# SitaoLuan/ACM-GNN

Measured on AMD Instinct MI355X. Metric: edges/sec ACM-GCN fwd+bwd on twitch-gamer, higher is better.
Workload: dtype f32; 1 GPU; twitch-gamer-shaped Chung-Lu graph: 168114 nodes, 6797557 undirected edges, nnz(A_low)=13763228, F_in=7, hidden=64, classes=2; 2-layer acmgcnp (variant=0, structure_info=0, attention LayerNorm on), dropout 0.1 (counter-based, masks regenerated in the kernels), AdamW (fused); step = fwd + NLL loss + bwd + optimizer update; parallelism=single-gpu, node_order=degree, launch=hipGraph replay of the captured step (1 consecutive steps per graph), operator_form=pattern-only P + row scale (shared by A_low and A_low^T), full=False, input_pipeline=True, checked=False

## Files before the change

acm_gnn_amd/_lib.py:

```python
import ctypes as C
import os
import threading

from . import build as _build

c_f32p = C.POINTER(C.c_float)
c_i32p = C.POINTER(C.c_int32)

ACM_OK = 0
STATUS_NAMES = {1: "ACM_EINVAL", 2: "ACM_ESHAPE", 3: "ACM_EHIP", 4: "ACM_EUNSUPPORTED", 5: "ACM_ENOMEM"}
ABI_VERSION = 28

EXPORTED_SYMBOLS = (
    "acm_version", "acm_last_error", "acm_tuning_get", "acm_tuning_set", "acm_csr_create", "acm_csr_transpose", "acm_csr_slice_rows",
    "acm_csr_destroy", "acm_csr_info", "acm_csr_build_streams", "acm_csr_build_item_streams", "acm_spmm_workspace_bytes", "acm_gemm_workspace_bytes",
    "acm_gemm", "acm_gemm_blocks", "acm_gemm_drop", "acm_proj3", "acm_gemm_split", "acm_proj_fwd", "acm_proj_fwd_at", "acm_proj_bwd_workspace_bytes", "acm_proj_bwd", "acm_spmm", "acm_spmm_v", "acm_spmm_ex", "acm_cast_bf16", "acm_conv_fwd", "acm_conv_bwd_local_workspace_bytes",
    "acm_conv_bwd_local", "acm_conv_bwd_spmm", "acm_conv_agg_fwd", "acm_conv_agg_bwd_workspace_bytes",
    "acm_conv_agg_bwd", "acm_nll_loss_workspace_bytes", "acm_nll_loss", "acm_adam_step", "acm_dropout",
    "acm_reduce_flush", "acm_conv_fwd_tail_workspace_bytes", "acm_conv_fwd_tail", "acm_shard_plan",
    "acm_conv_acmii_fwd_workspace_bytes", "acm_conv_acmii_fwd", "acm_linear_fwd", "acm_bias_act", "acm_bias_act_bwd_workspace_bytes", "acm_bias_act_bwd",
    "acm_acmii_table_bytes", "acm_acmii_table", "acm_conv_acmii_v_fwd", "acm_conv_acmii_v_bwd_workspace_bytes", "acm_conv_acmii_v_bwd",
    "acm_linear_bwd_workspace_bytes", "acm_linear_bwd", "acm_linear_fwd_add", "acm_linear_bwd_recompute",
    "acm_small_step_workspace_bytes", "acm_small_step", "acm_conv_head_fwd", "acm_conv_aggw_fwd", "acm_conv_aggw_bwd_workspace_bytes", "acm_conv_aggw_bwd",
    "acm_eval_metrics_workspace_bytes", "acm_eval_metrics",
)


class Dropout(C.Structure):
    _fields_ = [("p", C.c_float), ("tag", C.c_int32), ("seed", C.c_uint64), ("step", C.c_void_p),
                ("row_offset", C.c_int64), ("step_offset", C.c_int64)]


class CsrInfo(C.Structure):
    _fields_ = [("n_rows", C.c_int64), ("n_cols", C.c_int64), ("nnz", C.c_int64),
                ("n_items", C.c_int64), ("n_long_rows", C.c_int64), ("n_partial_slots", C.c_int64),
                ("chunk", C.c_int32), ("max_degree", C.c_int32),
                ("indptr", C.c_void_p), ("indices", C.c_void_p), ("vals", C.c_void_p),
                ("src_pos", C.c_void_p),
                ("stream_steps", C.c_int64), ("stream_slices", C.c_int64),
                ("stream_waves", C.c_int32), ("stream_long_rows", C.c_int32),
                ("item_stream_waves", C.c_int32), ("reserved", C.c_int32), ("item_stream_batches", C.c_int64)]


class ConvFwd(C.Structure):
    _fields_ = [("f_out", C.c_int32), ("n_channels", C.c_int32), ("relu_after", C.c_int32),
                ("relu_mlp", C.c_int32), ("layernorm", C.c_int32), ("scale", C.c_float),
                ("row_offset", C.c_int64),
                ("g_low", C.c_void_p), ("ld_g_low", C.c_int64),
                ("g_high", C.c_void_p), ("ld_g_high", C.c_int64),
                ("g_struc", C.c_void_p), ("ld_g_struc", C.c_int64),
                ("s_high", C.c_void_p), ("ld_s_high", C.c_int64),
                ("s_mlp", C.c_void_p), ("ld_s_mlp", C.c_int64),
                ("s_struc", C.c_void_p), ("ld_s_struc", C.c_int64),
                ("deg", C.c_void_p),
                ("att_vec", C.c_void_p * 4), ("ln_weight", C.c_void_p * 4), ("ln_bias", C.c_void_p * 4),
                ("att_mix", C.c_void_p),
                ("out", C.c_void_p), ("ld_out", C.c_int64),
                ("pre", C.c_void_p), ("ld_pre", C.c_int64),
                ("att", C.c_void_p), ("post_scale", C.c_void_p), ("ld_post_scale", C.c_int64), ("post_relu", C.c_int32),
                ("gather_bf16", C.c_int32), ("row_scale", C.c_void_p), ("post_drop", Dropout)]


class ConvBwdLocal(C.Structure):
    _fields_ = [("f_out", C.c_int32), ("n_channels", C.c_int32), ("relu_after", C.c_int32),
                ("relu_mlp", C.c_int32), ("layernorm", C.c_int32), ("scale", C.c_float),
                ("grad_out", C.c_void_p), ("ld_grad_out", C.c_int64),
                ("pre", C.c_void_p), ("ld_pre", C.c_int64),
                ("s_mlp", C.c_void_p), ("ld_s_mlp", C.c_int64),
                ("deg", C.c_void_p),
                ("att_vec", C.c_void_p * 4), ("ln_weight", C.c_void_p * 4), ("ln_bias", C.c_void_p * 4),
                ("att_mix", C.c_void_p),
                ("g_low", C.c_void_p), ("ld_g_low", C.c_int64),
                ("g_high", C.c_void_p), ("ld_g_high", C.c_int64),
                ("g_mlp", C.c_void_p), ("ld_g_mlp", C.c_int64),
                ("g_struc", C.c_void_p), ("ld_g_struc", C.c_int64),
                ("d_att_vec", C.c_void_p * 4), ("d_ln_weight", C.c_void_p * 4),
                ("d_ln_bias", C.c_void_p * 4), ("d_att_mix", C.c_void_p),
                ("post_scale", C.c_void_p), ("ld_post_scale", C.c_int64), ("post_relu", C.c_int32),
                ("g_scale", C.c_void_p), ("post_drop", Dropout), ("defer", C.c_void_p)]


class ConvBwdSpmm(C.Structure):
    _fields_ = [("f_out", C.c_int32), ("row_offset", C.c_int64),
                ("g_low", C.c_void_p), ("ld_g_low", C.c_int64),
                ("g_high", C.c_void_p), ("ld_g_high", C.c_int64),
                ("g_struc", C.c_void_p), ("ld_g_struc", C.c_int64),
                ("s_high", C.c_void_p), ("ld_s_high", C.c_int64),
                ("s_struc", C.c_void_p), ("ld_s_struc", C.c_int64),
                ("inv_deg", C.c_void_p),
                ("mask_low", C.c_void_p), ("ld_mask_low", C.c_int64),
                ("mask_high", C.c_void_p), ("ld_mask_high", C.c_int64),
                ("dz_low", C.c_void_p), ("ld_dz_low", C.c_int64),
                ("dz_high", C.c_void_p), ("ld_dz_high", C.c_int64),
                ("d_struc", C.c_void_p), ("ld_d_struc", C.c_int64), ("self_scale", C.c_void_p),
                ("gather_bf16", C.c_int32)]


class ConvAggFwd(C.Structure):
    _fields_ = [("f_in", C.c_int32), ("f_pad", C.c_int32), ("f_out", C.c_int32), ("relu_after", C.c_int32),
                ("relu_mlp", C.c_int32), ("layernorm", C.c_int32), ("scale", C.c_float),
                ("xg", C.c_void_p), ("ld_xg", C.c_int64),
                ("xs", C.c_void_p), ("ld_xs", C.c_int64),
                ("w_low", C.c_void_p), ("w_high", C.c_void_p), ("w_mlp", C.c_void_p), ("ld_w", C.c_int64),
                ("att_vec", C.c_void_p * 4), ("ln_weight", C.c_void_p * 4), ("ln_bias", C.c_void_p * 4),
                ("att_mix", C.c_void_p),
                ("out", C.c_void_p), ("ld_out", C.c_int64),
                ("agg", C.c_void_p), ("ld_agg", C.c_int64),
                ("att", C.c_void_p), ("post_scale", C.c_void_p), ("ld_post_scale", C.c_int64), ("post_relu", C.c_int32),
                ("n_channels", C.c_int32), ("sg", C.c_void_p), ("ld_sg", C.c_int64), ("sg_bf16", C.c_int32),
                ("ss", C.c_void_p), ("ld_ss", C.c_int64), ("deg", C.c_void_p),
                ("ps", C.c_void_p), ("ld_ps", C.c_int64), ("row_scale", C.c_void_p), ("post_drop", Dropout),
                ("head_stats", C.c_void_p), ("ld_head_stats", C.c_int64),
                ("next_w_low", C.c_void_p), ("next_w_high", C.c_void_p), ("next_w_mlp", C.c_void_p), ("next_ld_w", C.c_int64),
                ("next_f", C.c_int32), ("next_relu", C.c_int32),
                ("next_zlh", C.c_void_p), ("ld_next_zlh", C.c_int64), ("next_zi", C.c_void_p), ("ld_next_zi", C.c_int64),
                ("agg_given", C.c_int32), ("reserved0", C.c_int32),
                ("agg_copy", C.c_void_p), ("ld_agg_copy", C.c_int64), ("xs_copy", C.c_void_p), ("ld_xs_copy", C.c_int64),
                ("next_x", C.c_void_p), ("ld_next_x", C.c_int64), ("next_drop", Dropout)]


class ConvAggBwd(C.Structure):
    _fields_ = [("f_in", C.c_int32), ("f_pad", C.c_int32), ("f_out", C.c_int32), ("relu_after", C.c_int32),
                ("relu_mlp", C.c_int32), ("layernorm", C.c_int32), ("scale", C.c_float),
                ("grad_out", C.c_void_p), ("ld_grad_out", C.c_int64),
                ("agg", C.c_void_p), ("ld_agg", C.c_int64),
                ("xs", C.c_void_p), ("ld_xs", C.c_int64),
                ("w_low", C.c_void_p), ("w_high", C.c_void_p), ("w_mlp", C.c_void_p), ("ld_w", C.c_int64),
                ("att_vec", C.c_void_p * 4), ("ln_weight", C.c_void_p * 4), ("ln_bias", C.c_void_p * 4),
                ("att_mix", C.c_void_p),
                ("d_params", C.c_void_p), ("post_scale", C.c_void_p), ("ld_post_scale", C.c_int64), ("post_relu", C.c_int32),
                ("n_channels", C.c_int32), ("ps", C.c_void_p), ("ld_ps", C.c_int64),
                ("ss", C.c_void_p), ("ld_ss", C.c_int64), ("deg", C.c_void_p),
                ("g_struc", C.c_void_p), ("ld_g_struc", C.c_int64), ("g_struc_scale", C.c_void_p),
                ("post_drop", Dropout), ("defer", C.c_void_p),
                ("head_stats", C.c_void_p), ("ld_head_stats", C.c_int64),
                ("out", C.c_void_p), ("ld_out", C.c_int64),
                ("next_a", C.c_void_p), ("next_xg", C.c_void_p), ("ld_next_xg", C.c_int64),
                ("next_row_scale", C.c_void_p), ("next_agg", C.c_void_p), ("ld_next_agg", C.c_int64),
                ("proj_dz", C.c_void_p), ("ld_proj_dz", C.c_int64),
                ("proj_w_low", C.c_void_p), ("proj_w_high", C.c_void_p), ("proj_w_mlp", C.c_void_p), ("proj_ld_w", C.c_int64),
                ("proj_f", C.c_int32), ("proj_d_w", C.c_void_p)]


class ConvAcmiiFwd(C.Structure):
    _fields_ = [("f_in", C.c_int32), ("f_pad", C.c_int32), ("f_out", C.c_int32), ("layernorm", C.c_int32),
                ("scale", C.c_float),
                ("xg", C.c_void_p), ("ld_xg", C.c_int64), ("xs", C.c_void_p), ("ld_xs", C.c_int64),
                ("w_low", C.c_void_p), ("w_high", C.c_void_p), ("w_mlp", C.c_void_p), ("ld_w", C.c_int64),
                ("att_vec", C.c_void_p * 4), ("ln_weight", C.c_void_p * 4), ("ln_bias", C.c_void_p * 4),
                ("att_mix", C.c_void_p),
                ("out", C.c_void_p), ("ld_out", C.c_int64), ("pre", C.c_void_p), ("ld_pre", C.c_int64),
                ("att", C.c_void_p), ("zlh", C.c_void_p), ("ld_zlh", C.c_int64), ("zi", C.c_void_p), ("ld_zi", C.c_int64),
                ("post_scale", C.c_void_p), ("ld_post_scale", C.c_int64), ("post_relu", C.c_int32),
                ("row_scale", C.c_void_p), ("post_drop", Dropout),
                ("n_channels", C.c_int32), ("ps", C.c_void_p), ("ld_ps", C.c_int64), ("ss", C.c_void_p), ("ld_ss", C.c_int64),
                ("deg", C.c_void_p)]


class ConvAcmiiBwd(C.Structure):
    _fields_ = [("f_in", C.c_int32), ("table", C.c_void_p),
                ("g_low", C.c_void_p), ("ld_g_low", C.c_int64), ("g_high", C.c_void_p), ("ld_g_high", C.c_int64),
                ("g_mlp", C.c_void_p), ("ld_g_mlp", C.c_int64), ("x", C.c_void_p), ("ld_x", C.c_int64),
                ("self_offset", C.c_int64), ("row_scale", C.c_void_p),
                ("d_w_low", C.c_void_p), ("d_w_high", C.c_void_p), ("d_w_mlp", C.c_void_p), ("ld_dw", C.c_int64),
                ("defer", C.c_void_p)]


class Loss(C.Structure):
    _fields_ = [("n_classes", C.c_int32), ("labels", C.c_void_p), ("row_weight", C.c_void_p),
                ("loss", C.c_void_p), ("dlogits", C.c_void_p), ("ld_dlogits", C.c_int64)]


class ReduceSeg(C.Structure):
    _fields_ = [("partial", C.c_void_p), ("nblk", C.c_int32), ("row_stride", C.c_int32),
                ("q0", C.c_int32), ("len", C.c_int32), ("dst", C.c_void_p),
                ("inner", C.c_int32), ("col_block", C.c_int32),
                ("outer_stride", C.c_int64), ("block_stride", C.c_int64),
                ("elem_stride", C.c_int32), ("reserved", C.c_int32)]


class ReduceList(C.Structure):
    _fields_ = [("n", C.c_int32), ("cap", C.c_int32), ("segs", C.POINTER(ReduceSeg))]


class SpmmOpts(C.Structure):
    _fields_ = [("vals", C.c_void_p), ("row_scale", C.c_void_p), ("sub", C.c_void_p), ("ld_sub", C.c_int64),
                ("sub_scale", C.c_void_p), ("relu", C.c_int32), ("g_bf16", C.c_int32)]


class AdamTensor(C.Structure):
    _fields_ = [("param", C.c_void_p), ("grad", C.c_void_p), ("exp_avg", C.c_void_p), ("exp_avg_sq", C.c_void_p),
                ("step", C.c_void_p), ("numel", C.c_int64)]


class AdamConfig(C.Structure):
    _fields_ = [("lr", C.c_double), ("beta1", C.c_double), ("beta2", C.c_double), ("eps", C.c_double),
                ("weight_decay", C.c_double), ("decoupled", C.c_int32), ("also_advance", C.c_void_p),
                ("arrive", C.c_void_p), ("pending", C.c_void_p)]


SMALL_ROLES = 17
SR_W_LOW, SR_W_HIGH, SR_W_MLP, SR_V_LOW, SR_V_HIGH, SR_V_MLP, SR_V_STRUC = range(7)
SR_LNW_LOW, SR_LNW_HIGH, SR_LNW_MLP, SR_LNW_STRUC, SR_LNB_LOW, SR_LNB_HIGH, SR_LNB_MLP, SR_LNB_STRUC, SR_MIX, SR_STRUC = range(7, 17)


class SmallStep(C.Structure):
    _fields_ = [("n_classes", C.c_int32), ("n_channels", C.c_int32), ("relu_before", C.c_int32), ("layernorm", C.c_int32),
                ("scale", C.c_float), ("train", C.c_int32), ("update", C.c_int32), ("reserved0", C.c_int32),
                ("t", (AdamTensor * SMALL_ROLES) * 2),
                ("x_vals", C.c_void_p), ("xt_src_pos", C.c_void_p), ("xt_vals", C.c_void_p), ("f_in", C.c_int32), ("reserved1", C.c_int32), ("drop_in", Dropout), ("drop_hidden", Dropout),
                ("row_scale", C.c_void_p), ("labels", C.c_void_p), ("row_weight", C.c_void_p), ("loss", C.c_void_p),
                ("logits", C.c_void_p), ("att1", C.c_void_p), ("att2", C.c_void_p),
                ("lr", C.c_double), ("beta1", C.c_double), ("beta2", C.c_double), ("eps", C.c_double),
                ("weight_decay", C.c_double), ("decoupled", C.c_int32), ("also_advance", C.c_void_p), ("arrive", C.c_void_p),
                ("workspace", C.c_void_p), ("workspace_bytes", C.c_size_t)]


_lib = None
_lock = threading.Lock()


def _declare(lib):
    vp, i64, i32, sz = C.c_void_p, C.c_int64, C.c_int, C.c_size_t
    lib.acm_version.restype = C.c_int
    lib.acm_version.argtypes = []
    lib.acm_last_error.restype = C.c_char_p
    lib.acm_last_error.argtypes = []
    lib.acm_csr_create.argtypes = [i64, i64, i64, vp, vp, vp, i32, C.POINTER(vp)]
    lib.acm_csr_transpose.argtypes = [vp, i32, C.POINTER(vp)]
    lib.acm_csr_slice_rows.argtypes = [vp, i64, i64, i32, C.POINTER(vp)]
    lib.acm_csr_destroy.argtypes = [vp]
    lib.acm_csr_destroy.restype = None
    lib.acm_csr_info.argtypes = [vp, C.POINTER(CsrInfo)]
    lib.acm_csr_build_streams.argtypes = [vp, i32, i32]
    lib.acm_csr_build_item_streams.argtypes = [vp, i32]
    lib.acm_shard_plan.argtypes = [i64, vp, i32, i64, vp]
    lib.acm_conv_acmii_fwd_workspace_bytes.argtypes = [vp, C.POINTER(sz)]
    lib.acm_conv_acmii_fwd.argtypes = [vp, C.POINTER(ConvAcmiiFwd), vp, sz, vp]
    lib.acm_acmii_table_bytes.argtypes = [i64, C.POINTER(sz)]
    lib.acm_acmii_table.argtypes = [i64, i32, vp, i64, vp, vp, i64, vp, sz, vp]
    lib.acm_conv_acmii_v_fwd.argtypes = [vp, C.POINTER(ConvAcmiiFwd), vp, vp, sz, vp]
    lib.acm_conv_acmii_v_bwd_workspace_bytes.argtypes = [vp, C.POINTER(sz)]
    lib.acm_conv_acmii_v_bwd.argtypes = [vp, C.POINTER(ConvAcmiiBwd), vp, sz, vp]
    lib.acm_linear_fwd.argtypes = [i64, i64, i64, vp, i64, vp, i64, vp, i32, vp, vp, i64, vp, sz, vp]
    lib.acm_bias_act.argtypes = [i64, i32, vp, i64, vp, i32, vp, vp]
    lib.acm_linear_bwd_workspace_bytes.argtypes = [i64, i32, i32, C.POINTER(sz)]
    lib.acm_linear_bwd.argtypes = [i64, i32, i32, vp, i64, vp, i64, vp, i64, C.c_float, i32, vp, i64, vp, vp, sz, vp, vp]
    lib.acm_linear_fwd_add.argtypes = [i64, i32, i32, vp, i64, vp, i64, vp, i32, vp, vp, i64, vp, i64, vp]
    lib.acm_linear_bwd_recompute.argtypes = [i64, i32, i32, vp, i64, vp, i64, vp, i32, vp, vp, i64, vp, i64, vp, vp, sz, vp, vp]
    lib.acm_bias_act_bwd_workspace_bytes.argtypes = [i64, i32, C.POINTER(sz)]
    lib.acm_bias_act_bwd.argtypes = [i64, i32, vp, i64, vp, i64, C.c_float, i32, vp, i64, vp, vp, sz, vp, vp]
    lib.acm_spmm_workspace_bytes.argtypes = [vp, i32, C.POINTER(sz)]
    lib.acm_gemm_workspace_bytes.argtypes = [i32, i32, i64, i64, i64, C.POINTER(sz)]
    lib.acm_gemm.argtypes = [i32, i32, i64, i64, i64, vp, i64, vp, i64, vp, i64, i32, vp, sz, vp]
    lib.acm_proj_bwd_workspace_bytes.argtypes = [i64, i64, i32, C.POINTER(sz)]
    lib.acm_proj_fwd.argtypes = [i64, i64, i32, vp, i64, vp, vp, vp, i64, i32, vp, i64, vp, i64, vp]
    lib.acm_proj_fwd_at.argtypes = [i64, i64, i32, vp, i64, vp, vp, vp, i64, i32, vp, i64, i64, vp, i64, vp]
    lib.acm_proj_bwd.argtypes = [i64, i64, i32, vp, i64, vp, i64, vp, vp, vp, i64, vp, i64, vp, i64, i64, i64, vp, sz, vp, vp]
    lib.acm_gemm_split.argtypes = [i32, i32, i64, i64, i64, vp, i64, vp, i64, vp, i64, i64, vp, i64, i32, vp, sz, vp]
    lib.acm_gemm_blocks.argtypes = [i32, i32, i64, i64, i64, vp, i64, vp, i64, vp, i64, i64, i64, i32, vp, sz, vp]
    lib.acm_gemm_drop.argtypes = [i32, i32, i64, i64, i64, vp, i64, vp, i64, vp, i64, i64, i64, i32, C.POINTER(Dropout), vp, sz, vp]
    lib.acm_proj3.argtypes = [i64, i64, vp, i64, vp, vp, vp, i64, i64, i64, vp, i64, i64, vp, i64, i32, C.POINTER(Dropout), vp]
    lib.acm_spmm.argtypes = [vp, vp, i64, i32, vp, i64, vp, sz, vp]
    lib.acm_spmm_v.argtypes = [vp, vp, vp, i64, i32, vp, i64, i32, vp, sz, vp]
    lib.acm_adam_step.argtypes = [i32, vp, vp, vp]
    lib.acm_dropout.argtypes = [i64, i64, vp, i64, vp, i64, i64, vp, vp]
    lib.acm_spmm_ex.argtypes = [vp, vp, i64, i32, vp, i64, vp, vp, sz, vp]
    lib.acm_cast_bf16.argtypes = [i64, i64, vp, i64, vp, i64, vp]
    lib.acm_conv_fwd.argtypes = [vp, C.POINTER(ConvFwd), vp, sz, vp]
    lib.acm_conv_head_fwd.argtypes = [i64, C.POINTER(ConvFwd), vp]
    lib.acm_conv_aggw_bwd_workspace_bytes.argtypes = [i64, i64, C.POINTER(C.c_size_t)]
    lib.acm_conv_aggw_bwd.argtypes = [i64, i64, i64, vp, i64, vp, i64, C.POINTER(ConvBwdLocal), vp, vp, vp, i64, vp, C.c_size_t, vp]
    lib.acm_conv_aggw_fwd.argtypes = [i64, i64, i64, vp, i64, vp, i64, vp, vp, vp, i64, vp, i64, C.POINTER(ConvFwd), vp]
    lib.acm_conv_bwd_local_workspace_bytes.argtypes = [i64, i32, i32, C.POINTER(sz)]
    lib.acm_conv_bwd_local.argtypes = [i64, C.POINTER(ConvBwdLocal), vp, sz, vp]
    lib.acm_conv_bwd_spmm.argtypes = [vp, C.POINTER(ConvBwdSpmm), vp, sz, vp]
    lib.acm_conv_agg_fwd.argtypes = [vp, C.POINTER(ConvAggFwd), vp, sz, vp]
    lib.acm_conv_agg_bwd_workspace_bytes.argtypes = [i64, i32, i32, C.POINTER(sz)]
    lib.acm_conv_agg_bwd.argtypes = [i64, C.POINTER(ConvAggBwd), vp, sz, vp]
    lib.acm_nll_loss_workspace_bytes.argtypes = [i64, C.POINTER(sz)]
    lib.acm_nll_loss.argtypes = [i64, i32, vp, i64, vp, vp, vp, vp, i64, vp, sz, vp, vp]
    lib.acm_eval_metrics_workspace_bytes.argtypes = [i64, i32, C.POINTER(sz)]
    lib.acm_eval_metrics.argtypes = [i64, i32, vp, i64, vp, vp, i64, i32, i32, vp, vp, sz, vp]
    lib.acm_reduce_flush.argtypes = [vp, vp]
    lib.acm_conv_fwd_tail_workspace_bytes.argtypes = [i64, i32, i32, C.POINTER(sz)]
    lib.acm_conv_fwd_tail.argtypes = [vp, C.POINTER(ConvFwd), C.POINTER(Loss), C.POINTER(ConvBwdLocal), vp, sz, vp, sz, vp]
    lib.acm_small_step_workspace_bytes.argtypes = [vp, vp, vp, C.POINTER(sz)]
    lib.acm_small_step.argtypes = [vp, vp, vp, C.POINTER(SmallStep), vp]
    for name in EXPORTED_SYMBOLS:
        fn = getattr(lib, name)
        if name not in ("acm_version", "acm_last_error", "acm_csr_destroy"):
            fn.restype = C.c_int


def library_path():
    return os.environ.get("ACM_HIP_LIBRARY", _build.LIB_PATH)


def load(build_if_missing=True):
    global _lib
    with _lock:
        if _lib is not None:
            return _lib
        path = library_path()
        if "ACM_HIP_LIBRARY" not in os.environ and build_if_missing:
            try:
                if _build.is_stale():
                    _build.build_library()
            except Exception as exc:
                if not os.path.exists(path):
                    raise RuntimeError(f"libacm_hip.so is not built and cannot be built here: {exc}")
        if not os.path.exists(path):
            raise RuntimeError(f"libacm_hip.so not found at {path}; run `python -m acm_gnn_amd.build`")
        lib = C.CDLL(path)
        _declare(lib)
        ver = lib.acm_version()
        if ver != ABI_VERSION:
            raise RuntimeError(f"libacm_hip.so ABI version {ver} != expected {ABI_VERSION}")
        _lib = lib
        return _lib


def check(status, what=""):
    if status != ACM_OK:
        msg = load().acm_last_error().decode(errors="replace")
        raise RuntimeError(f"{what or 'libacm_hip'} failed with {STATUS_NAMES.get(status, status)}: {msg}")
```

acm_gnn_amd/csrc/acm_common.h:

```cpp
#pragma once

#include <hip/hip_runtime.h>
#include <math.h>
#include <stdint.h>

#include "acm_hip.h"

#define ACM_WAVE 64
#define ACM_NXCD 8
#define ACM_WINDOW 16
#define ACM_MIN_CHUNK 128
#define ACM_MAX_CHUNK 1024
#define ACM_GROUPS_IN_FLIGHT 8192
#define ACM_LN_EPS 1e-5f

void acm_set_error(const char* fmt, ...);
const acm_tuning_t& acm_tuning();
#define ACM_ROWS16_EPI 1
#define ACM_ROWS16_BWD 2
#define ACM_ROWS16_LOCAL 4
#define ACM_GEMM_ROWS 1
#define ACM_GEMM_BX3 2
#define ACM_GEMM_BX3_WIDE 4
#define ACM_GEMM_ROWS_ALWAYS 8

#define ACM_CHECK_HIP(expr)                                                            \
    do {                                                                               \
        hipError_t e__ = (expr);                                                       \
        if (e__ != hipSuccess) {                                                       \
            acm_set_error("%s -> %s (%s:%d)", #expr, hipGetErrorString(e__), __FILE__, \
                          __LINE__);                                                   \
            return ACM_EHIP;                                                           \
        }                                                                              \
    } while (0)

#define ACM_REQUIRE(cond, code, ...)    \
    do {                                \
        if (!(cond)) {                  \
            acm_set_error(__VA_ARGS__); \
            return (code);              \
        }                               \
    } while (0)

struct AcmItem {
    int32_t row, begin, end, slot;
};
struct AcmLongRow {
    int32_t row, slot_begin, slot_end, windows;
};

#define ACM_STREAM_SENTINEL 0x07FFFFFF
#define ACM_STREAM_PAD_STEPS 8
struct AcmStreams {
    int32_t* ids;
    int32_t* waves;
    int32_t* items;
    AcmLongRow* long_rows;
    int32_t* long_index;
    int32_t* counters;
    float* slots;
    int64_t total_steps, n_slices, n_long, n_slots;
    int32_t n_waves, lmax;
};

#define ACM_ITEM_STREAM_PAD 8
struct AcmItemStreams {
    int32_t* ids;
    int32_t* quads;
    int32_t* waves;
    int64_t total_batches, n_quads;
    int32_t n_waves;
};

struct acm_csr {
    int64_t n_rows, n_cols, nnz;
    int32_t chunk, max_degree;
    int32_t* indptr;
    int32_t* indices;
    float* vals;
    int32_t* src_pos;
    AcmItem* items;
    int64_t n_items;
    AcmLongRow* long_rows;
    int32_t* long_index;
    int64_t n_long;
    int64_t n_slots;
    int64_t n_windows;
    int64_t n_multi;
    AcmStreams* streams;
    AcmItemStreams* item_streams;
    int device;
};

struct StreamView {
    const int32_t* ids;
    const int32_t* waves;
    const int32_t* items;
    const AcmLongRow* long_rows;
    const int32_t* long_index;
    int32_t* counters;
    float* slots;
    unsigned ids_bytes, slots_bytes;
    int n_waves;
};

struct CsrView {
    const AcmItem* items;
    int n_items;
    const AcmLongRow* long_rows;
    const int32_t* long_index;
    int n_long;
    int n_windows;
    int n_multi;
    const int32_t* indices;
    const float* vals;
};

int acm_reduce_emit(acm_reduce_list_t* defer, const acm_reduce_seg_t* segs, int n, hipStream_t st);
int acm_reduce_check_segment(const acm_reduce_seg_t& sg, int index);

int acm_spmm_internal(const acm_csr* a, const void* G, int64_t ldg, int width, float* Y, int64_t ldy,
                      const acm_spmm_opts_t* o, void* workspace, size_t workspace_bytes, acm_stream_t stream,
                      bool* defer_fixup);
int acm_bwd_local_reduce(const acm_conv_bwd_local_t* p, const float* partial, int nblk, hipStream_t st);
int acm_bwd_local16(const acm_conv_bwd_local_t* p, int64_t n_rows, float* partial, int max_blocks, hipStream_t s);
int acm_agg_epi16(const acm_conv_agg_fwd_t* p, int64_t n_rows, bool* next_done, hipStream_t s);
struct GatherRole;
int acm_agg_bwd16(const acm_conv_agg_bwd_t* p, int64_t n_rows, float* partial, int max_blocks, hipStream_t s, const GatherRole* gr,
                  int gather_blocks);
int acm_acmii_fixup_launch(const acm_csr_t* a, const acm_conv_acmii_fwd_t* p, const float* partial, hipStream_t s);
bool acm_gemm_rows_nn_ok(int64_t M, int64_t N, int64_t K, const float* B, int64_t ldb);
int acm_gemm_rows_nn(int64_t M, int64_t N, int64_t K, const float* A, int64_t lda, const float* B, int64_t ldb, float* C,
                     int64_t ldc, int relu, const acm_dropout_t* drop, hipStream_t st);
bool acm_gemm_rows_tn_ok(int64_t n_rows, int64_t K, int64_t N);
int acm_gemm_rows_tn_blocks(int64_t n_rows);
int acm_gemm_rows_tn(int64_t n_rows, int64_t K, int64_t N, const float* X, int64_t ldx, const float* Dz, int64_t lddz,
                     float* slabs, int blocks, const acm_dropout_t* drop, hipStream_t st);
bool acm_gemm_bx3_nn_ok(int64_t M, int64_t N, int64_t K, const float* A, int64_t lda);
int acm_gemm_bx3_nn(int64_t M, int64_t N, int64_t K, const float* A, int64_t lda, const float* B, int64_t ldb, float* C,
                    int64_t ldc, int relu, const acm_dropout_t* drop, hipStream_t st);
bool acm_gemm_bx3_tn_ok(int64_t n_rows, int64_t K, int64_t N);
int acm_gemm_bx3_tn_blocks(int64_t n_rows, int64_t K);
int acm_gemm_bx3_tn(int64_t n_rows, int64_t K, int64_t N, const float* X, int64_t ldx, const float* Dz, int64_t lddz,
                    float* slabs, int blocks, const acm_dropout_t* drop, hipStream_t st);
int acm_linear_fwd_narrow(int64_t n_rows, int64_t f_in, int64_t f_out, const float* X, int64_t ldx, const float* W, int64_t ldw,
                          const float* bias, int relu, const acm_dropout_t* drop, float* Y, int64_t ldy, hipStream_t s,
                          const float* add, int64_t ld_add);

static inline CsrView acm_view(const acm_csr* a) {
    CsrView v;
    v.items = a->items;
    v.n_items = (int)a->n_items;
    v.long_rows = a->long_rows;
    v.long_index = a->long_index;
    v.n_long = (int)a->n_long;
    v.n_windows = (int)a->n_windows;
    v.n_multi = (int)a->n_multi;
    v.indices = a->indices;
    v.vals = a->vals;
    return v;
}

#ifdef __HIPCC__
template <int CTRL>
__device__ __forceinline__ float acm_dpp(float v) {
    return __int_as_float(__builtin_amdgcn_update_dpp(0, __float_as_int(v), CTRL, 0xf, 0xf, false));
}
typedef unsigned acm_u32x2 __attribute__((ext_vector_type(2)));
template <int W>
__device__ __forceinline__ float acm_group_sum(float v) {
    static_assert(W == 1 || W == 2 || W == 4 || W == 8 || W == 16 || W == 32 || W == 64, "group width");
    if (W >= 2) v += acm_dpp<0xB1>(v);
    if (W >= 4) v += acm_dpp<0x4E>(v);
    if (W >= 8) v += acm_dpp<0x141>(v);
    if (W >= 16) v += acm_dpp<0x140>(v);
    if (W >= 32) {
        const acm_u32x2 r = __builtin_amdgcn_permlane16_swap(__float_as_uint(v), __float_as_uint(v), false, false);
        v = __uint_as_float(r[0]) + __uint_as_float(r[1]);
    }
    if (W >= 64) {
        const acm_u32x2 r = __builtin_amdgcn_permlane32_swap(__float_as_uint(v), __float_as_uint(v), false, false);
        v = __uint_as_float(r[0]) + __uint_as_float(r[1]);
    }
    return v;
}

__device__ __forceinline__ float acm_cross_row_sum(float v) {
    acm_u32x2 r = __builtin_amdgcn_permlane16_swap(__float_as_uint(v), __float_as_uint(v), false, false);
    v = __uint_as_float(r[0]) + __uint_as_float(r[1]);
    r = __builtin_amdgcn_permlane32_swap(__float_as_uint(v), __float_as_uint(v), false, false);
    return __uint_as_float(r[0]) + __uint_as_float(r[1]);
}

__device__ __forceinline__ int acm_row_bcast(int v, int u) {
#define ACM_BC(U) case U: return __builtin_amdgcn_update_dpp(0, v, 0x150 + U, 0xf, 0xf, false)
    switch (u & 15) {
        ACM_BC(0); ACM_BC(1); ACM_BC(2); ACM_BC(3); ACM_BC(4); ACM_BC(5); ACM_BC(6); ACM_BC(7);
        ACM_BC(8); ACM_BC(9); ACM_BC(10); ACM_BC(11); ACM_BC(12); ACM_BC(13); ACM_BC(14);
        default: return __builtin_amdgcn_update_dpp(0, v, 0x15F, 0xf, 0xf, false);
    }
#undef ACM_BC
}

__device__ __forceinline__ int acm_uniform(int v) { return __builtin_amdgcn_readfirstlane(v); }
__device__ __forceinline__ float acm_lane_f(float v, int lane) {
    return __int_as_float(__builtin_amdgcn_readlane(__float_as_int(v), lane));
}

__device__ __forceinline__ float acm_nll_row(int C, const float* zi, int yi, float wi, float* di) {
    if (wi == 0.f) {
        for (int c = 0; c < C; ++c) di[c] = 0.f;
        return 0.f;
    }
    float m = -INFINITY;
    for (int c = 0; c < C; ++c) m = fmaxf(m, zi[c]);
    float s = 0.f;
    for (int c = 0; c < C; ++c) s += expf(zi[c] - m);
    const float lse = m + logf(s);
    const float inv = 1.0f / s;
    const float zy = zi[yi];
    for (int c = 0; c < C; ++c) di[c] = wi * (expf(zi[c] - m) * inv - (c == yi ? 1.f : 0.f));
    return wi * (lse - zy);
}

struct AcmDropCtx {
    unsigned k0, k1, c2, c3, thresh, tag16;
    float inv_keep;
    long row_offset;
    bool on;
};

__device__ __forceinline__ AcmDropCtx acm_drop_ctx(const acm_dropout_t& d) {
    AcmDropCtx c;
    c.on = d.p > 0.f;
    const unsigned long long step = c.on ? (unsigned long long)(d.step[0] + d.step_offset) : 0ull;
    c.k0 = (unsigned)d.seed;
    c.k1 = (unsigned)(d.seed >> 32);
    c.c2 = (unsigned)step;
    c.c3 = (unsigned)(step >> 32);
    const double t = (double)d.p * 4294967296.0;
    c.thresh = t >= 4294967295.0 ? 0xFFFFFFFFu : (unsigned)t;
    c.tag16 = ((unsigned)d.tag) << 16;
    c.inv_keep = 1.0f / (1.0f - d.p);
    c.row_offset = (long)d.row_offset;
    return c;
// ... 42 lines not shown
```

acm_gnn_amd/csrc/acm_conv.hip:

```cpp
#include "acm_gather_device.h"

struct EpiFwd {
    static constexpr bool kFusedHead = true;
    using Args = acm_conv_fwd_t;
    template <class L, int NG>
    static __device__ __forceinline__ void apply(const Args& p, int row, const L& lay, int F,
                                                 const float (&acc)[NG][L::NV]) {
        constexpr int NV = L::NV;
        float H[4][NV], hn[4][NV], xhat[4][NV], pre[3][NV];
        const float dg = (NG == 3) ? p.deg[row] : 0.f;
        const float rs = p.row_scale ? p.row_scale[row] : 1.f;
#pragma unroll
        for (int i = 0; i < NV; ++i) {
            const int col = lay.col(i);
            const bool ok = col < F;
            const float zh = ok ? p.s_high[(long)row * p.ld_s_high + col] : 0.f;
            const float zi = ok ? p.s_mlp[(long)row * p.ld_s_mlp + col] : 0.f;
            const float p0 = rs * acc[0][i];
            const float p1 = zh - rs * acc[1][i];
            pre[0][i] = p0;
            pre[1][i] = p1;
            H[0][i] = p.relu_after ? fmaxf(p0, 0.f) : p0;
            H[1][i] = p.relu_after ? fmaxf(p1, 0.f) : p1;
            H[2][i] = p.relu_mlp ? fmaxf(zi, 0.f) : zi;
// ... 62 lines not shown
                                                            const float* __restrict__ partial, int row_blocks) {
    const int F = p.f_out;
    float acc[NG][FP];
    if ((int)blockIdx.x >= row_blocks) {
        const int m = threadIdx.x & 15;
        const int w = ((int)blockIdx.x - row_blocks) * 16 + (threadIdx.x >> 4);
        if (w >= csr.n_long) return;
        const AcmLongRow lr = csr.long_rows[w];
#pragma unroll
        for (int c = 0; c < NG; ++c)
#pragma unroll
            for (int f = 0; f < FP; ++f) acc[c][f] = 0.f;
        for (int s = lr.slot_begin + m; s < lr.slot_end; s += 16) {
            const float* ps = partial + (long)s * (NG * F);
#pragma unroll
            for (int c = 0; c < NG; ++c)
#pragma unroll
                for (int f = 0; f < FP; ++f)
                    if (f < F) acc[c][f] += ps[c * F + f];
        }
#pragma unroll
        for (int c = 0; c < NG; ++c)
#pragma unroll
            for (int f = 0; f < FP; ++f) acc[c][f] = acm_group_sum<16>(acc[c][f]);
        const LaySerial<FP> lay{m == 0};
        EpiFwd::apply<LaySerial<FP>, NG>(p, lr.row, lay, F, acc);
        return;
    }
    const int row = blockIdx.x * 256 + threadIdx.x;
    if (row >= n_rows) return;
    if (csr.long_index && csr.long_index[row] >= 0) return;
    const float* pr = p.pre + (long)row * p.ld_pre;
#pragma unroll
    for (int c = 0; c < NG; ++c)
#pragma unroll
        for (int f = 0; f < FP; ++f) acc[c][f] = (f < F) ? pr[c * F + f] : 0.f;
    const LaySerial<FP> lay{true};
    EpiFwd::apply<LaySerial<FP>, NG>(p, row, lay, F, acc);
}

__global__ __launch_bounds__(256) void conv_head_rows_kernel(acm_conv_fwd_t p, int n_rows) {
    const int lane = threadIdx.x & 63, m = lane & 15;
    const int row = ((int)blockIdx.x * 4 + (threadIdx.x >> 6)) * 4 + (lane >> 4);
    if (row >= n_rows) return;
    constexpr int F = 64;
    const float4 a = *reinterpret_cast<const float4*>(p.g_low + (long)row * p.ld_g_low + 4 * m);
    const float4 b = *reinterpret_cast<const float4*>(p.g_high + (long)row * p.ld_g_high + 4 * m);
    const float4 zh4 = *reinterpret_cast<const float4*>(p.s_high + (long)row * p.ld_s_high + 4 * m);
    const float4 zi4 = *reinterpret_cast<const float4*>(p.s_mlp + (long)row * p.ld_s_mlp + 4 * m);
    const float aa[4] = {a.x, a.y, a.z, a.w}, bb[4] = {b.x, b.y, b.z, b.w};
    const float zh[4] = {zh4.x, zh4.y, zh4.z, zh4.w}, zi[4] = {zi4.x, zi4.y, zi4.z, zi4.w};
    float H[4][4], hn[4][4], xhat[4][4], pre[2][4];
#pragma unroll
    for (int i = 0; i < 4; ++i) {
        const float p0 = 1.f * aa[i];
        const float p1 = zh[i] - 1.f * bb[i];
        pre[0][i] = p0, pre[1][i] = p1;
        H[0][i] = p.relu_after ? fmaxf(p0, 0.f) : p0;
        H[1][i] = p.relu_after ? fmaxf(p1, 0.f) : p1;
        H[2][i] = p.relu_mlp ? fmaxf(zi[i], 0.f) : zi[i];
        H[3][i] = 0.f;
    }
    const LayRow16 lay{lane};
    HeadOut ho;
    const HeadParams hp = acm_head_params(p);
    acm_head<LayRow16, 3>(lay, F, p.layernorm, hp, H, hn, xhat, ho);
    float o[4];
    const AcmDropCtx dc = acm_drop_ctx(p.post_drop);
#pragma unroll
    for (int i = 0; i < 4; ++i) {
        const int col = 4 * m + i;
        float v = ho.alpha[0] * H[0][i] + ho.alpha[1] * H[1][i] + ho.alpha[2] * H[2][i];
        v *= p.scale;
        if (p.post_relu) v = fmaxf(v, 0.f);
        if (p.post_scale) v *= p.post_scale[(long)row * p.ld_post_scale + col];
        if (p.post_drop.p > 0.f) v *= acm_drop1(dc, row, col);
        o[i] = v;
    }
    *reinterpret_cast<float4*>(p.out + (long)row * p.ld_out + 4 * m) = make_float4(o[0], o[1], o[2], o[3]);
    float* pr = p.pre + (long)row * p.ld_pre + 4 * m;
    *reinterpret_cast<float4*>(pr) = make_float4(pre[0][0], pre[0][1], pre[0][2], pre[0][3]);
    *reinterpret_cast<float4*>(pr + F) = make_float4(pre[1][0], pre[1][1], pre[1][2], pre[1][3]);
    if (m == 0) *reinterpret_cast<float4*>(p.att + (long)row * 4) = make_float4(ho.alpha[0], ho.alpha[1], ho.alpha[2], ho.alpha[3]);
}

extern "C" int acm_conv_head_fwd(int64_t n_rows, const acm_conv_fwd_t* p, acm_stream_t stream) {
    ACM_REQUIRE(p, ACM_EINVAL, "acm_conv_head_fwd: NULL argument");
    ACM_REQUIRE(n_rows >= 0 && n_rows < INT32_MAX, ACM_ESHAPE, "acm_conv_head_fwd: bad row count");
    ACM_REQUIRE(p->f_out == 64 && p->n_channels == 3 && !p->gather_bf16 && !p->row_scale && !p->deg, ACM_EUNSUPPORTED,
                "acm_conv_head_fwd: three fp32 channels of 64 columns, no row scale (got F %d, k %d)", p->f_out, p->n_channels);
    ACM_REQUIRE(p->g_low && p->g_high && p->s_high && p->s_mlp && p->out && p->pre && p->att && p->att_mix, ACM_EINVAL,
                "acm_conv_head_fwd: NULL pointer in the parameter block");
    const uintptr_t bits = (uintptr_t)p->g_low | (uintptr_t)p->g_high | (uintptr_t)p->s_high | (uintptr_t)p->s_mlp | (uintptr_t)p->out |
                           (uintptr_t)p->pre | (uintptr_t)p->att;
    ACM_REQUIRE((p->ld_g_low | p->ld_g_high | p->ld_s_high | p->ld_s_mlp | p->ld_out | p->ld_pre) % 4 == 0 && (bits & 15) == 0,
                ACM_EUNSUPPORTED, "acm_conv_head_fwd: every row (inputs, out, pre, att) must be 16-byte aligned");
    if (n_rows == 0) return ACM_OK;
    hipLaunchKernelGGL(conv_head_rows_kernel, dim3((unsigned)((n_rows + 15) / 16)), dim3(256), 0, (hipStream_t)stream, *p, (int)n_rows);
    ACM_CHECK_HIP(hipGetLastError());
    return ACM_OK;
}

extern "C" int acm_conv_fwd(const acm_csr_t* a, const acm_conv_fwd_t* p, void* workspace,
                            size_t workspace_bytes, acm_stream_t stream) {
    ACM_REQUIRE(a && p, ACM_EINVAL, "acm_conv_fwd: NULL argument");
    const int F = p->f_out, k = p->n_channels;
    ACM_REQUIRE(F > 0 && (k == 3 || k == 4), ACM_ESHAPE, "acm_conv_fwd: f_out %d n_channels %d", F, k);
    ACM_REQUIRE(p->g_low && p->g_high && p->s_high && p->s_mlp && p->out && p->pre && p->att &&
                    p->att_mix, ACM_EINVAL, "acm_conv_fwd: NULL tensor pointer");
    for (int c = 0; c < k; ++c) {
        ACM_REQUIRE(p->att_vec[c], ACM_EINVAL, "acm_conv_fwd: att_vec[%d] is NULL", c);
        ACM_REQUIRE(!p->layernorm || (p->ln_weight[c] && p->ln_bias[c]), ACM_EINVAL,
                    "acm_conv_fwd: layernorm parameters of channel %d are NULL", c);
    }
    ACM_REQUIRE(p->ld_out >= F && p->ld_pre >= (k - 1) * F, ACM_ESHAPE,
                "acm_conv_fwd: ld_out %lld / ld_pre %lld too small", (long long)p->ld_out,
                (long long)p->ld_pre);
    ACM_REQUIRE(((uintptr_t)p->att) % 16 == 0, ACM_EINVAL, "acm_conv_fwd: att must be 16-byte aligned");
    ACM_REQUIRE(k == 3 || (p->g_struc && p->s_struc && p->deg), ACM_EINVAL,
                "acm_conv_fwd: structure channel pointers are NULL");
    const GatherSrc g = {{p->g_low, p->g_high, k == 4 ? p->g_struc : nullptr}, {p->ld_g_low, p->ld_g_high, k == 4 ? p->ld_g_struc : 0}};
    hipStream_t s = (hipStream_t)stream;
    int st = ACM_OK;
    if (F > 8) {
        acm_with_k(k, [&](auto kc) {
            st = launch_gather<decltype(kc)::value - 1, EpiFwd>(a, g, F, *p, workspace, workspace_bytes, s, "acm_conv_fwd", nullptr, p->gather_bf16 != 0);
        });
        return st;
    }
    ACM_REQUIRE(!p->gather_bf16, ACM_EUNSUPPORTED, "acm_conv_fwd: bf16 operands need F > 8");
    acm_with_k(k, [&](auto kc) {
        st = launch_gather<decltype(kc)::value - 1, EpiRaw>(a, g, F, *p, workspace, workspace_bytes, s, "acm_conv_fwd", nullptr, false, true);
    });
    if (st != ACM_OK || a->n_rows == 0) return st;
    const int grid = (int)((a->n_rows + 255) / 256), n = (int)a->n_rows;
    CsrView cv = acm_view(a);
    const float* part = (const float*)workspace;
    const bool done = narrow_finishes_long_rows(a);
    if (done) cv.long_index = nullptr;
    const int tail = done ? 0 : (int)((a->n_long + 15) / 16);
    acm_with_fp(F, [&](auto fp) {
        acm_with_k(k, [&](auto kc) {
            hipLaunchKernelGGL((conv_fwd_rows_kernel<decltype(fp)::value, decltype(kc)::value - 1>), dim3(grid + tail), dim3(256), 0, s, *p, n,
                               cv, part, grid);
        });
    });
    ACM_CHECK_HIP(hipGetLastError());
    return ACM_OK;
}

template <int FP, int NG>
__global__ __launch_bounds__(256) void conv_tail_rows_kernel(acm_conv_fwd_t pf, acm_loss_t pl, acm_conv_bwd_local_t pb,
                                                             int n_rows, float* __restrict__ loss_partial,
                                                             float* __restrict__ k3_partial) {
    extern __shared__ float lds[];
    __shared__ float red[256];
    constexpr int K = NG + 1;
    const int F = pf.f_out;
    const int npg = 3 * K * F + K * K;
    const int row = blockIdx.x * 256 + threadIdx.x;
    const bool active = row < n_rows;
    const LaySerial<FP> lay{true};
    ParamAcc<LaySerial<FP>> pa;
    pa.zero();
    float term = 0.f;
    if (active) {
        float acc[NG][FP];
        const float* pr = pf.pre + (long)row * pf.ld_pre;
#pragma unroll
        for (int c = 0; c < NG; ++c)
#pragma unroll
            for (int f = 0; f < FP; ++f) acc[c][f] = (f < F) ? pr[c * F + f] : 0.f;
        EpiFwd::apply<LaySerial<FP>, NG>(pf, row, lay, F, acc);
        term = acm_nll_row(F, pf.out + (long)row * pf.ld_out, (int)pl.labels[row], pl.row_weight[row],
                           pl.dlogits + (long)row * pl.ld_dlogits);
        conv_bwd_row<LaySerial<FP>, K>(pb, row, true, lay, pa);
    }
    red[threadIdx.x] = term;
    __syncthreads();
    for (int m = 128; m >= 1; m >>= 1) {
        if ((int)threadIdx.x < m) red[threadIdx.x] += red[threadIdx.x + m];
        __syncthreads();
    }
    if (threadIdx.x == 0) loss_partial[blockIdx.x] = red[0];
    bwd_local_block_reduce<LaySerial<FP>, 64, K>(pa, lay, F, lds, k3_partial + (long)blockIdx.x * npg);
}

__device__ __forceinline__ float acm_group8_max(float v) {
    v = fmaxf(v, acm_dpp<0xB1>(v));
    v = fmaxf(v, acm_dpp<0x4E>(v));
    return fmaxf(v, acm_dpp<0x141>(v));
}

template <int NG>
__global__ __launch_bounds__(256) void conv_tail_packed8_kernel(acm_conv_fwd_t pf, acm_loss_t pl, acm_conv_bwd_local_t pb,
                                                                int n_rows, float* __restrict__ loss_partial,
                                                                float* __restrict__ k3_partial) {
    extern __shared__ float lds[];
    __shared__ float red[256];
    constexpr int K = NG + 1;
    using L = LayPacked<8>;
    const int F = pf.f_out;
    const int npg = 3 * K * F + K * K;
    const int lane = threadIdx.x & 63, col = lane & 7;
    const int row = blockIdx.x * 32 + (threadIdx.x >> 3);
    const bool active = row < n_rows;
    const int rr = active ? row : 0;
    const L lay{lane};
    ParamAcc<L> pa;
    pa.zero();
    float term = 0.f;
    {
        float acc[NG][1];
        const float* pr = pf.pre + (long)rr * pf.ld_pre;
#pragma unroll
        for (int c = 0; c < NG; ++c) acc[c][0] = (col < F) ? pr[c * F + col] : 0.f;
        if (active) EpiFwd::apply<L, NG>(pf, rr, lay, F, acc);
        const bool mine = active && col < F;
        const float z = mine ? pf.out[(long)rr * pf.ld_out + col] : -INFINITY;
        const float wi = active ? pl.row_weight[rr] : 0.f;
        const int yi = active ? (int)pl.labels[rr] : 0;
        const float m = acm_group8_max(z);
        const float e = mine ? expf(z - m) : 0.f;
        const float ssum = acm_group_sum<8>(e);
        const float zy = acm_group_sum<8>((mine && col == yi) ? z : 0.f);
        if (mine) pl.dlogits[(long)rr * pl.ld_dlogits + col] = (wi == 0.f) ? 0.f : wi * (e / ssum - (col == yi ? 1.f : 0.f));
        if (active && col == 0 && wi != 0.f) term = wi * (m + logf(ssum) - zy);
        conv_bwd_row<L, K>(pb, rr, active, lay, pa);
    }
    red[threadIdx.x] = term;
    __syncthreads();
    for (int m = 128; m >= 1; m >>= 1) {
        if ((int)threadIdx.x < m) red[threadIdx.x] += red[threadIdx.x + m];
        __syncthreads();
    }
    if (threadIdx.x == 0) loss_partial[blockIdx.x] = red[0];
    bwd_local_block_reduce<L, 8, K>(pa, lay, F, lds, k3_partial + (long)blockIdx.x * npg);
}

extern "C" int acm_conv_fwd_tail_workspace_bytes(int64_t n_rows, int f_out, int n_channels, size_t* bytes) {
    ACM_REQUIRE(bytes, ACM_EINVAL, "acm_conv_fwd_tail_workspace_bytes: NULL argument");
    ACM_REQUIRE(n_rows >= 0 && f_out > 0 && f_out <= 8 && n_channels == 3, ACM_EUNSUPPORTED,
                "acm_conv_fwd_tail: f_out %d n_channels %d (needs f_out <= 8, three channels)", f_out, n_channels);
    const int64_t rows_per_block = f_out > 4 ? 32 : 256;
    const int64_t nblk = (n_rows + rows_per_block - 1) / rows_per_block > 0 ? (n_rows + rows_per_block - 1) / rows_per_block : 1;
    *bytes = (size_t)nblk * (size_t)(1 + 3 * n_channels * f_out + n_channels * n_channels) * sizeof(float);
    return ACM_OK;
}

extern "C" int acm_conv_fwd_tail(const acm_csr_t* a, const acm_conv_fwd_t* p, const acm_loss_t* l,
                                 const acm_conv_bwd_local_t* b, void* workspace, size_t workspace_bytes,
                                 void* tail_workspace, size_t tail_workspace_bytes, acm_stream_t stream) {
    ACM_REQUIRE(a && p && l && b, ACM_EINVAL, "acm_conv_fwd_tail: NULL argument");
    const int F = p->f_out, k = p->n_channels;
    size_t need = 0;
    int st = acm_conv_fwd_tail_workspace_bytes(a->n_rows, F, k, &need);
    if (st != ACM_OK) return st;
    ACM_REQUIRE(l->n_classes == F && b->f_out == F && b->n_channels == k, ACM_EUNSUPPORTED,
                "acm_conv_fwd_tail: the layer's f_out must be the number of classes");
    ACM_REQUIRE(!p->post_relu && !p->post_scale && p->post_drop.p == 0.f && !b->post_relu && !b->post_scale &&
                    b->post_drop.p == 0.f && !p->gather_bf16, ACM_EUNSUPPORTED,
                "acm_conv_fwd_tail: post-ops / bf16 operands are not part of the fused tail");
    ACM_REQUIRE(a->n_long == 0 || narrow_finishes_long_rows(a), ACM_EUNSUPPORTED,
                "acm_conv_fwd_tail: this graph's narrow gather leaves partial sums of long rows");
    ACM_REQUIRE(p->g_low && p->g_high && p->s_high && p->s_mlp && p->out && p->pre && p->att && p->att_mix &&
                    l->labels && l->row_weight && l->loss && l->dlogits && b->att_mix && b->g_low && b->g_high &&
                    b->g_mlp && b->d_att_mix, ACM_EINVAL, "acm_conv_fwd_tail: NULL tensor pointer");
    ACM_REQUIRE(b->grad_out == l->dlogits && b->ld_grad_out == l->ld_dlogits && b->pre == p->pre &&
                    b->ld_pre == p->ld_pre && b->s_mlp == p->s_mlp && b->ld_s_mlp == p->ld_s_mlp, ACM_EINVAL,
                "acm_conv_fwd_tail: bwd must read what fwd / loss write (grad_out = dlogits, pre, s_mlp)");
    ACM_REQUIRE(p->ld_out >= F && p->ld_pre >= (k - 1) * F && l->ld_dlogits >= F && ((uintptr_t)p->att) % 16 == 0,
                ACM_ESHAPE, "acm_conv_fwd_tail: leading dimensions / alignment");
    for (int c = 0; c < k; ++c) {
        ACM_REQUIRE(p->att_vec[c] && b->att_vec[c], ACM_EINVAL, "acm_conv_fwd_tail: att_vec[%d] is NULL", c);
        ACM_REQUIRE(!p->layernorm || (p->ln_weight[c] && p->ln_bias[c] && b->ln_weight[c] && b->ln_bias[c]), ACM_EINVAL,
                    "acm_conv_fwd_tail: layernorm parameters of channel %d are NULL", c);
    }
    ACM_REQUIRE(tail_workspace && tail_workspace_bytes >= need, ACM_ENOMEM,
                "acm_conv_fwd_tail: tail workspace %zu B < required %zu B", tail_workspace_bytes, need);
    if (a->n_rows == 0) return ACM_OK;
    hipStream_t s = (hipStream_t)stream;
    GatherSrc g = {{p->g_low, p->g_high, nullptr}, {p->ld_g_low, p->ld_g_high, 0}};
    st = launch_gather<2, EpiRaw>(a, g, F, *p, workspace, workspace_bytes, s, "acm_conv_fwd_tail", nullptr, false, true);
    if (st != ACM_OK) return st;
    const bool packed = F > 4;
    const int n = (int)a->n_rows, nblk = packed ? (n + 31) / 32 : (n + 255) / 256;
    const int npg = 3 * k * F + k * k;
    float* loss_partial = (float*)tail_workspace;
    float* k3_partial = loss_partial + nblk;
    const size_t lds = (size_t)4 * npg * sizeof(float);
    acm_with_fp(F, [&](auto fp) {
        if constexpr (decltype(fp)::value == 8)
            hipLaunchKernelGGL((conv_tail_packed8_kernel<2>), dim3(nblk), dim3(256), lds, s, *p, *l, *b, n, loss_partial, k3_partial);
        else
            hipLaunchKernelGGL((conv_tail_rows_kernel<decltype(fp)::value, 2>), dim3(nblk), dim3(256), lds, s, *p, *l, *b, n, loss_partial,
                               k3_partial);
    });
    ACM_CHECK_HIP(hipGetLastError());
    const acm_reduce_seg_t seg = {loss_partial, nblk, 1, 0, 1, l->loss, 1, 0, 0, 0};
    st = acm_reduce_emit(b->defer, &seg, 1, s);
    if (st != ACM_OK) return st;
    return acm_bwd_local_reduce(b, k3_partial, nblk, s);
}
```

acm_gnn_amd/csrc/acm_csr.cpp:

```cpp
#include <stdarg.h>
#include <stdio.h>
#include <string.h>

#include <stdlib.h>

#include <algorithm>
#include <functional>
#include <new>
#include <queue>
#include <string>
#include <utility>
#include <vector>

#include "acm_common.h"

static thread_local char g_err[512] = "";

void acm_set_error(const char* fmt, ...) {
    va_list ap;
    va_start(ap, fmt);
    vsnprintf(g_err, sizeof(g_err), fmt, ap);
    va_end(ap);
}

extern "C" int acm_version(void) { return ACM_ABI_VERSION; }
extern "C" const char* acm_last_error(void) { return g_err; }

namespace {
const acm_tuning_t kTuningDefaults = {0, 0, -1, 7, 1, 7, {0}};
struct TuningField { const char* name; int32_t acm_tuning_t::*field; };
const TuningField kTuningFields[] = {{"chunk", &acm_tuning_t::chunk},           {"wide_form", &acm_tuning_t::wide_form},
                                     {"bwd_split", &acm_tuning_t::bwd_split},   {"rows16", &acm_tuning_t::rows16},
                                     {"agg_fused", &acm_tuning_t::agg_fused},   {"gemm_forms", &acm_tuning_t::gemm_forms}};
const char* const kHostKeys[] = {"rewrites", "implicit", "relabel", "pipeline", "csr_features", "small_step"};

const char* tuning_invalid(const acm_tuning_t& t) {
    if (t.chunk != 0 && (t.chunk < 8 || t.chunk > 4096 || (t.chunk & (t.chunk - 1)))) return "chunk";
    if (t.wide_form < 0 || t.wide_form > 3) return "wide_form";
    if (t.bwd_split < -1 || t.bwd_split > 1) return "bwd_split";
    if (t.rows16 < 0 || t.rows16 > 7) return "rows16";
    if (t.agg_fused < 0 || t.agg_fused > 1) return "agg_fused";
    if (t.gemm_forms < 0 || t.gemm_forms > 15) return "gemm_forms";
    return nullptr;
}

acm_tuning_t tuning_from_environment() {
    acm_tuning_t t = kTuningDefaults;
    const char* env = getenv("ACM_TUNING");
    if (!env) return t;
    std::string text(env);
    size_t pos = 0;
    while (pos < text.size()) {
        size_t end = text.find(',', pos);
        if (end == std::string::npos) end = text.size();
        const std::string item = text.substr(pos, end - pos);
        pos = end + 1;
        if (item.empty()) continue;
        const size_t eq = item.find('=');
        const std::string key = item.substr(0, eq), val = eq == std::string::npos ? "" : item.substr(eq + 1);
        bool known = false;
        for (const char* h : kHostKeys) known = known || key == h;
        for (const TuningField& f : kTuningFields) {
            if (key != f.name) continue;
            known = true;
            char* stop = nullptr;
            const long v = strtol(val.c_str(), &stop, 0);
            acm_tuning_t probe = t;
            probe.*(f.field) = (int32_t)v;
            if (val.empty() || *stop || tuning_invalid(probe)) fprintf(stderr, "libacm_hip: ACM_TUNING: bad value '%s' ignored\n", item.c_str());
            else t = probe;
        }
        if (!known) fprintf(stderr, "libacm_hip: ACM_TUNING: unknown key '%s' ignored\n", key.c_str());
    }
    return t;
}
const acm_tuning_t g_tuning_loaded = tuning_from_environment();
acm_tuning_t g_tuning = g_tuning_loaded;
}

const acm_tuning_t& acm_tuning() { return g_tuning; }

extern "C" int acm_tuning_get(acm_tuning_t* out) {
    ACM_REQUIRE(out, ACM_EINVAL, "acm_tuning_get: NULL argument");
    *out = g_tuning;
    return ACM_OK;
}

extern "C" int acm_tuning_set(const acm_tuning_t* in) {
    if (!in) {
        g_tuning = g_tuning_loaded;
        return ACM_OK;
    }
    const char* bad = tuning_invalid(*in);
    ACM_REQUIRE(!bad, ACM_EINVAL, "acm_tuning_set: field '%s' out of range", bad);
    g_tuning = *in;
    for (int32_t& r : g_tuning.reserved) r = 0;
    return ACM_OK;
}

namespace {

void free_streams(AcmStreams* t) {
    if (!t) return;
    for (void* q : {(void*)t->ids, (void*)t->waves, (void*)t->items, (void*)t->long_rows,
                    (void*)t->long_index, (void*)t->counters, (void*)t->slots})
        if (q) (void)hipFree(q);
    delete t;
}

void free_item_streams(AcmItemStreams* t) {
    if (!t) return;
    for (void* q : {(void*)t->ids, (void*)t->quads, (void*)t->waves})
        if (q) (void)hipFree(q);
    delete t;
}

void free_handle(acm_csr* a) {
    if (!a) return;
    if (a->indptr) (void)hipFree(a->indptr);
    if (a->indices) (void)hipFree(a->indices);
    if (a->vals) (void)hipFree(a->vals);
    if (a->long_index) (void)hipFree(a->long_index);
    if (a->src_pos) (void)hipFree(a->src_pos);
    if (a->items) (void)hipFree(a->items);
    if (a->long_rows) (void)hipFree(a->long_rows);
    free_streams(a->streams);
    free_item_streams(a->item_streams);
    delete a;
}

void build_items(const std::vector<int32_t>& indptr, int chunk, std::vector<AcmItem>& items,
                 std::vector<AcmLongRow>& longs, int64_t& n_slots, int32_t& max_deg, int64_t& n_windows, int64_t& n_multi) {
    const int64_t n = (int64_t)indptr.size() - 1;
    items.clear();
    longs.clear();
    items.reserve(n + n / 8);
    n_slots = 0;
    max_deg = 0;
    n_multi = 0;
    for (int64_t r = 0; r < n; ++r) {
        const int32_t b = indptr[r], e = indptr[r + 1];
        const int32_t deg = e - b;
        max_deg = std::max(max_deg, deg);
        if (deg <= chunk) continue;
        int32_t pieces = (deg + chunk - 1) / chunk;
        int32_t windows = 0;
        if (pieces > ACM_WINDOW && (deg + ACM_WINDOW - 1) / ACM_WINDOW > 4 * chunk) {
            windows = (deg + 2 * ACM_WINDOW * chunk - 1) / (2 * ACM_WINDOW * chunk);
            if (windows > ACM_WINDOW) windows = ACM_WINDOW;
            pieces = windows * ACM_WINDOW;
        } else if (pieces > ACM_WINDOW) {
            pieces = ACM_WINDOW;
        }
        const int32_t room = ACM_WINDOW - (int32_t)(items.size() % ACM_WINDOW);
        if ((room < pieces || windows) && room < ACM_WINDOW) {
            AcmLongRow& prev = longs.back();
            for (int32_t q = 0; q < room; ++q) items.push_back({prev.row, indptr[prev.row + 1], indptr[prev.row + 1], (int32_t)n_slots++});
            prev.slot_end = (int32_t)n_slots;
        }
        const int32_t per = (deg + pieces - 1) / pieces;
        AcmLongRow lr = {(int32_t)r, (int32_t)n_slots, 0, windows};
        for (int32_t q = 0; q < pieces; ++q) {
            const int32_t s = std::min(e, b + q * per);
            items.push_back({(int32_t)r, s, std::min(e, s + per), (int32_t)n_slots++});
        }
        lr.slot_end = (int32_t)n_slots;
        n_multi += windows > 1;
        longs.push_back(lr);
    }
    if (!longs.empty() && items.size() % ACM_WINDOW) {
        AcmLongRow& prev = longs.back();
        while (items.size() % ACM_WINDOW) items.push_back({prev.row, indptr[prev.row + 1], indptr[prev.row + 1], (int32_t)n_slots++});
        prev.slot_end = (int32_t)n_slots;
    }
    n_windows = (int64_t)items.size() / ACM_WINDOW;
    for (int64_t r = 0; r < n; ++r)
        if (indptr[r + 1] - indptr[r] <= chunk) items.push_back({(int32_t)r, indptr[r], indptr[r + 1], -1});
}

int finish_handle(acm_csr* a, const std::vector<int32_t>& h_indptr, int chunk) {
    const int env_chunk = acm_tuning().chunk;
    int auto_chunk = ACM_MIN_CHUNK;
    while (auto_chunk < ACM_MAX_CHUNK && 2 * (int64_t)auto_chunk <= a->nnz / ACM_GROUPS_IN_FLIGHT) auto_chunk *= 2;
    a->chunk = chunk > 0 ? chunk : (env_chunk > 0 ? env_chunk : auto_chunk);
    std::vector<AcmItem> items;
    std::vector<AcmLongRow> longs;
    build_items(h_indptr, a->chunk, items, longs, a->n_slots, a->max_degree, a->n_windows, a->n_multi);
    a->n_items = (int64_t)items.size();
    a->n_long = (int64_t)longs.size();
    if (a->n_items) {
        ACM_CHECK_HIP(hipMalloc((void**)&a->items, items.size() * sizeof(AcmItem)));
        ACM_CHECK_HIP(hipMemcpy(a->items, items.data(), items.size() * sizeof(AcmItem),
                                hipMemcpyHostToDevice));
    }
    if (a->n_long) {
        ACM_CHECK_HIP(hipMalloc((void**)&a->long_rows, longs.size() * sizeof(AcmLongRow)));
        ACM_CHECK_HIP(hipMemcpy(a->long_rows, longs.data(), longs.size() * sizeof(AcmLongRow),
                                hipMemcpyHostToDevice));
        std::vector<int32_t> index((size_t)a->n_rows, -1);
        for (size_t i = 0; i < longs.size(); ++i) index[(size_t)longs[i].row] = (int32_t)i;
        ACM_CHECK_HIP(hipMalloc((void**)&a->long_index, index.size() * sizeof(int32_t)));
        ACM_CHECK_HIP(hipMemcpy(a->long_index, index.data(), index.size() * sizeof(int32_t), hipMemcpyHostToDevice));
    }
    return ACM_OK;
}

acm_csr* new_handle(int64_t n_rows, int64_t n_cols, int64_t nnz) {
    acm_csr* a = new (std::nothrow) acm_csr();
    if (!a) return nullptr;
    memset(a, 0, sizeof(*a));
    a->n_rows = n_rows;
    a->n_cols = n_cols;
    a->nnz = nnz;
    (void)hipGetDevice(&a->device);
    return a;
}

int alloc_arrays(acm_csr* a, bool with_vals = true) {
    ACM_CHECK_HIP(hipMalloc((void**)&a->indptr, (size_t)(a->n_rows + 1) * sizeof(int32_t)));
    const size_t m = (size_t)std::max<int64_t>(a->nnz, 1);
    ACM_CHECK_HIP(hipMalloc((void**)&a->indices, m * sizeof(int32_t)));
    if (with_vals) ACM_CHECK_HIP(hipMalloc((void**)&a->vals, m * sizeof(float)));
    return ACM_OK;
}

}

extern "C" int acm_csr_create(int64_t n_rows, int64_t n_cols, int64_t nnz,
                              const int32_t* indptr_dev, const int32_t* indices_dev,
                              const float* vals_dev, int chunk, acm_csr_t** out) {
    ACM_REQUIRE(out, ACM_EINVAL, "acm_csr_create: out is NULL");
    *out = nullptr;
    ACM_REQUIRE(indptr_dev, ACM_EINVAL, "acm_csr_create: indptr is NULL");
    ACM_REQUIRE(nnz == 0 || indices_dev, ACM_EINVAL, "acm_csr_create: indices NULL with nnz > 0");
    ACM_REQUIRE(n_rows >= 0 && n_cols >= 0 && nnz >= 0, ACM_ESHAPE, "acm_csr_create: negative size");
    ACM_REQUIRE(n_rows < INT32_MAX && n_cols < INT32_MAX && nnz < INT32_MAX, ACM_EUNSUPPORTED,
                "acm_csr_create: sizes must fit int32 (rows %lld cols %lld nnz %lld)",
                (long long)n_rows, (long long)n_cols, (long long)nnz);
    ACM_CHECK_HIP(hipDeviceSynchronize());
    std::vector<int32_t> h_indptr((size_t)n_rows + 1);
    ACM_CHECK_HIP(hipMemcpy(h_indptr.data(), indptr_dev, h_indptr.size() * sizeof(int32_t),
                            hipMemcpyDeviceToHost));
    ACM_REQUIRE(h_indptr[0] == 0 && h_indptr[n_rows] == nnz, ACM_ESHAPE,
                "acm_csr_create: indptr[0]=%d indptr[n]=%d but nnz=%lld", h_indptr[0],
                h_indptr[n_rows], (long long)nnz);
    for (int64_t r = 0; r < n_rows; ++r)
        ACM_REQUIRE(h_indptr[r] <= h_indptr[r + 1], ACM_ESHAPE,
                    "acm_csr_create: indptr not monotone at row %lld", (long long)r);
    if (nnz) {
        std::vector<int32_t> h_idx((size_t)nnz);
        ACM_CHECK_HIP(hipMemcpy(h_idx.data(), indices_dev, (size_t)nnz * sizeof(int32_t),
                                hipMemcpyDeviceToHost));
        for (int64_t k = 0; k < nnz; ++k)
            ACM_REQUIRE(h_idx[k] >= 0 && h_idx[k] < n_cols, ACM_ESHAPE,
                        "acm_csr_create: column id %d out of range at position %lld", h_idx[k],
                        (long long)k);
    }
    acm_csr* a = new_handle(n_rows, n_cols, nnz);
    ACM_REQUIRE(a, ACM_ENOMEM, "acm_csr_create: host allocation failed");
    int st = alloc_arrays(a, vals_dev != nullptr);
    if (st == ACM_OK) {
        hipError_t e = hipMemcpy(a->indptr, indptr_dev, (size_t)(n_rows + 1) * sizeof(int32_t),
                                 hipMemcpyDeviceToDevice);
        if (e == hipSuccess && nnz)
            e = hipMemcpy(a->indices, indices_dev, (size_t)nnz * sizeof(int32_t),
                          hipMemcpyDeviceToDevice);
        if (e == hipSuccess && nnz && vals_dev)
            e = hipMemcpy(a->vals, vals_dev, (size_t)nnz * sizeof(float), hipMemcpyDeviceToDevice);
        if (e != hipSuccess) {
            acm_set_error("acm_csr_create: device copy failed: %s", hipGetErrorString(e));
            st = ACM_EHIP;
        }
    }
    if (st == ACM_OK) st = finish_handle(a, h_indptr, chunk);
    if (st != ACM_OK) {
        free_handle(a);
        return st;
    }
    *out = a;
    return ACM_OK;
}

extern "C" int acm_csr_transpose(const acm_csr_t* a, int chunk, acm_csr_t** out) {
    ACM_REQUIRE(a && out, ACM_EINVAL, "acm_csr_transpose: NULL argument");
    *out = nullptr;
    ACM_CHECK_HIP(hipDeviceSynchronize());
    const int64_t n = a->n_rows, m = a->n_cols, nnz = a->nnz;
    std::vector<int32_t> ip((size_t)n + 1), ix((size_t)nnz);
    std::vector<float> v((size_t)nnz);
    ACM_CHECK_HIP(hipMemcpy(ip.data(), a->indptr, ip.size() * sizeof(int32_t), hipMemcpyDeviceToHost));
    if (nnz) {
        ACM_CHECK_HIP(hipMemcpy(ix.data(), a->indices, (size_t)nnz * sizeof(int32_t), hipMemcpyDeviceToHost));
        if (a->vals) ACM_CHECK_HIP(hipMemcpy(v.data(), a->vals, (size_t)nnz * sizeof(float), hipMemcpyDeviceToHost));
    }
    std::vector<int32_t> tp((size_t)m + 1, 0), tx((size_t)nnz), tpos((size_t)nnz);
    std::vector<float> tv((size_t)nnz);
    for (int64_t k = 0; k < nnz; ++k) ++tp[(size_t)ix[k] + 1];
    for (int64_t c = 0; c < m; ++c) tp[c + 1] += tp[c];
    std::vector<int32_t> cur(tp.begin(), tp.end() - 1);
    for (int64_t r = 0; r < n; ++r)
        for (int32_t k = ip[r]; k < ip[r + 1]; ++k) {
            const int32_t pos = cur[ix[k]]++;
            tx[pos] = (int32_t)r;
            tv[pos] = v[k];
            tpos[pos] = k;
        }
    acm_csr* t = new_handle(m, n, nnz);
    ACM_REQUIRE(t, ACM_ENOMEM, "acm_csr_transpose: host allocation failed");
    int st = alloc_arrays(t, a->vals != nullptr);
    if (st == ACM_OK) {
        hipError_t e = hipMemcpy(t->indptr, tp.data(), tp.size() * sizeof(int32_t), hipMemcpyHostToDevice);
        if (e == hipSuccess && nnz)
            e = hipMemcpy(t->indices, tx.data(), (size_t)nnz * sizeof(int32_t), hipMemcpyHostToDevice);
        if (e == hipSuccess && nnz && t->vals)
            e = hipMemcpy(t->vals, tv.data(), (size_t)nnz * sizeof(float), hipMemcpyHostToDevice);
        if (e == hipSuccess) e = hipMalloc((void**)&t->src_pos, (size_t)(nnz > 0 ? nnz : 1) * sizeof(int32_t));
        if (e == hipSuccess && nnz)
            e = hipMemcpy(t->src_pos, tpos.data(), (size_t)nnz * sizeof(int32_t), hipMemcpyHostToDevice);
        if (e != hipSuccess) {
            acm_set_error("acm_csr_transpose: upload failed: %s", hipGetErrorString(e));
            st = ACM_EHIP;
        }
    }
    if (st == ACM_OK) st = finish_handle(t, tp, chunk);
    if (st != ACM_OK) {
        free_handle(t);
        return st;
    }
    *out = t;
    return ACM_OK;
}

extern "C" int acm_csr_slice_rows(const acm_csr_t* a, int64_t row_begin, int64_t row_end, int chunk,
                                  acm_csr_t** out) {
    ACM_REQUIRE(a && out, ACM_EINVAL, "acm_csr_slice_rows: NULL argument");
    *out = nullptr;
    ACM_REQUIRE(0 <= row_begin && row_begin <= row_end && row_end <= a->n_rows, ACM_ESHAPE,
                "acm_csr_slice_rows: bad range [%lld,%lld) of %lld rows", (long long)row_begin,
                (long long)row_end, (long long)a->n_rows);
    ACM_CHECK_HIP(hipDeviceSynchronize());
    const int64_t n = row_end - row_begin;
    std::vector<int32_t> ip((size_t)n + 1);
    ACM_CHECK_HIP(hipMemcpy(ip.data(), a->indptr + row_begin, ip.size() * sizeof(int32_t),
                            hipMemcpyDeviceToHost));
    const int32_t base = ip[0];
    for (auto& x : ip) x -= base;
    const int64_t nnz = ip[n];
    acm_csr* s = new_handle(n, a->n_cols, nnz);
    ACM_REQUIRE(s, ACM_ENOMEM, "acm_csr_slice_rows: host allocation failed");
    int st = alloc_arrays(s, a->vals != nullptr);
    if (st == ACM_OK) {
        hipError_t e = hipMemcpy(s->indptr, ip.data(), ip.size() * sizeof(int32_t), hipMemcpyHostToDevice);
        if (e == hipSuccess && nnz)
            e = hipMemcpy(s->indices, a->indices + base, (size_t)nnz * sizeof(int32_t), hipMemcpyDeviceToDevice);
        if (e == hipSuccess && nnz && a->vals)
            e = hipMemcpy(s->vals, a->vals + base, (size_t)nnz * sizeof(float), hipMemcpyDeviceToDevice);
        if (e != hipSuccess) {
            acm_set_error("acm_csr_slice_rows: copy failed: %s", hipGetErrorString(e));
            st = ACM_EHIP;
        }
    }
    if (st == ACM_OK) st = finish_handle(s, ip, chunk);
    if (st != ACM_OK) {
        free_handle(s);
        return st;
    }
    *out = s;
    return ACM_OK;
}

extern "C" void acm_csr_destroy(acm_csr_t* a) { free_handle(a); }

extern "C" int acm_shard_plan(int64_t n_rows, const int64_t* indptr, int world, int64_t row_cost, int64_t* bounds) {
    ACM_REQUIRE(indptr && bounds, ACM_EINVAL, "acm_shard_plan: NULL argument");
    ACM_REQUIRE(n_rows >= 0 && world >= 1 && row_cost >= 0, ACM_ESHAPE, "acm_shard_plan: n_rows %lld world %d row_cost %lld",
                (long long)n_rows, world, (long long)row_cost);
    ACM_REQUIRE(indptr[0] == 0, ACM_EINVAL, "acm_shard_plan: indptr[0] must be 0");
    auto cost = [&](int64_t r) { return (__int128)indptr[r] + (__int128)row_cost * r; };
    const __int128 total = cost(n_rows);
    bounds[0] = 0;
    for (int p = 1; p < world; ++p) {
        const __int128 target = total * p / world;
        int64_t lo = bounds[p - 1], hi = n_rows;
        while (lo < hi) {
            const int64_t mid = lo + (hi - lo) / 2;
            if (cost(mid) >= target) hi = mid; else lo = mid + 1;
        }
        int64_t r = lo;
        if (r > bounds[p - 1] && target - cost(r - 1) < cost(r) - target) --r;
        bounds[p] = r;
    }
    bounds[world] = n_rows;
    return ACM_OK;
}


namespace {

template <class T>
int upload(T** dev, const std::vector<T>& host, size_t min_elems = 1) {
    const size_t n = std::max(host.size(), min_elems);
    ACM_CHECK_HIP(hipMalloc((void**)dev, n * sizeof(T)));
    if (!host.empty()) ACM_CHECK_HIP(hipMemcpy(*dev, host.data(), host.size() * sizeof(T), hipMemcpyHostToDevice));
    return ACM_OK;
}

}

extern "C" int acm_csr_build_streams(acm_csr_t* a, int n_waves, int lmax) {
    ACM_REQUIRE(a, ACM_EINVAL, "acm_csr_build_streams: NULL handle");
    if (a->streams) return ACM_OK;
    ACM_REQUIRE(a->vals == nullptr, ACM_EUNSUPPORTED, "acm_csr_build_streams: pattern-only operators only");
    ACM_REQUIRE(a->n_cols < ACM_STREAM_SENTINEL, ACM_EUNSUPPORTED, "acm_csr_build_streams: %lld columns", (long long)a->n_cols);
    if (lmax <= 0) lmax = 512;
    ACM_REQUIRE(lmax % 32 == 0 && lmax <= 4096, ACM_EINVAL, "acm_csr_build_streams: lmax %d must be a multiple of 32, at most 4096", lmax);
    ACM_CHECK_HIP(hipDeviceSynchronize());
    const int64_t n = a->n_rows, nnz = a->nnz;
    std::vector<int32_t> ip((size_t)n + 1), ix((size_t)nnz);
    ACM_CHECK_HIP(hipMemcpy(ip.data(), a->indptr, ip.size() * sizeof(int32_t), hipMemcpyDeviceToHost));
    if (nnz) ACM_CHECK_HIP(hipMemcpy(ix.data(), a->indices, (size_t)nnz * sizeof(int32_t), hipMemcpyDeviceToHost));
    struct Item { int32_t row, begin, len, slot; };
    std::vector<Item> items;
    items.reserve((size_t)n + (size_t)(nnz / lmax) + 16);
    std::vector<AcmLongRow> longs;
    int64_t n_slots = 0;
    for (int64_t r = 0; r < n; ++r) {
        const int32_t b = ip[r], deg = ip[r + 1] - ip[r];
        if (deg <= lmax) {
            items.push_back({(int32_t)r, b, deg, -1});
            continue;
        }
        const int32_t pieces = (deg + lmax - 1) / lmax;
        const int32_t per = (((deg + pieces - 1) / pieces) + 31) / 32 * 32;
        AcmLongRow lr = {(int32_t)r, (int32_t)n_slots, 0, 0};
        for (int32_t q = 0; q * per < deg; ++q) items.push_back({(int32_t)r, b + q * per, std::min(per, deg - q * per), (int32_t)n_slots++});
        lr.slot_end = (int32_t)n_slots;
        longs.push_back(lr);
    }
    std::stable_sort(items.begin(), items.end(), [](const Item& x, const Item& y) { return x.len > y.len; });
    const int64_t n_items = (int64_t)items.size(), n_slices = (n_items + 3) / 4;
    std::vector<int32_t> sl_steps((size_t)n_slices);
    int64_t total_steps = 0;
    for (int64_t s = 0; s < n_slices; ++s) {
        int32_t longest = 0;
        for (int64_t i = s * 4; i < std::min(n_items, s * 4 + 4); ++i) longest = std::max(longest, items[(size_t)i].len);
        sl_steps[(size_t)s] = std::max(1, (longest + 31) / 32);
        total_steps += sl_steps[(size_t)s];
    }
    ACM_REQUIRE((total_steps + ACM_STREAM_PAD_STEPS) * 512 < (int64_t)0xFFFFFFF0u, ACM_EUNSUPPORTED,
                "acm_csr_build_streams: %lld steps exceed 32-bit stream offsets", (long long)total_steps);
    if (n_waves <= 0) {
        int cus = 256;
        (void)hipDeviceGetAttribute(&cus, hipDeviceAttributeMultiprocessorCount, a->device);
        n_waves = cus * 4 * 5;
    }
    if ((int64_t)n_waves > n_slices) n_waves = (int)std::max<int64_t>(n_slices, 1);
    n_waves = (n_waves + 3) / 4 * 4;
    const int64_t epi_cost = 1;
    std::vector<int32_t> wave_of((size_t)n_slices);
    {
        typedef std::pair<int64_t, int32_t> Load;
        std::priority_queue<Load, std::vector<Load>, std::greater<Load>> heap;
        for (int32_t w = 0; w < n_waves; ++w) heap.push({0, w});
        for (int64_t s = 0; s < n_slices; ++s) {
            Load l = heap.top();
            heap.pop();
            wave_of[(size_t)s] = l.second;
            l.first += 4 * (int64_t)sl_steps[(size_t)s] + epi_cost;
            heap.push(l);
        }
    }
    std::vector<int32_t> count((size_t)n_waves + 1, 0);
    for (int64_t s = 0; s < n_slices; ++s) ++count[(size_t)wave_of[(size_t)s] + 1];
    for (int32_t w = 0; w < n_waves; ++w) count[(size_t)w + 1] += count[(size_t)w];
    std::vector<int32_t> pos_of((size_t)n_slices), cur(count.begin(), count.end() - 1);
    for (int64_t s = 0; s < n_slices; ++s) pos_of[(size_t)s] = cur[(size_t)wave_of[(size_t)s]]++;
    {
        {
            std::vector<int32_t> slice_at((size_t)n_slices);
            for (int64_t s = 0; s < n_slices; ++s) slice_at[(size_t)pos_of[(size_t)s]] = (int32_t)s;
            for (int32_t w = 0; w < n_waves; ++w) {
                const int32_t b = count[(size_t)w], m = count[(size_t)w + 1] - b;
                uint64_t state = 0x9E3779B97F4A7C15ull * (uint64_t)(w + 1);
                for (int32_t i = m - 1; i > 0; --i) {
                    state = state * 6364136223846793005ull + 1442695040888963407ull;
                    const int32_t j = (int32_t)((state >> 33) % (uint64_t)(i + 1));
                    std::swap(slice_at[(size_t)(b + i)], slice_at[(size_t)(b + j)]);
                }
            }
            for (int64_t q = 0; q < n_slices; ++q) pos_of[(size_t)slice_at[(size_t)q]] = (int32_t)q;
        }
    }
    std::vector<int32_t> h_steps((size_t)n_slices + 2, 1), h_items(((size_t)n_slices + 2) * 16, -1), step_base((size_t)n_slices + 1, 0);
    for (int64_t s = 0; s < n_slices; ++s) h_steps[(size_t)pos_of[(size_t)s]] = sl_steps[(size_t)s];
    for (int64_t q = 0; q < n_slices; ++q) step_base[(size_t)q + 1] = step_base[(size_t)q] + h_steps[(size_t)q];
    std::vector<int32_t> h_waves((size_t)n_waves * 4);
    for (int32_t w = 0; w < n_waves; ++w) {
        const int32_t b = count[(size_t)w], e = count[(size_t)w + 1];
        h_waves[(size_t)w * 4 + 0] = b;
        h_waves[(size_t)w * 4 + 1] = e;
        h_waves[(size_t)w * 4 + 2] = step_base[(size_t)b];
        h_waves[(size_t)w * 4 + 3] = step_base[(size_t)e] - step_base[(size_t)b];
    }
    std::vector<int32_t> h_ids(((size_t)total_steps + ACM_STREAM_PAD_STEPS) * 128, ACM_STREAM_SENTINEL);
    for (int64_t s = 0; s < n_slices; ++s) {
        const size_t q = (size_t)pos_of[(size_t)s];
        for (int g = 0; g < 4; ++g) {
            const int64_t i = s * 4 + g;
            if (i >= n_items) break;
            const Item& it = items[(size_t)i];
            h_items[q * 16 + 4 * g + 0] = it.row;
            h_items[q * 16 + 4 * g + 1] = it.slot;
            int32_t* dst = h_ids.data() + (size_t)step_base[q] * 128 + (size_t)g * 32;
            for (int32_t k = 0; k < it.len; ++k) dst[(size_t)(k >> 5) * 128 + (k & 31)] = ix[(size_t)it.begin + k];
        }
    }
    for (size_t q = 0; q < (size_t)n_slices + 2; ++q)
        for (int g = 0; g < 4; ++g) h_items[q * 16 + 4 * g + 2] = h_steps[q], h_items[q * 16 + 4 * g + 3] = 0;
    AcmStreams* t = new (std::nothrow) AcmStreams();
    ACM_REQUIRE(t, ACM_ENOMEM, "acm_csr_build_streams: host allocation failed");
    memset(t, 0, sizeof(*t));
    t->total_steps = total_steps;
    t->n_slices = n_slices;
    t->n_long = (int64_t)longs.size();
    t->n_slots = n_slots;
    t->n_waves = n_waves;
    t->lmax = lmax;
    int st = upload(&t->ids, h_ids);
    if (st == ACM_OK) st = upload(&t->waves, h_waves);
    if (st == ACM_OK) st = upload(&t->items, h_items);
    if (st == ACM_OK && !longs.empty()) {
        st = upload(&t->long_rows, longs);
        std::vector<int32_t> index((size_t)n, -1);
        for (size_t i = 0; i < longs.size(); ++i) index[(size_t)longs[i].row] = (int32_t)i;
        if (st == ACM_OK) st = upload(&t->long_index, index);
        if (st == ACM_OK && hipMalloc((void**)&t->counters, longs.size() * sizeof(int32_t)) != hipSuccess) st = ACM_EHIP;
        if (st == ACM_OK && hipMemset(t->counters, 0, longs.size() * sizeof(int32_t)) != hipSuccess) st = ACM_EHIP;
        if (st == ACM_OK && hipMalloc((void**)&t->slots, (size_t)n_slots * 8 * sizeof(float)) != hipSuccess) st = ACM_EHIP;
        if (st == ACM_EHIP) acm_set_error("acm_csr_build_streams: device allocation failed");
    }
    if (st != ACM_OK) {
        free_streams(t);
        return st;
    }
    a->streams = t;
    return ACM_OK;
}

extern "C" int acm_csr_build_item_streams(acm_csr_t* a, int n_waves) {
    ACM_REQUIRE(a, ACM_EINVAL, "acm_csr_build_item_streams: NULL handle");
    if (a->item_streams) return ACM_OK;
    ACM_REQUIRE(a->vals == nullptr, ACM_EUNSUPPORTED, "acm_csr_build_item_streams: pattern-only operators only");
    ACM_REQUIRE(a->n_items > 0 && a->nnz > 0, ACM_EUNSUPPORTED, "acm_csr_build_item_streams: empty operator");
    ACM_REQUIRE(a->n_cols < ((int64_t)1 << 31) - 1, ACM_EUNSUPPORTED, "acm_csr_build_item_streams: %lld columns", (long long)a->n_cols);
    ACM_CHECK_HIP(hipDeviceSynchronize());
    const int64_t n_items = a->n_items, nnz = a->nnz;
    std::vector<AcmItem> items((size_t)n_items);
    std::vector<AcmLongRow> longs((size_t)a->n_long);
    std::vector<int32_t> ix((size_t)nnz), lidx;
    ACM_CHECK_HIP(hipMemcpy(items.data(), a->items, items.size() * sizeof(AcmItem), hipMemcpyDeviceToHost));
    ACM_CHECK_HIP(hipMemcpy(ix.data(), a->indices, ix.size() * sizeof(int32_t), hipMemcpyDeviceToHost));
    if (a->n_long) {
        ACM_REQUIRE(a->long_index, ACM_EUNSUPPORTED, "acm_csr_build_item_streams: handle without a long-row index");
        lidx.resize((size_t)a->n_rows);
        ACM_CHECK_HIP(hipMemcpy(longs.data(), a->long_rows, longs.size() * sizeof(AcmLongRow), hipMemcpyDeviceToHost));
        ACM_CHECK_HIP(hipMemcpy(lidx.data(), a->long_index, lidx.size() * sizeof(int32_t), hipMemcpyDeviceToHost));
    }
    const int64_t n_quads = (n_items + 3) / 4;
    std::vector<int32_t> qb((size_t)n_quads, 0);
    int64_t total = 0;
    for (int64_t i = 0; i < n_items; ++i) {
        const int32_t nb = (items[(size_t)i].end - items[(size_t)i].begin + 31) / 32;
        qb[(size_t)(i / 4)] += nb;
        total += nb;
    }
    ACM_REQUIRE((total + ACM_ITEM_STREAM_PAD) * 128 < ((int64_t)1 << 32), ACM_EUNSUPPORTED,
                "acm_csr_build_item_streams: %lld batches exceed 32-bit stream offsets", (long long)total);
    if (n_waves <= 0) {
        int cus = 256;
        (void)hipDeviceGetAttribute(&cus, hipDeviceAttributeMultiprocessorCount, a->device);
        n_waves = cus * 8;
    }
    if ((int64_t)n_waves > n_quads) n_waves = (int)n_quads;
    n_waves = (n_waves + 3) / 4 * 4;
    const int64_t quad_cost = 10;
    std::vector<int32_t> order((size_t)n_quads), wave_of((size_t)n_quads);
    for (int64_t q = 0; q < n_quads; ++q) order[(size_t)q] = (int32_t)q;
    std::stable_sort(order.begin(), order.end(), [&](int32_t x, int32_t y) { return qb[(size_t)x] > qb[(size_t)y]; });
    {
        typedef std::pair<int64_t, int32_t> Load;
        std::priority_queue<Load, std::vector<Load>, std::greater<Load>> heap;
        for (int32_t w = 0; w < n_waves; ++w) heap.push({0, w});
        for (int64_t o = 0; o < n_quads; ++o) {
            Load l = heap.top();
            heap.pop();
            wave_of[(size_t)order[(size_t)o]] = l.second;
            l.first += qb[(size_t)order[(size_t)o]] + quad_cost;
            heap.push(l);
        }
    }
    std::vector<int32_t> count((size_t)n_waves + 1, 0);
    for (int64_t q = 0; q < n_quads; ++q) ++count[(size_t)wave_of[(size_t)q] + 1];
    for (int32_t w = 0; w < n_waves; ++w) count[(size_t)w + 1] += count[(size_t)w];
    std::vector<int32_t> cur(count.begin(), count.end() - 1), quad_at((size_t)n_quads);
    for (int64_t o = 0; o < n_quads; ++o) quad_at[(size_t)cur[(size_t)wave_of[(size_t)order[(size_t)o]]]++] = order[(size_t)o];
    const int32_t zero_row = (int32_t)a->n_cols;
    std::vector<int32_t> h_quads((size_t)n_quads * 16, 0), h_waves((size_t)n_waves * 4, 0),
        h_ids(((size_t)total + ACM_ITEM_STREAM_PAD) * 32, zero_row);
    int64_t batch = 0;
    for (int32_t w = 0; w < n_waves; ++w) {
        h_waves[(size_t)w * 4 + 0] = count[(size_t)w];
        h_waves[(size_t)w * 4 + 1] = count[(size_t)w + 1];
        h_waves[(size_t)w * 4 + 2] = (int32_t)batch;
        for (int32_t pos = count[(size_t)w]; pos < count[(size_t)w + 1]; ++pos) {
            const int64_t q = quad_at[(size_t)pos];
            for (int g = 0; g < 4; ++g) {
                int32_t* d = h_quads.data() + (size_t)pos * 16 + 4 * g;
                const int64_t i = q * 4 + g;
                d[1] = -1;
                if (i >= n_items) continue;
                const AcmItem& it = items[(size_t)i];
                const int32_t len = it.end - it.begin, nb = (len + 31) / 32;
                bool owner = it.slot < 0;
                if (!owner) owner = longs[(size_t)lidx[(size_t)it.row]].slot_begin == it.slot;
                d[0] = it.row, d[1] = it.slot, d[2] = nb, d[3] = 1 | (owner ? 2 : 0);
                for (int32_t k = 0; k < len; ++k) h_ids[(size_t)batch * 32 + (size_t)k] = ix[(size_t)it.begin + (size_t)k];
                batch += nb;
            }
        }
        h_waves[(size_t)w * 4 + 3] = (int32_t)batch - h_waves[(size_t)w * 4 + 2];
    }
    AcmItemStreams* t = new (std::nothrow) AcmItemStreams();
    ACM_REQUIRE(t, ACM_ENOMEM, "acm_csr_build_item_streams: host allocation failed");
    memset(t, 0, sizeof(*t));
    t->total_batches = total;
    t->n_quads = n_quads;
    t->n_waves = n_waves;
    int st = upload(&t->ids, h_ids);
    if (st == ACM_OK) st = upload(&t->quads, h_quads);
    if (st == ACM_OK) st = upload(&t->waves, h_waves);
    if (st != ACM_OK) {
        free_item_streams(t);
        return st;
    }
    a->item_streams = t;
    return ACM_OK;
}

extern "C" int acm_csr_info(const acm_csr_t* a, acm_csr_info_t* info) {
    ACM_REQUIRE(a && info, ACM_EINVAL, "acm_csr_info: NULL argument");
    info->n_rows = a->n_rows;
    info->n_cols = a->n_cols;
    info->nnz = a->nnz;
    info->n_items = a->n_items;
    info->n_long_rows = a->n_long;
    info->n_partial_slots = a->n_slots;
    info->chunk = a->chunk;
    info->max_degree = a->max_degree;
    info->indptr = a->indptr;
    info->indices = a->indices;
    info->vals = a->vals;
    info->src_pos = a->src_pos;
    info->stream_steps = a->streams ? a->streams->total_steps : 0;
    info->stream_slices = a->streams ? a->streams->n_slices : 0;
    info->stream_waves = a->streams ? a->streams->n_waves : 0;
    info->stream_long_rows = a->streams ? (int32_t)a->streams->n_long : 0;
    info->item_stream_waves = a->item_streams ? a->item_streams->n_waves : 0;
    info->reserved = 0;
    info->item_stream_batches = a->item_streams ? a->item_streams->total_batches : 0;
    return ACM_OK;
}

extern "C" int acm_spmm_workspace_bytes(const acm_csr_t* a, int width, size_t* bytes) {
    ACM_REQUIRE(a && bytes, ACM_EINVAL, "acm_spmm_workspace_bytes: NULL argument");
    ACM_REQUIRE(width > 0, ACM_ESHAPE, "acm_spmm_workspace_bytes: width must be positive");
    *bytes = (size_t)a->n_slots * (size_t)width * sizeof(float);
    return ACM_OK;
}
```

acm_gnn_amd/functional/__init__.py:

```python
from .. import _lib, tuning
from ..graph import CsrGraph, FilterOperators, SparseFeatures, _device_ctx, _require_cuda, _stream
from ._launch import KernelTimer, _Timed, set_kernel_timer
from ._context import (CallContext, DeferredReductions, InputPipeline, Tape, TapeBroken, _ambient,
                       deferred_reductions, deferred_reductions_as, fused_loss_tail, input_pipeline, on_tape)
from .ops import (DropoutState, _drop_spec, agg_pad_width, cast_bf16, dropout, eval_metrics, eval_metrics_buffers,
                  gemm, gemm_drop_supported, gemm_split, masked_nll, mm, nll_loss_and_grad, proj3, proj_bwd,
                  proj_bwd_supported, proj_fwd, spmm, spmm_v)
from .linear import residual_add_linear, residual_add_supported, residual_linear
from ._conv_shared import AcmConfig, _flat_views, _gather_rows, _ptr_array
from .conv_agg import AGG_WIDE_MIN_DEGREE, _AcmAggWide, agg_wide_supported
from .conv_literal import _AcmAcmii
from .conv import _conv_route, acm_conv, in_drop_supported
```

acm_gnn_amd/functional/_context.py:

```python
import bisect
import ctypes as C
import threading

import torch

from .. import _lib, tuning
from ._launch import _F32, _Timed, _vp, launch


class DeferredReductions:
    CAP = 96

    def __init__(self):
        self._segs = (_lib.ReduceSeg * self.CAP)()
        self._list = _lib.ReduceList(0, self.CAP, C.cast(self._segs, C.POINTER(_lib.ReduceSeg)))
        self._keep = []
        self.outputs = []
        self._allreduce = []

    def pointer(self):
        return C.addressof(self._list)

    def hold(self, workspace, outputs, keep=None):
        self._keep.append(workspace)
        self._keep.extend(outputs if keep is None else keep)
        self.outputs.extend((t.data_ptr(), t.numel() * t.element_size()) for t in outputs if t is not None)

    @property
    def pending(self):
        return int(self._list.n)

    def all_adopted(self, tensors):
        ptrs = sorted(t.data_ptr() for t in tensors if t is not None)
        for a, nb in self.outputs:
            i = bisect.bisect_left(ptrs, a)
            if i == len(ptrs) or ptrs[i] >= a + nb:
                return False
        return True

    def allreduce(self, tensor, group):
        self._allreduce.append((tensor, group))

    def flush(self):
        if self._list.n:
            launch("acm_reduce_flush", "reduce_flush", self._keep[0].device, C.byref(self._list))
        if self._allreduce:
            import torch.distributed as dist
            pending, self._allreduce = self._allreduce, []
            group = pending[0][1]
            coalesce = (len(pending) > 1 and all(g is group for _, g in pending) and hasattr(dist, "_coalescing_manager")
                        and dist.get_backend(group) == "nccl")
            with _Timed("all_reduce/gradients", sum(t.numel() * t.element_size() for t, _ in pending)):
                if coalesce:
                    with dist._coalescing_manager(group=group, device=pending[0][0].device, async_ops=False):
                        for t, _ in pending:
                            dist.all_reduce(t, group=group)
                else:
                    for t, g in pending:
                        dist.all_reduce(t, group=g)
        self._keep.clear()

    @property
    def collectives_pending(self):
        return bool(self._allreduce)

    def flushed(self):
        assert self._list.n == 0 and not self._allreduce
        self._keep.clear()

    def discard(self):
        self._list.n = 0
        self._keep.clear()
        self._allreduce = []


def _sum_over_ranks(flat, group, defer):
    if defer is not None:
        defer.allreduce(flat, group)
    else:
        import torch.distributed as dist
        dist.all_reduce(flat, group=group)


class CallContext:
    __slots__ = ("defer", "tail", "pipe", "next_proj", "pre_proj", "hidden_private")

    def __init__(self, defer=None, tail=None, pipe=None):
        self.defer, self.tail, self.pipe = defer, tail, pipe
        self.next_proj = self.pre_proj = None
        self.hidden_private = None

    @classmethod
    def from_ambient(cls):
        a = _ambient()
        return cls(a.defer, a.tail, a.pipe)

    def defer_ptr(self):
        return self.defer.pointer() if self.defer is not None else None


_TLS = threading.local()


def _ambient():
    c = getattr(_TLS, "call", None)
    if c is None:
        c = _TLS.call = CallContext()
    return c


def _call_or_ambient(call):
    return call if call is not None else CallContext.from_ambient()


class TapeBroken(RuntimeError):
    """A step cannot run on a Tape (see there): something other than this package's Functions sits between them."""


class _TapeCtx:

    def __init__(self, needs_input_grad):
        self.needs_input_grad = needs_input_grad
        self.saved_tensors = ()
        self.non_differentiable = ()

    def save_for_backward(self, *tensors):
        self.saved_tensors = tensors

    def mark_non_differentiable(self, *tensors):
        self.non_differentiable = tuple(id(t) for t in tensors)

    def release(self):
        self.__dict__.clear()
        self.saved_tensors = ()

    def set_materialize_grads(self, value):
        pass


class Tape:

    def __init__(self):
        self.records = []
        self.produced = {}
        self.ctx_of = {}

    def run(self, fn, args):
        needs = []
        for a in args:
            if not isinstance(a, torch.Tensor):
                needs.append(False)
            elif id(a) in self.produced:
                needs.append(True)
            elif a.grad_fn is not None:
                raise TapeBroken(f"{fn.__name__}: an argument was computed by torch operations from tensors that need gradients")
            else:
                needs.append(bool(a.requires_grad))
        ctx = _TapeCtx(tuple(needs))
        with torch.no_grad():
            out = fn.forward(ctx, *args)
        outs = out if isinstance(out, tuple) else (out,)
        if not any(needs):
            return out
        for o in outs:
            if isinstance(o, torch.Tensor) and o.is_floating_point() and id(o) not in ctx.non_differentiable:
                o.requires_grad_(True)
                self.ctx_of[id(o)] = ctx
                self.produced[id(o)] = o
        self.records.append((fn, ctx, args, outs))
        return out

    def producer(self, t):
        return self.ctx_of.get(id(t)) if self.produced.get(id(t)) is t else None

    def release(self):
        for _, ctx, _, _ in self.records:
            ctx.release()
        self.records, self.produced, self.ctx_of = [], {}, {}

    def backward(self, out, grad):
        if id(out) not in self.produced:
            raise TapeBroken("the model's output is not the output of one of this package's Functions")
        grads = {id(out): grad}
        try:
            self._backward(grads)
        finally:
            self.release()

    def _backward(self, grads):
        with torch.no_grad():
            for fn, ctx, args, outs in reversed(self.records):
                gouts = tuple(grads.pop(id(o), None) if isinstance(o, torch.Tensor) else None for o in outs)
                if all(g is None for g in gouts):
                    continue
                gins = fn.backward(ctx, *gouts)
                if not isinstance(gins, tuple):
                    gins = (gins,)
                for a, g in zip(args, gins):
                    if g is None or not isinstance(a, torch.Tensor):
                        continue
                    if id(a) in self.produced:
                        grads[id(a)] = g if id(a) not in grads else grads[id(a)] + g
                    elif a.requires_grad:
                        if g.stride() != a.stride():
                            g = g.contiguous()
                        if a.grad is None:
                            a.grad = g
                        else:
                            a.grad.add_(g)


class on_tape:

    def __init__(self, tape):
        self.tape = tape

    def __enter__(self):
        self.prev = _current_tape()
        _TLS.tape = self.tape
        return self.tape

    def __exit__(self, *exc):
        _TLS.tape = self.prev
        return False


def _current_tape():
    return getattr(_TLS, "tape", None)


def _run(fn, *args):
    tape = _current_tape()
    return fn.apply(*args) if tape is None else tape.run(fn, args)


class deferred_reductions:

    def __enter__(self):
        a = _ambient()
        self.prev, self.d = a.defer, DeferredReductions()
        a.defer = self.d
# ... 24 lines not shown


class fused_loss_tail:

    def __init__(self, labels, row_weight):
        self.labels, self.row_weight = labels, row_weight
        self.loss = self.dz = self.out = None

    def __enter__(self):
        a = _ambient()
        self.prev = a.tail
        a.tail = self
        return self

    def __exit__(self, *exc):
        _ambient().tail = self.prev
        return False

    def matches(self, out):
        return self.out is not None and out is not None and out.data_ptr() == self.out.data_ptr() \
            and out.shape == self.out.shape


class input_pipeline:

    def __init__(self, pipe):
        self.pipe = pipe

    def __enter__(self):
        a = _ambient()
        self.prev = a.pipe
        a.pipe = self.pipe
        return self.pipe

    def __exit__(self, *exc):
        _ambient().pipe = self.prev
        return False


class InputPipeline:

    def __init__(self, ops, x, p, state, tag=0):
        self.x_rows = x
        src = ops.x_full if getattr(ops, "sharded", False) else x
        n_tab, n = src.shape[0], x.shape[0]
        self.row_offset = int(getattr(ops, "row_offset", 0)) if getattr(ops, "sharded", False) else 0
        self.ops, self.x, self.p, self.state, self.tag = ops, src, float(p), state, int(tag)
        if n_tab == n:
            both = torch.zeros(2, n, 8, dtype=_F32, device=x.device)
            self.filled = (both[0], both[1])
        else:
            self.filled = (torch.zeros(n_tab, 8, dtype=_F32, device=x.device), torch.zeros(n, 8, dtype=_F32, device=x.device))
        self.saved = torch.zeros(2, n, 8, dtype=_F32, device=x.device)
        self.primed = False
        self._x_version = (src._version, x._version)
        self._host_steps = state.host_steps
        self.next_table_ready = False
        self.next_agg_ready = False
        self.adopted = False

    @staticmethod
    def eligible(model, ops, x):
        from ..graph import FilterOperators
        if tuning.HOST.pipeline <= 0 or not isinstance(ops, FilterOperators) or not isinstance(x, torch.Tensor):
            return False
        if getattr(model, "model_type", None) not in ("acmgcn", "acmgcnp", "acmgcnpp"):
            return False
        if model.model_type == "acmgcnpp":
            lins = getattr(getattr(model, "mlpX", None), "lins", None)
            if lins is None or len(lins) != 1 or lins[0].out_features > 256:
                return False
        gcns = getattr(model, "gcns", None)
        if not gcns or len(gcns) != 2 or not getattr(model, "fused_dropout", False) or getattr(model, "dropout", 0) <= 0:
            return False
        l0 = gcns[0]
        try:
            cfg = l0._config()
            f_in, f = l0.weight_low.shape
        except AttributeError:
            return False
        if cfg.relu_before or f != 64 or not 4 < f_in <= 8 or x.dim() != 2 or x.shape[1] != f_in:
            return False
        if not ops.implicit or getattr(ops, "general", False) or int(getattr(ops, "hops", 1)) != 1:
            return False
        if ops.sharded:
            xf = ops.x_full
            if (not ops.uniform or xf is None or xf.dtype != _F32 or xf.dim() != 2 or xf.shape != (ops.low.n_cols, f_in)
                    or xf.device != x.device or xf.requires_grad):
                return False
        if x.dtype != _F32 or x.device != l0.weight_low.device or x.requires_grad:
            return False
        n, nnz = ops.low.n_rows, ops.low.nnz
        min_rows = tuning.HOST.pipeline
        if n != x.shape[0] or n < max(min_rows, 32) or not 12.0 * n < nnz <= 160.0 * n:
            return False
        if x.device.type == "cuda" and torch.cuda.is_current_stream_capturing():
            return False
        gw = 4
        if not ops.low.build_streams(n_waves=max(gw, min(256 * gw, gw * ((n + 15) // 16)))):
            return False
        return ops.low.stream_waves % gw == 0 and gw <= ops.low.stream_waves <= min(256 * gw, gw * ((n + 15) // 16))

    def table(self):
        return self.filled[0]

    def local_table(self):
        return self.filled[0][self.row_offset:self.row_offset + self.x_rows.shape[0]]

    def agg(self):
        return self.filled[1]

    def _drop_into(self, dst, step_offset):
        d = self.state.spec(self.p, self.tag, 0)
        d.step_offset = int(step_offset)
        n, c = self.x.shape
        launch("acm_dropout", f"dropout/{n}x{c}", self.x.device, n, c, _vp(self.x), self.x.stride(0), _vp(dst), dst.stride(0), 8, C.byref(d))

    def stale(self):
        return (not self.primed or (self.x._version, self.x_rows._version) != self._x_version or self.next_table_ready
                or self.state.host_steps != self._host_steps)

    def prime(self):
        from .ops import spmm
        self._drop_into(self.filled[0], 0)
        spmm(self.ops.low, self.filled[0], out=self.filled[1], row_scale=self.ops.row_scale)
        self.primed = True
        self._x_version = (self.x._version, self.x_rows._version)
        self._host_steps = self.state.host_steps
        self.next_table_ready = self.next_agg_ready = self.adopted = False

    def refill_spec(self, p):
        if self.filled[0].shape[0] != self.x_rows.shape[0] or self.next_table_ready or self.x.stride(1) != 1:
            return False
        d = self.state.spec(self.p, self.tag, 0)
        d.step_offset = 1
        p.next_x, p.ld_next_x, p.next_drop = self.x.data_ptr(), self.x.stride(0), d
        return True

    def make_next(self):
        if not self.adopted:
            return False
        if not self.next_table_ready:
            self._drop_into(self.filled[0], 1)
            self.next_table_ready = True
        return True

    def end_step(self):
        if not (self.next_table_ready and self.next_agg_ready):
            self.primed = False
        self.next_table_ready = self.next_agg_ready = self.adopted = False
        self._host_steps = self.state.host_steps


def _next_proj_request(call, f, dev, row_local_only=False):
    nxt, call.next_proj = call.next_proj, None
    if nxt is None or not row_local_only or not (tuning.kernel()["rows16"] & tuning.ROWS16_EPI):
        return None
    try:
        w3 = (nxt.weight_low, nxt.weight_high, nxt.weight_mlp)
        cfg = nxt._config()
    except AttributeError:
        return None
    f2 = w3[0].shape[1]
    ok = (f2 <= 2 and all(w.dtype == _F32 and w.is_contiguous() and w.device == dev and
                                                   tuple(w.shape) == (f, f2) for w in w3))
    return (w3, bool(cfg.relu_before), f2, cfg.n_channels == 4 and f2 == 2) if ok else None


def _take_pre_proj(call, x, w3, relu):
    pre, call.pre_proj = call.pre_proj, None
    if pre is None or not isinstance(x, torch.Tensor):
        return None
    out, zlh, zi, ptrs, prelu = pre
    if (x.data_ptr() == out.data_ptr() and x.shape == out.shape and x.stride() == out.stride() and prelu == bool(relu)
            and tuple(w.data_ptr() for w in w3) == ptrs):
        return zlh, zi
    return None
```

acm_gnn_amd/functional/conv_literal.py:

```python
import ctypes as C

import torch

from .. import _lib, tuning
from .. import functional as _pkg
from ..graph import SparseFeatures
from ._context import _current_tape, _take_pre_proj
from ._conv_shared import _NO_GRADS, _chan_block, _conv_prologue, _flat_views, _gathered_input, _grads, _head_params, _hop_buffer, \
    _k3_setup, _low_product, _narrow_tables, _pack_head, _reduce_replicated, _set_head, _set_post, _struc_grad, _struc_rows, \
    _unpack_head
from ._launch import _F32, _as_f32c, _capturing, _vp, _workspace, _workspace_bytes, launch
from .ops import _drop_now, _drop_spec, cast_bf16, gemm, gemm_drop_supported, gemm_split, proj3, proj_bwd, proj_bwd_supported, \
    proj_fwd, spmm, spmm_v


def _literal_project(ctx, x, w3, ops, cfg):
    call, hops = ctx.call, ctx.hops
    sparse_x = isinstance(x, SparseFeatures)
    n, dev = x.shape[0], w3[0].device
    f_in, f = w3[0].shape
    four = cfg.n_channels == 4
    use_proj = (not sparse_x and f <= 5 and f_in <= 64
                and w3[0].stride(0) == w3[1].stride(0) == w3[2].stride(0))
    fb = ctx.fb = _chan_block(f)
    ldz = 3 * f
    if f in (2, 4, 8):
        ldz = -(-3 * f // (2 * f)) * (2 * f)
    elif fb != f:
        ldz = -(-(2 * fb + f) // 4) * 4
    pre = _take_pre_proj(call, x, w3, cfg.relu_before) if use_proj else None
    drop_spec = _drop_spec(ctx.in_drop, ops.row_offset) if ctx.in_drop is not None else None
    two_tables = (use_proj or f in (2, 4, 8) or hops > 1) and not sparse_x
    pack4 = four and f == 2 and fb == 2 and two_tables and not ops.sharded and not getattr(ops, "general", False)
    done3 = False
    if pre is None and not sparse_x:
        if two_tables:
            zlh, _ = _narrow_tables(n, fb, f, dev, pack4)
            zi = torch.empty(n, f, dtype=_F32, device=dev)
            done3 = proj3(x, w3, fb, zlh, zi, relu=cfg.relu_before, x_drop=drop_spec)
        else:
            z = torch.empty(n, ldz, dtype=_F32, device=dev)[:, : 2 * fb + f]
            done3 = proj3(x, w3, fb, z, relu=cfg.relu_before, x_drop=drop_spec)
            zlh, zi = z[:, : 2 * fb], z[:, 2 * fb:]
        if done3:
            ctx.in_drop_used = drop_spec is not None
    if (not done3 and drop_spec is not None
            and (pre is not None or use_proj or two_tables or sparse_x or not gemm_drop_supported(n, f_in, 2 * fb + f))):
        if sparse_x:
            raise NotImplementedError("in_drop with CSR features: the caller applies the dropout to the values")
        x, pre = _drop_now(x, drop_spec), None
        drop_spec = None
    if done3:
        pass
    elif pre is not None:
        zlh, zi = pre
    elif use_proj:
        zlh, _ = _narrow_tables(n, fb, f, dev, pack4)
        zi = torch.empty(n, f, dtype=_F32, device=dev)
        proj_fwd(x, w3, zlh, zi, relu=cfg.relu_before, h_col=fb)
    else:
        if fb != f:
            zpad = w3[0].new_zeros(w3[0].shape[0], fb - f)
            wcat = torch.cat((w3[0], zpad, w3[1], zpad, w3[2]), dim=1).contiguous()
        else:
            wcat = torch.cat(w3, dim=1).contiguous()
        if two_tables:
            zlh, _ = _narrow_tables(n, fb, f, dev, pack4)
            zi = torch.empty(n, f, dtype=_F32, device=dev)
            gemm_split(x, wcat, zlh, zi, relu=cfg.relu_before)
        else:
            z = torch.empty(n, ldz, dtype=_F32, device=dev)[:, : 2 * fb + f]
            if sparse_x:
                spmm_v(x.csr, x.values, wcat, relu=cfg.relu_before, out=z)
            else:
                gemm(x, wcat, relu=cfg.relu_before, out=z, a_drop=drop_spec)
                ctx.in_drop_used = drop_spec is not None
            zlh, zi = z[:, : 2 * fb], z[:, 2 * fb:]
    if hops > 2:
        t = zlh[:, :f]
        for hop in range(hops - 1):
            t = _low_product(ops, t, out=zlh[:, :f] if hop == hops - 2 else None)
        zg = _pkg._gather_rows(ops, zlh) if ops.sharded else zlh
    elif hops > 1:
        zc = torch.empty(n, 2 * fb, dtype=_F32, device=dev)
        _low_product(ops, zlh[:, :f], out=zc[:, :f])
        zc[:, fb:fb + f] = zlh[:, fb:fb + f]
        zg = _pkg._gather_rows(ops, zc)
    else:
        zg = _pkg._gather_rows(ops, zlh) if ops.sharded else zlh
    return x, zlh, zi, zg


class _AcmLiteral(torch.autograd.Function):

    @staticmethod
    def forward(ctx, x, w_low, w_high, w_mlp, v_low, v_high, v_mlp, v_struc, struc_low, att_mix, lnw_low, lnw_high, lnw_mlp,
                lnw_struc, lnb_low, lnb_high, lnb_mlp, lnb_struc, ops, cfg, post_relu, post_scale, post_drop, call, tail_layer,
                agg_holder, in_drop, pregathered):
        x = _conv_prologue(ctx, x, w_low, ops, post_relu, post_scale, post_drop, call, in_drop)
        call, post_scale = ctx.call, ctx.post_scale
        sparse_x = isinstance(x, SparseFeatures)
        dev, n = x.device, x.shape[0]
        f_in, f = w_low.shape
        k = cfg.n_channels
        four = k == 4
        general = bool(getattr(ops, "general", False))
        hops = ctx.hops = int(getattr(ops, "hops", 1))
        if hops > 1 and (cfg.relu_before or cfg.relu_after or four or general):
            raise NotImplementedError("hops > 1 is the ACM-SGC chain: model_type 'acmsgc' only")
        if general and ops.sharded:
            raise NotImplementedError("general operator pairs are not row-sharded")
        zero_padded = x.shape[1] != f_in
        if zero_padded:
            x = x[:, :f_in].contiguous()
        w3 = tuple(_as_f32c(t, "weight") for t in (w_low, w_high, w_mlp))
        x, zlh, zi, zg = _literal_project(ctx, x, w3, ops, cfg)
        fb = ctx.fb
        if four and general:
            if ops.un is None:
                raise RuntimeError("structure_info=1 needs adj_low_unnormalized")
            s_local = _as_f32c(struc_low, "struc_low")
        elif four:
            s_local, s_gath = _struc_rows(ops, struc_low, n)
        vecs, lnw, lnb, mix = _head_params(cfg, (v_low, v_high, v_mlp, v_struc), att_mix, (lnw_low, lnw_high, lnw_mlp, lnw_struc),
                                           (lnb_low, lnb_high, lnb_mlp, lnb_struc))
        out = torch.empty(n, f, dtype=_F32, device=dev)
        att = torch.empty(n, 4, dtype=_F32, device=dev)
        pre = torch.empty(n, (k - 1) * f, dtype=_F32, device=dev)
        p = _lib.ConvFwd()
        p.f_out, p.row_offset = f, ops.row_offset
        _set_head(p, cfg, vecs, lnw, lnb, mix)
        if ops.implicit:
            p.row_scale = ops.row_scale.data_ptr()
        graph = ops.low
        if general:
            pl = spmm(ops.low, zlh[:, :f])
            ph = spmm(ops.high, zlh[:, fb:fb + f])
            zero = ops.zeros(n, f)
            graph = ops.eye
            p.g_low, p.ld_g_low = pl.data_ptr(), pl.stride(0)
            p.g_high, p.ld_g_high = zero.data_ptr(), zero.stride(0)
            p.s_high, p.ld_s_high = ph.data_ptr(), ph.stride(0)
            if four:
                ps = spmm(ops.un, s_local)
                ones = ops.zeros(n, 1).new_ones(n)
                p.g_struc, p.ld_g_struc = ps.data_ptr(), ps.stride(0)
                p.s_struc, p.ld_s_struc = zero.data_ptr(), zero.stride(0)
                p.deg = ones.data_ptr()
            keep_alive = (pl, ph, zero) + ((ps, ones) if four else ())
        else:
            if cfg.gather_bf16 and 8 < f <= 64 and f % 2 == 0:
                zb = cast_bf16(zg[:, : 2 * f])
                p.gather_bf16 = 1
                p.g_low, p.ld_g_low = zb.data_ptr(), zb.stride(0)
                p.g_high, p.ld_g_high = zb.data_ptr() + 2 * f, zb.stride(0)
                if four:
                    sb = cast_bf16(s_gath)
                    p.g_struc, p.ld_g_struc = sb.data_ptr(), sb.stride(0)
            else:
                p.g_low, p.ld_g_low = zg.data_ptr(), zg.stride(0)
                p.g_high, p.ld_g_high = zg.data_ptr() + 4 * fb, zg.stride(0)
                if four:
                    p.g_struc, p.ld_g_struc = s_gath.data_ptr(), s_gath.stride(0)
                    if (f == 2 and fb == 2 and zg is zlh and zlh.stride(0) == 8 and zlh.data_ptr() % 32 == 0 and s_gath is s_local
                            and zlh.untyped_storage().nbytes() - zlh.storage_offset() * 4 >= n * 32):
                        torch.as_strided(zlh, (n, 2), (8, 1), zlh.storage_offset() + 4).copy_(s_local)
                        p.g_struc, p.ld_g_struc = zlh.data_ptr() + 16, 8
            p.s_high, p.ld_s_high = zlh.data_ptr() + 4 * fb, zlh.stride(0)
            if four:
                p.s_struc, p.ld_s_struc = s_local.data_ptr(), s_local.stride(0)
                p.deg = ops.deg.data_ptr()
        p.s_mlp, p.ld_s_mlp = zi.data_ptr(), zi.stride(0)
        p.out, p.ld_out = out.data_ptr(), out.stride(0)
        p.pre, p.ld_pre = pre.data_ptr(), pre.stride(0)
        p.att = att.data_ptr()
        _set_post(p, ctx.post_relu, post_scale, ctx.post_drop, ops.row_offset)
        ws = graph.workspace((k - 1) * f)
        tail_req = call.tail
        ctx.tail = None
        st = None
        if (tail_req is not None and tail_req.out is None and tail_layer and not general and k == 3 and f <= 8
                and not cfg.gather_bf16 and not post_relu and post_scale is None and post_drop is None
                and any(ctx.needs_input_grad) and tail_req.labels.numel() == n
                and (graph.n_long_rows == 0 or 12.0 < graph.nnz / max(graph.n_rows, 1) <= 160.0)):
            st = _fwd_tail(ctx, ops, cfg, graph, p, ws, tail_req, w3, pre, zi, vecs, lnw, lnb, mix, out)
        if st != 0:
            launch("acm_conv_fwd", f"conv_fwd/F{f}k{k}", dev, graph.handle, C.byref(p), _vp(ws), ws.numel() * 4)
        ctx.ops, ctx.cfg = ops, cfg
        ctx.sparse_x = x if sparse_x else None
        ctx.lazy_producer = None
        tape = _current_tape()
        prod = (getattr(x, "grad_fn", None) or (tape.producer(x) if tape is not None else None)) if not sparse_x else None
        if (call.hidden_private is x and prod is not None and getattr(prod, "agg_first", False) and getattr(prod, "call", None) is call
                and not zero_padded and hops == 1 and call.defer is not None):
            ctx.lazy_producer = prod
        ctx.save_for_backward(w3[0] if sparse_x else x, *w3, zlh, zi, pre, *_pack_head(vecs, lnw, lnb, mix))
        ctx.mark_non_differentiable(att)
        return out, att

    @staticmethod
    def backward(ctx, grad_out, _grad_att):
        if grad_out is None:
            return _NO_GRADS
        return _literal_backward(ctx, grad_out)


def _fwd_tail(ctx, ops, cfg, graph, p, ws, tail_req, w3, pre, zi, vecs, lnw, lnb, mix, out):
    call = ctx.call
    (n, f), k, dev = out.shape, cfg.n_channels, out.device
    dlog = torch.empty(n, f, dtype=_F32, device=dev)
    st3 = _k3_setup(cfg, ops, k, f, n, dev, w3[0].shape[0], pre, zi, vecs, lnw, lnb, mix, dlog, False, None, None, fb=ctx.fb)
    loss = torch.empty((), dtype=_F32, device=dev)
    lo = _lib.Loss()
    lo.n_classes = f
    y = tail_req.labels.to(torch.int64).contiguous().reshape(-1)
    w_row = _as_f32c(tail_req.row_weight, "row_weight")
    lo.labels, lo.row_weight = y.data_ptr(), w_row.data_ptr()
    lo.loss, lo.dlogits, lo.ld_dlogits = loss.data_ptr(), dlog.data_ptr(), dlog.stride(0)
    q = st3["q"]
    q.defer = call.defer_ptr()
    nbytes = _workspace_bytes("acm_conv_fwd_tail_workspace_bytes", n, f, k, or_none=True)
    if nbytes is None:
        return None
    wt = torch.empty(max(nbytes // 4, 1), dtype=_F32, device=dev)
    st = launch("acm_conv_fwd_tail", f"conv_fwd_tail/F{f}k{k}", dev, graph.handle, C.byref(p), C.byref(lo), C.byref(q), _vp(ws), ws.numel() * 4,
                _vp(wt), nbytes, unsupported_ok=True)
    if st == 0:
        st3["keep"] = (y, w_row, wt)
        ctx.tail = st3
        tail_req.loss, tail_req.dz, tail_req.out = loss, dlog, out
        if call.defer is not None:
            call.defer.hold(wt, [loss, st3["d_mix"], *st3["d_vec"], *st3["d_lnw"], *st3["d_lnb"]], keep=[loss, st3["flat"]])
    return st


def _k3_backward(ctx, grad_out):
    ops, cfg, defer = ctx.ops, ctx.cfg, ctx.call.defer
    k = cfg.n_channels
    saved = ctx.saved_tensors
    x, wl, wh, wm, zlh, zi, pre = saved[:7]
    vecs, lnw, lnb, mix = _unpack_head(saved, cfg, 7)
    dev = zlh.device
    n, f = zlh.shape[0], wl.shape[1]
    grad_out = _as_f32c(grad_out, "grad_out")
    tail = ctx.tail
    done = tail is not None and grad_out.data_ptr() == tail["grad_out"].data_ptr()
    st3 = tail if done else _k3_setup(cfg, ops, k, f, n, dev, wl.shape[0], pre, zi, vecs, lnw, lnb, mix, grad_out,
                                      ctx.post_relu, ctx.post_scale, ctx.post_drop, fb=ctx.fb)
    if done:
        ctx.tail = None
    elif getattr(ctx, "mask_table", None) is not None:
        st3["q"].g_scale = None
    d_vec, d_lnw, d_lnb, d_mix = _flat_views(st3["flat"], st3["nw"], k, f, cfg.layernorm)
    st3.update(d_vec=d_vec, d_lnw=d_lnw, d_lnb=d_lnb, d_mix=d_mix)
    if not done:
        ws = _workspace(dev, "acm_conv_bwd_local_workspace_bytes", n, f, k)
        q = st3["q"]
        q.defer = defer.pointer() if defer is not None else None
        launch("acm_conv_bwd_local", f"conv_bwd_local/F{f}k{k}", dev, n, C.byref(q), _vp(ws), ws.numel() * 4)
        if defer is not None:
            defer.hold(ws, [d_mix, *d_vec, *d_lnw, *d_lnb], keep=[st3["flat"]])
    return x, (wl, wh, wm), zlh, st3


def _literal_backward(ctx, grad_out):
    x, w3, zlh, s = _k3_backward(ctx, grad_out)
    ops, cfg, defer = ctx.ops, ctx.cfg, ctx.call.defer
    g, dz, gs, flat, nw, ones = s["g"], s["dz"], s["gs"], s["flat"], s["nw"], s["ones"]
    k, fb, dev = cfg.n_channels, ctx.fb, dz.device
    four = k == 4
    n, (f_in_w, f) = dz.shape[0], w3[0].shape
    d_struc = torch.empty(n, f, dtype=_F32, device=dev) if four else None
    r = _lib.ConvBwdSpmm()
    r.f_out, r.row_offset = f, ops.row_offset
    if s["general"]:
        t_l = spmm(ops.low.transpose(), g[:, :f])
        t_h = spmm(ops.high.transpose(), g[:, fb:fb + f])
        zero = ops.zeros(n, f)
        low_t = ops.eye
        r.g_low, r.ld_g_low = t_l.data_ptr(), t_l.stride(0)
        r.g_high, r.ld_g_high = zero.data_ptr(), zero.stride(0)
        r.s_high, r.ld_s_high = t_h.data_ptr(), t_h.stride(0)
        if four:
            t_s = spmm(ops.un.transpose(), gs)
            r.g_struc, r.ld_g_struc = t_s.data_ptr(), t_s.stride(0)
            r.s_struc, r.ld_s_struc = zero.data_ptr(), zero.stride(0)
            r.inv_deg = ones.data_ptr()
            r.d_struc, r.ld_d_struc = d_struc.data_ptr(), d_struc.stride(0)
    else:
        gg = _pkg._gather_rows(ops, g)
        gsg = _pkg._gather_rows(ops, gs) if four else None
        low_t = ops.low_t
        if cfg.gather_bf16 and 8 < f <= 64 and f % 2 == 0 and fb == f:
            gb = cast_bf16(gg[:, : 2 * f])
            r.gather_bf16 = 1
            r.g_low, r.ld_g_low = gb.data_ptr(), gb.stride(0)
            r.g_high, r.ld_g_high = gb.data_ptr() + 2 * f, gb.stride(0)
            if four:
                gsg = cast_bf16(gsg)
        else:
            r.g_low, r.ld_g_low = gg.data_ptr(), gg.stride(0)
            r.g_high, r.ld_g_high = gg.data_ptr() + 4 * fb, gg.stride(0)
        r.s_high, r.ld_s_high = g.data_ptr() + 4 * fb, g.stride(0)
        if four:
            r.g_struc, r.ld_g_struc = gsg.data_ptr(), gsg.stride(0)
            r.s_struc, r.ld_s_struc = gs.data_ptr(), gs.stride(0)
            r.inv_deg = None if ops.implicit else ops.inv_deg.data_ptr()
            r.d_struc, r.ld_d_struc = d_struc.data_ptr(), d_struc.stride(0)
        if ops.implicit:
            r.self_scale = ops.self_scale.data_ptr()
    if cfg.relu_before:
        r.mask_low, r.ld_mask_low = zlh.data_ptr(), zlh.stride(0)
        r.mask_high, r.ld_mask_high = zlh.data_ptr() + 4 * fb, zlh.stride(0)
    r.dz_low, r.ld_dz_low = dz.data_ptr(), dz.stride(0)
    r.dz_high, r.ld_dz_high = dz.data_ptr() + 4 * f, dz.stride(0)
    ws2 = low_t.workspace((k - 1) * f)
    launch("acm_conv_bwd_spmm", f"conv_bwd_spmm/F{f}k{k}", dev, low_t.handle, C.byref(r), _vp(ws2), ws2.numel() * 4)
    if ctx.hops > 2 and ops.implicit:
        sc = _hop_buffer(dz, f)
        torch.mul(dz[:, :f], ops.row_scale[:, None], out=sc)
        for hop in range(ctx.hops - 2):
            sc = spmm(ops.low_t, _pkg._gather_rows(ops, sc), out=_hop_buffer(dz, f), row_scale=ops.row_scale)
        spmm(ops.low_t, _pkg._gather_rows(ops, sc), out=dz[:, :f])
    elif ctx.hops > 1:
        t = dz[:, :f]
        last = ctx.hops - 2
        for hop in range(ctx.hops - 1):
            t = _low_product(ops, t, transpose=True, out=dz[:, :f] if (hop == last and hop > 0) else None)
        if last == 0:
            dz[:, :f] = t

    if ctx.sparse_x is not None:
        xs = ctx.sparse_x
        xt = xs.csr_t
        d_wcat = spmm_v(xt, xs.values.index_select(0, xt.src_pos), dz, out=flat[:nw].view(f_in_w, 3 * f))
        d_x = None
    elif (ctx.needs_input_grad[0] and proj_bwd_supported(3 * f)
          and w3[0].stride(0) == w3[1].stride(0) == w3[2].stride(0)):
        d_wcat = flat[:nw].view(3, f_in_w, f)
        prod = getattr(ctx, "lazy_producer", None)
        if (prod is not None and f <= 2 and f_in_w == 64 and x.shape[1] == 64 and getattr(prod, "lazy", None) is None
                and all(w.stride(0) == f and w.is_contiguous() for w in w3)):
            d_x = torch.empty(n, x.shape[1], dtype=_F32, device=dev)
            prod.lazy = dict(dz=dz, w3=w3, d_w=d_wcat, x=x, placeholder=d_x)
        else:
            d_x = proj_bwd(x, dz, w3, d_wcat, defer=defer)
    else:
        d_wcat = gemm(x, dz, trans_a=True, col_blocks=3,
                      out=flat[:nw].view(3, f_in_w, f),
                      a_drop=_drop_spec(ctx.in_drop, ops.row_offset) if getattr(ctx, "in_drop_used", False) else None)
        d_x = gemm(dz, torch.cat(w3, dim=1), trans_b=True) if ctx.needs_input_grad[0] else None
    if d_x is not None and d_x.shape[1] != ctx.x_width:
        d_x = torch.nn.functional.pad(d_x, (0, ctx.x_width - d_x.shape[1]))
    _reduce_replicated(flat, ops, defer)
    if d_wcat.dim() == 3:
        d_w3 = (d_wcat[0], d_wcat[1], d_wcat[2])
    else:
        d_w3 = tuple(d_wcat[:, i * f:(i + 1) * f] for i in range(3))
    return _grads(d_x, d_w3, s["d_vec"], d_struc, s["d_mix"], s["d_lnw"], s["d_lnb"])


class _AcmAcmii(torch.autograd.Function):

    @staticmethod
    def forward(ctx, x, w_low, w_high, w_mlp, v_low, v_high, v_mlp, v_struc, struc_low, att_mix, lnw_low, lnw_high, lnw_mlp,
                lnw_struc, lnb_low, lnb_high, lnb_mlp, lnb_struc, ops, cfg, post_relu, post_scale, post_drop, call, tail_layer,
                agg_holder, in_drop, pregathered):
        x = _conv_prologue(ctx, x, w_low, ops, post_relu, post_scale, post_drop, call, in_drop)
        dev, n = x.device, x.shape[0]
        f_in, f = w_low.shape
        k = cfg.n_channels
        four = k == 4
        fp = 8
        zero_padded = x.shape[1] != f_in
        x, xpad, xg, _, _ = _gathered_input(ctx, x, ops, f_in, f, fp, agg_holder, pregathered, False)
        w3 = wl, wh, wm = tuple(_as_f32c(t, "weight") for t in (w_low, w_high, w_mlp))
        x = x[:, :f_in].contiguous() if zero_padded else x
        if four:
            s_local, s_gath = _struc_rows(ops, struc_low, n)
        vecs, lnw, lnb, mix = _head_params(cfg, (v_low, v_high, v_mlp, v_struc), att_mix, (lnw_low, lnw_high, lnw_mlp, lnw_struc),
                                           (lnb_low, lnb_high, lnb_mlp, lnb_struc))
        out = torch.empty(n, f, dtype=_F32, device=dev)
        att = torch.empty(n, 4, dtype=_F32, device=dev)
        zlh = torch.empty(n, 2 * f, dtype=_F32, device=dev)
        zi = torch.empty(n, f, dtype=_F32, device=dev)
        pre = torch.empty(n, (k - 1) * f, dtype=_F32, device=dev)
        p = _lib.ConvAcmiiFwd()
        p.f_in, p.f_pad, p.f_out = f_in, fp, f
        _set_head(p, cfg, vecs, lnw, lnb, mix)
        if four:
            ps = spmm(ops.low, s_gath, row_scale=ops.row_scale if ops.implicit else None, bf16=cfg.gather_bf16)
            p.ps, p.ld_ps = ps.data_ptr(), ps.stride(0)
            p.ss, p.ld_ss = s_local.data_ptr(), s_local.stride(0)
            p.deg = ops.deg.data_ptr()
        p.xg, p.ld_xg = xg.data_ptr(), xg.stride(0)
        p.xs, p.ld_xs = xpad.data_ptr(), xpad.stride(0)
        p.w_low, p.w_high, p.w_mlp, p.ld_w = wl.data_ptr(), wh.data_ptr(), wm.data_ptr(), f
        p.out, p.ld_out = out.data_ptr(), out.stride(0)
        p.pre, p.ld_pre = pre.data_ptr(), pre.stride(0)
        p.att = att.data_ptr()
        p.zlh, p.ld_zlh = zlh.data_ptr(), zlh.stride(0)
# ... 66 lines not shown
```

acm_gnn_amd/graph.py:

```python
import ctypes as C
import weakref

import torch

from . import _lib


_raw_stream = getattr(torch._C, "_cuda_getCurrentRawStream", None)


def _stream():
    if _raw_stream is not None:
        return C.c_void_p(_raw_stream(torch.cuda.current_device()))
    return C.c_void_p(torch.cuda.current_stream().cuda_stream)


class _NoSwitch:
    def __enter__(self):
        return None

    def __exit__(self, *a):
        return False


_NO_SWITCH = _NoSwitch()


def _device_ctx(dev):
    idx = dev.index if isinstance(dev, torch.device) else torch.device(dev).index
    if idx is None or idx == torch.cuda.current_device():
        return _NO_SWITCH
    return torch.cuda.device(dev)


def _sync(dev):
    torch.cuda.synchronize(dev)


def _copy_from_ptr(ptr, n, dtype, device):
    t = torch.empty(n, dtype=dtype, device=device)
    if n:
        C.cdll.LoadLibrary("libamdhip64.so").hipMemcpy(
            C.c_void_p(t.data_ptr()), C.c_void_p(ptr), C.c_size_t(n * t.element_size()), 3)
    return t


def _require_cuda(t, name):
    if not t.is_cuda:
        raise RuntimeError(
            f"acm_gnn_amd: {name} is on {t.device}; the ACM operators run only on an AMD GPU "
            "(there is no CPU fallback)")


class CsrGraph:

    def __init__(self, handle, device):
        self._h = C.c_void_p(handle)
        self.device = device
        info = _lib.CsrInfo()
        _lib.check(_lib.load().acm_csr_info(self._h, C.byref(info)), "acm_csr_info")
        self.n_rows, self.n_cols, self.nnz = info.n_rows, info.n_cols, info.nnz
        self.n_items, self.n_long_rows = info.n_items, info.n_long_rows
        self.n_partial_slots, self.chunk, self.max_degree = info.n_partial_slots, info.chunk, info.max_degree
        self._ptrs = (info.indptr, info.indices, info.vals)
        self._src_pos_ptr = info.src_pos
        self._src_pos = None
        self._transposed = None
        self.stream_steps, self.stream_waves = info.stream_steps, info.stream_waves
        self.stream_slices, self.stream_long_rows = info.stream_slices, info.stream_long_rows
        self._finalizer = weakref.finalize(self, _lib.load().acm_csr_destroy, C.c_void_p(handle))

    @classmethod
    def from_csr(cls, indptr, indices, vals, n_cols, chunk=0):
        _require_cuda(indptr, "indptr")
        indptr = indptr.to(torch.int32).contiguous()
        indices = indices.to(device=indptr.device, dtype=torch.int32).contiguous()
        n_rows, nnz = indptr.numel() - 1, indices.numel()
        if vals is not None:
            vals = vals.to(device=indptr.device, dtype=torch.float32).contiguous()
            if vals.numel() != nnz:
                raise ValueError(f"vals has {vals.numel()} entries, indices {nnz}")
        out = C.c_void_p()
        with _device_ctx(indptr.device):
            _sync(indptr.device)
            st = _lib.load().acm_csr_create(n_rows, int(n_cols), nnz, indptr.data_ptr(),
                                            indices.data_ptr() if nnz else None,
                                            vals.data_ptr() if (nnz and vals is not None) else None, int(chunk),
                                            C.byref(out))
        _lib.check(st, "acm_csr_create")
        return cls(out.value, indptr.device)

    @classmethod
    def from_torch(cls, adj, chunk=0):
        _require_cuda(adj, "adjacency")
        if adj.layout == torch.sparse_csr:
            return cls.from_csr(adj.crow_indices(), adj.col_indices(), adj.values(), adj.shape[1], chunk)
        if adj.layout == torch.strided:
            adj = adj.to_sparse()
        if adj.layout != torch.sparse_coo:
            raise TypeError(f"unsupported adjacency layout {adj.layout}")
        adj = adj.coalesce()
        idx, vals = adj.indices(), adj.values().to(torch.float32)
        n_rows, n_cols = adj.shape
        counts = torch.bincount(idx[0], minlength=n_rows)
        indptr = torch.zeros(n_rows + 1, dtype=torch.int64, device=adj.device)
        indptr[1:] = torch.cumsum(counts, 0)
        return cls.from_csr(indptr.to(torch.int32), idx[1].to(torch.int32), vals, n_cols, chunk)

    @classmethod
    def from_scipy(cls, mat, device, chunk=0):
        m = mat.tocsr()
        m.sort_indices()
        dev = torch.device(device)
        return cls.from_csr(torch.from_numpy(m.indptr.astype("int32")).to(dev),
                            torch.from_numpy(m.indices.astype("int32")).to(dev),
                            torch.from_numpy(m.data.astype("float32")).to(dev), m.shape[1], chunk)

    def build_streams(self, n_waves=0, lmax=0):
        if self.stream_steps:
            return True
        if self._ptrs[2]:
            return False
        with _device_ctx(self.device):
            _sync(self.device)
            st = _lib.load().acm_csr_build_streams(self._h, int(n_waves), int(lmax))
        _lib.check(st, "acm_csr_build_streams")
        info = _lib.CsrInfo()
        _lib.check(_lib.load().acm_csr_info(self._h, C.byref(info)), "acm_csr_info")
        self.stream_steps, self.stream_waves = info.stream_steps, info.stream_waves
        self.stream_slices, self.stream_long_rows = info.stream_slices, info.stream_long_rows
        return True

    def build_item_streams(self, n_waves=0):
        if getattr(self, "item_stream_waves", 0):
            return True
        if self._ptrs[2] or self.nnz == 0:
            return False
        with _device_ctx(self.device):
            _sync(self.device)
            st = _lib.load().acm_csr_build_item_streams(self._h, int(n_waves))
        if st == 4:
            return False
        _lib.check(st, "acm_csr_build_item_streams")
        info = _lib.CsrInfo()
        _lib.check(_lib.load().acm_csr_info(self._h, C.byref(info)), "acm_csr_info")
        self.item_stream_waves = info.item_stream_waves
        return self.item_stream_waves > 0

    def transpose(self):
        if self._transposed is None:
            out = C.c_void_p()
            with _device_ctx(self.device):
                _lib.check(_lib.load().acm_csr_transpose(self._h, 0, C.byref(out)), "acm_csr_transpose")
            self._transposed = CsrGraph(out.value, self.device)
        return self._transposed

    def slice_rows(self, begin, end):
        out = C.c_void_p()
        with _device_ctx(self.device):
            _lib.check(_lib.load().acm_csr_slice_rows(self._h, int(begin), int(end), 0, C.byref(out)),
                       "acm_csr_slice_rows")
        return CsrGraph(out.value, self.device)

    def arrays(self):
        _sync(self.device)
        return (_copy_from_ptr(self._ptrs[0], self.n_rows + 1, torch.int32, self.device),
                _copy_from_ptr(self._ptrs[1], self.nnz, torch.int32, self.device),
                _copy_from_ptr(self._ptrs[2], self.nnz, torch.float32, self.device) if self._ptrs[2] or not self.nnz
                else None)

    @property
    def pattern_only(self):
        return self.nnz > 0 and not self._ptrs[2]

    @property
    def src_pos(self):
        if self._src_pos is None:
            if not self._src_pos_ptr:
                raise RuntimeError("src_pos exists only on handles made by transpose()")
            _sync(self.device)
            self._src_pos = _copy_from_ptr(self._src_pos_ptr, self.nnz, torch.int32, self.device).to(torch.int64)
        return self._src_pos

    def workspace(self, width):
        nbytes = C.c_size_t()
        _lib.check(_lib.load().acm_spmm_workspace_bytes(self._h, int(width), C.byref(nbytes)),
                   "acm_spmm_workspace_bytes")
        n = max(nbytes.value // 4, 1)
        return torch.empty(n, dtype=torch.float32, device=self.device)

    @property
    def handle(self):
        return self._h

    def __repr__(self):
        return (f"CsrGraph({self.n_rows}x{self.n_cols}, nnz={self.nnz}, items={self.n_items}, "
                f"long_rows={self.n_long_rows}, max_degree={self.max_degree})")


class SparseFeatures:

    def __init__(self, csr, values):
        self.csr, self.values = csr, values
        self.shape = (csr.n_rows, csr.n_cols)
        self.device = csr.device

    @classmethod
    def from_scipy(cls, mat, device):
        m = mat.tocsr()
        m.sort_indices()
        csr = CsrGraph.from_scipy(m, device)
        return cls(csr, torch.from_numpy(m.data.astype("float32")).to(torch.device(device)))

    @classmethod
    def from_torch(cls, x):
        csr = CsrGraph.from_torch(x if x.layout != torch.strided else x.to_sparse())
        return cls(csr, csr.arrays()[2])

    @classmethod
    def auto(cls, x, min_cols=None):
        if min_cols is None:
            from . import tuning
            min_cols = tuning.HOST.csr_features
        if (min_cols <= 0 or not isinstance(x, torch.Tensor) or x.layout != torch.strided or x.dim() != 2
                or x.dtype != torch.float32 or x.requires_grad or x.shape[1] < min_cols or x.shape[0] == 0):
            return x
        try:
            _require_cuda(x, "features")
        except RuntimeError:
            return x
        memo = getattr(x, "_acm_csr_twin", None)
        if memo is not None and memo[0] == x._version:
            return x if memo[1] is None else memo[1]
        if x.is_cuda and torch.cuda.is_current_stream_capturing():
            return x
        twin = None
        if int(torch.count_nonzero(x)) * 16 <= x.numel():
            twin = cls.from_torch(x.detach())
        x._acm_csr_twin = (x._version, twin)
        return x if twin is None else twin

    @staticmethod
    def known_twin(x):
        memo = getattr(x, "_acm_csr_twin", None) if isinstance(x, torch.Tensor) else None
        return memo[1] if (memo is not None and memo[0] == x._version) else None

    def twin_of_masked(self, x):
        if tuple(x.shape) != tuple(self.shape) or not x.is_contiguous():
            return None
        flat = getattr(self, "_flat_index", None)
        if flat is None:
            ip, ix, _ = self.csr.arrays()
            ip = ip.to(torch.int64)
            rows = torch.repeat_interleave(torch.arange(self.shape[0], device=ip.device), ip[1:] - ip[:-1])
            flat = self._flat_index = rows * self.shape[1] + ix.to(torch.int64)
        vals = x.reshape(-1).index_select(0, flat)
        if flat.numel() < (1 << 24):
            same = bool(torch.linalg.vector_norm(x, 0) == torch.linalg.vector_norm(vals, 0))
        else:
            same = int(torch.count_nonzero(x) - torch.count_nonzero(vals)) == 0
        if not same:
            return None
        out = self.with_values(vals)
        out._flat_index = flat
        return out

    def with_values(self, values):
        if values.shape != self.values.shape:
            raise ValueError("values must keep the CSR order and length")
        out = SparseFeatures(self.csr, values)
        out._perm_cache = getattr(self, "_perm_cache", None)
        return out

    def permute_rows(self, perm):
        cache = getattr(self, "_perm_cache", None)
        if cache is None or cache[0] != perm.data_ptr():
            ip, ix, _ = self.csr.arrays()
            ip = ip.to(torch.int64)
            counts = (ip[1:] - ip[:-1]).index_select(0, perm)
            new_ip = torch.zeros(perm.numel() + 1, dtype=torch.int64, device=ip.device)
            new_ip[1:] = torch.cumsum(counts, 0)
            start = ip[:-1].index_select(0, perm)
            pos = torch.repeat_interleave(start - new_ip[:-1], counts) + torch.arange(int(new_ip[-1]), device=ip.device)
            csr = CsrGraph.from_csr(new_ip.to(torch.int32), ix.index_select(0, pos), None, self.csr.n_cols)
            cache = (perm.data_ptr(), csr, pos)
            self._perm_cache = cache
        out = SparseFeatures(cache[1], self.values.index_select(0, cache[2]))
        return out

    @property
    def csr_t(self):
        return self.csr.transpose()


class FilterOperators:

    def __init__(self, low, deg=None, row_offset=0, n_global=None, group=None, row_scale=None):
        self.low = low
        self._low_t = None
        self.row_scale = row_scale
        self.self_scale = (1.0 / row_scale) if row_scale is not None else None
        self.deg = deg
        self.inv_deg = (1.0 / deg) if deg is not None else None
        self.row_offset = int(row_offset)
        self.n_global = int(n_global if n_global is not None else low.n_cols)
        self.group = group
        self.plan = None
        self.perm = None
        self.inv_perm = None
        self.low_t_override = None
        self.x_full = None
        self._pregathered = None
        self.hops = 1
        self.general = False
        self.high = None
# ... 285 lines not shown
```

acm_gnn_amd/train.py:

```python
import torch
import torch.nn.functional as F

from . import functional as AF
from .graph import FilterOperators, SparseFeatures, operators_for

_TORCH_DROPOUT = F.dropout


def row_weights(train_idx, n_rows, n_train_total=None, device=None):
    device = device if device is not None else train_idx.device
    w = torch.zeros(n_rows, dtype=torch.float32, device=device)
    total = n_train_total if n_train_total is not None else train_idx.numel()
    w[train_idx.to(device)] = 1.0 / float(total)
    return w


def _tape_safe(model):
    from .models import GCN
    return type(model) is GCN and model.model_type in ("acmgcn", "acmgcnp", "acmsgc")


def _rng_snapshot(device):
    dev = torch.device(device)
    cuda = torch.cuda.get_rng_state(dev) if (dev.type == "cuda" and not torch.cuda.is_current_stream_capturing()) else None
    return torch.get_rng_state(), cuda, dev


def _rng_restore(snap):
    if snap is None:
        return
    cpu, cuda, dev = snap
    torch.set_rng_state(cpu)
    if cuda is not None:
        torch.cuda.set_rng_state(cuda, dev)


def _held_entries(model):
    held = []
    for m in model.modules():
        entries = getattr(m, "held_entries", None)
        if entries is not None:
            held.extend(entries())
    return held


def _capture_mode():
    import torch.distributed as dist
    if dist.is_available() and dist.is_initialized():
        return {"capture_error_mode": "thread_local"}
    return {}


class TrainStep:
    def __init__(self, model, optimizer, x, adj, labels, weights, adj_high=None, adj_un=None, use_graph=False,
                 fused_dropout=None, pipeline_input=None, steps_per_graph=1, flush_in_optimizer=True, small_step=None, tape=True):
        self.model, self.opt = model, optimizer
        self.steps_per_call = max(int(steps_per_graph), 1) if use_graph else 1
        self.losses = []
        self.x, self.adj, self.adj_high, self.adj_un = x, adj, adj_high, adj_un
        self.labels, self.weights = labels, weights
        self._permuted = False
        ops = adj
        if not isinstance(adj, FilterOperators) and isinstance(adj, torch.Tensor) and hasattr(model, "structure_info"):
            four = model.structure_info and getattr(model, "model_type", "") in ("acmgcnp", "acmgcnpp")
            ops = operators_for(adj, adj_high, adj_un if four else None)
            self.adj = ops
        if hasattr(model, "auto_csr"):
            self.x = x = model.auto_csr(x, ops if isinstance(ops, FilterOperators) else None)
        if isinstance(ops, FilterOperators) and ops.perm is not None and hasattr(model, "_forward"):
            self.adj = ops
            self.x = x.permute_rows(ops.perm) if isinstance(x, SparseFeatures) else x.index_select(0, ops.perm)
            self.labels, self.weights = labels.index_select(0, ops.perm), weights.index_select(0, ops.perm)
            self._permuted = True
        self.graph, self.loss = None, None
        self._held = None
        self._manual_advance = False
        self._defer = True
        self._tape = bool(tape)
        self._tape_proven = False
        if self._tape and F.dropout is not _TORCH_DROPOUT and getattr(model, "dropout", 0) > 0 and not _tape_safe(model):
            self._tape = False
        from .optim import _FusedAdamBase
        self._opt_flushes = bool(flush_in_optimizer) and isinstance(optimizer, _FusedAdamBase)
        self._unflushed = None
        if fused_dropout is None:
            fused_dropout = F.dropout is _TORCH_DROPOUT
        if fused_dropout and getattr(model, "dropout", 0) > 0 and hasattr(model, "fused_dropout"):
            model.fused_dropout = True
            if model.dropout_state is None:
                model.dropout_state = AF.DropoutState(labels.device)
            if hasattr(optimizer, "also_advance"):
                optimizer.also_advance = model.dropout_state.step
            else:
                self._manual_advance = True
        self._params = list(model.parameters())
        import inspect
        try:
            self._takes_call = "call" in inspect.signature(model.forward).parameters
        except (TypeError, ValueError):
            self._takes_call = False
        self.pipe = None
        if pipeline_input is not False and not self._manual_advance and getattr(model, "fused_dropout", False) \
                and AF.InputPipeline.eligible(model, self.adj, self.x):
            self.pipe = AF.InputPipeline(self.adj, self.x, model.dropout, model.dropout_state, tag=0)
        self.small, self.small_refused = None, "not requested"
        if small_step is not False:
            from .small import SmallPlan
            why = "the loop advances the dropout counter by hand" if self._manual_advance else \
                SmallPlan.why_not(model, self.x, self.adj, optimizer)
            if why is None and getattr(model, "dropout", 0) > 0 and not getattr(model, "fused_dropout", False):
                why = "F.dropout masks (counter-based dropout only)"
            self.small_refused = why
            if why is None:
                self.small = SmallPlan(model, self.x, self.adj, self.labels, self.weights, optimizer)
                self.pipe = None
        if use_graph:
            self._capture()

    def _one_step(self):
        if self.small is not None:
            loss = self.small.run()
        else:
            loss = self._forward_backward(for_optimizer=True)
            self._opt_step()
        self._count_advance()
        if self.pipe is not None:
            self.pipe.end_step()
        return loss

    def _forward_backward(self, for_optimizer=False):
        pipe = self.pipe
        if pipe is not None and pipe.stale():
            if self.x.is_cuda and torch.cuda.is_current_stream_capturing():
                self.pipe = pipe = None
            else:
                pipe.prime()
        pending = AF.DeferredReductions() if self._defer else None
        call = AF.CallContext(defer=pending, pipe=pipe)
        tape = AF.Tape() if (self._tape and not (torch.cuda.is_available() and torch.cuda.is_current_stream_capturing())) else None
        rng = _rng_snapshot(self.labels.device) if (tape is not None and not self._tape_proven) else None
        try:
            with AF.on_tape(tape):
                loss, dz, out = self._forward_loss(call)
            if pipe is not None:
                pipe.make_next()
            if tape is not None:
                tape.backward(out, dz)
                self._tape_proven = True
            else:
                out.backward(dz)
        except (AF.TapeBroken, RuntimeError) as err:
            if tape is not None:
                tape.release()
            if pending is not None:
                pending.discard()
            broken = tape is not None and not self._tape_proven and (isinstance(err, AF.TapeBroken) or "leaf Variable" in str(err))
            if not broken:
                raise
            self._tape = False
            _rng_restore(rng)
            self.opt.zero_grad(set_to_none=True)
            if pipe is not None:
                pipe.primed = False
            return self._forward_backward(for_optimizer)
        except BaseException:
            if tape is not None:
                tape.release()
            if pending is not None:
                pending.discard()
            raise
        if pending is None:
            return loss
        adopted = pending.all_adopted([loss] + [p.grad for p in self._params])
        self._unflushed = None
        if for_optimizer and adopted and self._opt_flushes and not pending.collectives_pending:
            self._unflushed = pending
            return loss
        pending.flush()
        if not adopted:
            self._defer = False
            self.opt.zero_grad(set_to_none=True)
            if pipe is not None:
                pipe.primed = False
            return self._forward_backward(for_optimizer)
        return loss

    def _forward_loss(self, call):
        tail = call.tail = AF.fused_loss_tail(self.labels, self.weights)
        kw = {"call": call} if self._takes_call else {}
        if self._permuted:
            kw["rows_permuted"] = True
        if self._takes_call:
            out = self.model(self.x, self.adj, self.adj_high, self.adj_un, **kw)
        else:
            with AF.deferred_reductions_as(call.defer), AF.input_pipeline(call.pipe), tail:
                out = self.model(self.x, self.adj, self.adj_high, self.adj_un, **kw)
        call.tail = None
        if tail.matches(out):
            return tail.loss, tail.dz, out
        loss, dz = AF.nll_loss_and_grad(out, self.labels, self.weights, defer=call.defer)
        return loss, dz, out

    def _eager(self):
        if not self.model.training:
            self.model.train()
        if type(self.opt).zero_grad is torch.optim.Optimizer.zero_grad:
            for group in self.opt.param_groups:
                for p in group["params"]:
                    p.grad = None
        else:
            self.opt.zero_grad(set_to_none=True)
        loss = self._one_step()
        return loss

    def _snapshot(self):
        model_state = [(t, t.detach().clone()) for t in self.model.state_dict().values() if torch.is_tensor(t)]
        opt_state = [(p, {k: (v.detach().clone() if torch.is_tensor(v) else v) for k, v in st.items()})
                     for p, st in self.opt.state.items()]
        ds = getattr(self.model, "dropout_state", None)
        return model_state, opt_state, ((ds.step.clone(), ds.host_steps) if ds is not None else None)

    def _restore(self, snap):
        model_state, opt_state, drop_step = snap
        with torch.no_grad():
            for t, v in model_state:
                t.copy_(v)
            had = {id(p): st for p, st in opt_state}
            for p, st in self.opt.state.items():
                old = had.get(id(p))
                for k, v in st.items():
                    if not torch.is_tensor(v):
                        if old is not None and k in old:
                            st[k] = old[k]
                        continue
                    if old is not None and k in old:
                        v.copy_(old[k])
                    else:
                        v.zero_()
            if drop_step is not None:
                self.model.dropout_state.step.copy_(drop_step[0])
                self.model.dropout_state.host_steps = drop_step[1]
        if getattr(self, "pipe", None) is not None:
            self.pipe.primed = False

    def _capture(self):
        snap = self._snapshot()
        side = torch.cuda.Stream()
        side.wait_stream(torch.cuda.current_stream())
        with torch.cuda.stream(side):
            for _ in range(3):
                self._eager()
        torch.cuda.current_stream().wait_stream(side)
        torch.cuda.synchronize()
        self._restore(snap)
        if self.pipe is not None:
            self.pipe.prime()
            torch.cuda.synchronize()
        self.graph = torch.cuda.CUDAGraph()
        self.model.train()
        self.opt.zero_grad(set_to_none=True)
        losses = []
        with torch.cuda.graph(self.graph, **_capture_mode()):
            for k in range(self.steps_per_call):
                if k:
                    self.opt.zero_grad(set_to_none=True)
                loss = self._one_step()
                if self.small is not None and self.steps_per_call > 1:
                    loss = loss.clone()
                losses.append(loss)
            self.loss, self.losses = loss, losses
        del loss, losses
        self._held = _held_entries(self.model)

    def refresh(self):
        if self.graph is not None:
            self.graph = None
            if self.pipe is not None:
                self.pipe.primed = False
            self._capture()

    def _opt_step(self):
        pending, self._unflushed = self._unflushed, None
        if pending is not None:
            self.opt.step(pending=pending)
        else:
            self.opt.step()

    def _count_advance(self):
        ds = getattr(self.model, "dropout_state", None)
        if self._manual_advance:
            ds.advance()
# ... 197 lines not shown
```

acm_gnn_amd/tuning.py:

```python
import contextlib
import ctypes as C
import os
import threading

KERNEL_KEYS = ("chunk", "wide_form", "bwd_split", "rows16", "agg_fused", "gemm_forms")
HOST_DEFAULTS = {"rewrites": 15, "implicit": 1, "relabel": -1, "pipeline": 8192, "csr_features": 256, "small_step": 16384}
HOST_RANGES = {"rewrites": (0, 15), "implicit": (0, 1), "relabel": (-1, 1), "pipeline": (0, 1 << 31), "csr_features": (0, 1 << 31),
               "small_step": (0, 16384)}

REWRITE_AGG_FIRST = 1
REWRITE_ACMII_RECOMPUTE = 2
REWRITE_ACMII_MASK = 4
REWRITE_AGGW_FUSED = 8
ROWS16_EPI, ROWS16_BWD, ROWS16_LOCAL = 1, 2, 4
GEMM_ROWS, GEMM_BX3, GEMM_BX3_WIDE, GEMM_ROWS_ALWAYS = 1, 2, 4, 8


class Tuning(C.Structure):
    _fields_ = [(k, C.c_int32) for k in KERNEL_KEYS] + [("reserved", C.c_int32 * 10)]


class _Host:
    __slots__ = tuple(HOST_DEFAULTS)

    def __init__(self, **kw):
        for k, v in HOST_DEFAULTS.items():
            setattr(self, k, int(kw.get(k, v)))

    def as_dict(self):
        return {k: getattr(self, k) for k in HOST_DEFAULTS}


def parse(text):
    kern, host = {}, {}
    for item in (text or "").split(","):
        item = item.strip()
        if not item:
            continue
        key, sep, val = item.partition("=")
        if not sep:
            raise ValueError(f"ACM_TUNING: '{item}' is not key=value")
        try:
            v = int(val, 0)
        except ValueError:
            raise ValueError(f"ACM_TUNING: '{item}': the value must be an integer") from None
        if key in KERNEL_KEYS:
            kern[key] = v
        elif key in HOST_DEFAULTS:
            lo, hi = HOST_RANGES[key]
            if not lo <= v <= hi:
                raise ValueError(f"ACM_TUNING: {key}={v} outside {lo}..{hi}")
            host[key] = v
        else:
            raise ValueError(f"ACM_TUNING: unknown key '{key}' (known: {', '.join(KERNEL_KEYS + tuple(HOST_DEFAULTS))})")
    return kern, host


def parse_lenient(text, report=None):
    import sys
    report = report or (lambda msg: sys.stderr.write(f"acm_gnn_amd: {msg} (ignored)\n"))
    kern, host = {}, {}
    for item in (text or "").split(","):
        if not item.strip():
            continue
        try:
            k, h = parse(item)
        except ValueError as exc:
            report(str(exc))
            continue
        kern.update(k)
        host.update(h)
    return kern, host


LEGACY_ENV = ("ACM_GATHER_DTYPE", "ACM_EVAL_AGG_CACHE", "ACM_CHUNK", "ACM_WIDE_FORM", "ACM_BWD_SPLIT", "ACM_AGG_FUSED", "ACM_PIPELINE",
              "ACM_IMPLICIT", "ACM_RELABEL", "ACM_REWRITES", "ACM_ROWS16", "ACM_GEMM_FORMS")


def _report_legacy(environ, report=None):
    import sys
    report = report or (lambda msg: sys.stderr.write(f"acm_gnn_amd: {msg}\n"))
    found = [k for k in LEGACY_ENV if k in environ]
    if found:
        report(f"{', '.join(found)}: environment switches of earlier rounds are no longer read; use ACM_TUNING=\"key=value,...\"")
    return found


_LOADED_HOST = parse_lenient(os.environ.get("ACM_TUNING", ""))[1]
_report_legacy(os.environ)
HOST = _Host(**_LOADED_HOST)
_lock = threading.RLock()
_kernel_cache = None
_kernel_touched = False


def kernel():
    global _kernel_cache
    if _kernel_cache is None:
        from . import _lib
        t = Tuning()
        _lib.check(_lib.load().acm_tuning_get(C.byref(t)), "acm_tuning_get")
        _kernel_cache = {k: int(getattr(t, k)) for k in KERNEL_KEYS}
    return _kernel_cache


def set_kernel(**kw):
    global _kernel_cache, _kernel_touched
    from . import _lib
    with _lock:
        _kernel_touched = True
        cur = dict(kernel())
        for k, v in kw.items():
            if k not in KERNEL_KEYS:
                raise KeyError(k)
            cur[k] = int(v)
        t = Tuning()
        for k, v in cur.items():
            setattr(t, k, v)
        _lib.check(_lib.load().acm_tuning_set(C.byref(t)), "acm_tuning_set")
        _kernel_cache = None


def apply(**kw):
    host_kw = {k: v for k, v in kw.items() if k in HOST_DEFAULTS}
    kern_kw = {k: v for k, v in kw.items() if k in KERNEL_KEYS}
    unknown = set(kw) - set(host_kw) - set(kern_kw)
    if unknown:
        raise KeyError(f"unknown tuning switch(es): {sorted(unknown)}")
    for k, v in host_kw.items():
        lo, hi = HOST_RANGES[k]
        if not lo <= int(v) <= hi:
            raise ValueError(f"{k}={v} outside {lo}..{hi}")
    with _lock:
        for k, v in host_kw.items():
            setattr(HOST, k, int(v))
        if kern_kw:
            set_kernel(**kern_kw)


def reset(kernel_too=True):
    global _kernel_cache, _kernel_touched
    with _lock:
        for k, v in HOST_DEFAULTS.items():
            setattr(HOST, k, int(_LOADED_HOST.get(k, v)))
        if kernel_too and _kernel_touched:
            from . import _lib
            _lib.check(_lib.load().acm_tuning_set(None), "acm_tuning_set")
            _kernel_touched = False
        _kernel_cache = None


def invalidate():
    global _kernel_cache
    _kernel_cache = None


def gemm_forms():
    return kernel()["gemm_forms"]


@contextlib.contextmanager
# ... 35 lines not shown
```

include/acm_hip.h:

```cpp
#ifndef ACM_HIP_H
#define ACM_HIP_H

#include <stddef.h>
#include <stdint.h>

#ifdef __cplusplus
extern "C" {
#endif

#define ACM_ABI_VERSION 28

typedef enum {
    ACM_OK = 0,
    ACM_EINVAL = 1,
    ACM_ESHAPE = 2,
    ACM_EHIP = 3,
    ACM_EUNSUPPORTED = 4,
    ACM_ENOMEM = 5,
} acm_status_t;

typedef struct acm_csr acm_csr_t;
typedef void* acm_stream_t;

int acm_version(void);
const char* acm_last_error(void);

typedef struct {
    int32_t chunk;
    int32_t wide_form;
    int32_t bwd_split;
    int32_t rows16;
    int32_t agg_fused;
    int32_t gemm_forms;
    int32_t reserved[10];
} acm_tuning_t;
int acm_tuning_get(acm_tuning_t* out);
int acm_tuning_set(const acm_tuning_t* in);

int acm_csr_create(int64_t n_rows, int64_t n_cols, int64_t nnz,
                   const int32_t* indptr_dev, const int32_t* indices_dev,
                   const float* vals_dev, int chunk, acm_csr_t** out);
int acm_csr_transpose(const acm_csr_t* a, int chunk, acm_csr_t** out);
int acm_csr_slice_rows(const acm_csr_t* a, int64_t row_begin, int64_t row_end,
                       int chunk, acm_csr_t** out);
void acm_csr_destroy(acm_csr_t* a);

int acm_shard_plan(int64_t n_rows, const int64_t* indptr_host, int world, int64_t row_cost,
                   int64_t* bounds_host);

typedef struct {
    int64_t n_rows, n_cols, nnz;
    int64_t n_items;
    int64_t n_long_rows;
    int64_t n_partial_slots;
    int32_t chunk;
    int32_t max_degree;
    const int32_t* indptr;
    const int32_t* indices;
    const float* vals;
    const int32_t* src_pos;
    int64_t stream_steps;
    int64_t stream_slices;
    int32_t stream_waves;
    int32_t stream_long_rows;
    int32_t item_stream_waves;
    int32_t reserved;
    int64_t item_stream_batches;
} acm_csr_info_t;
int acm_csr_info(const acm_csr_t* a, acm_csr_info_t* info);

int acm_csr_build_streams(acm_csr_t* a, int n_waves, int lmax);

int acm_csr_build_item_streams(acm_csr_t* a, int n_waves);

int acm_spmm_workspace_bytes(const acm_csr_t* a, int width, size_t* bytes);

int acm_gemm_workspace_bytes(int transA, int transB, int64_t M, int64_t N, int64_t K,
                             size_t* bytes);
int acm_gemm(int transA, int transB, int64_t M, int64_t N, int64_t K,
             const float* A, int64_t lda, const float* B, int64_t ldb,
             float* C, int64_t ldc, int relu, void* workspace, size_t workspace_bytes,
             acm_stream_t stream);

int acm_gemm_blocks(int transA, int transB, int64_t M, int64_t N, int64_t K,
                    const float* A, int64_t lda, const float* B, int64_t ldb,
                    float* C, int64_t ldc, int64_t c_col_block, int64_t c_block_stride, int relu,
                    void* workspace, size_t workspace_bytes, acm_stream_t stream);

typedef struct {
    float    p;
    int32_t  tag;
    uint64_t seed;
    const int64_t* step;
    int64_t  row_offset;
    int64_t  step_offset;
} acm_dropout_t;

int acm_dropout(int64_t n_rows, int64_t n_cols, const float* src, int64_t ld_src,
                float* dst, int64_t ld_dst, int64_t dst_cols, const acm_dropout_t* d, acm_stream_t stream);

int acm_gemm_drop(int transA, int transB, int64_t M, int64_t N, int64_t K,
                  const float* A, int64_t lda, const float* B, int64_t ldb,
                  float* C, int64_t ldc, int64_t c_col_block, int64_t c_block_stride, int relu,
                  const acm_dropout_t* a_drop, void* workspace, size_t workspace_bytes, acm_stream_t stream);

int acm_proj3(int64_t n_rows, int64_t K, const float* X, int64_t ldx,
              const float* w_low, const float* w_high, const float* w_mlp, int64_t ld_w, int64_t f, int64_t f_block,
              float* C, int64_t ldc, int64_t split_col, float* C2, int64_t ldc2, int relu,
              const acm_dropout_t* x_drop, acm_stream_t stream);

typedef struct {
    const float* partial;
    int32_t nblk, row_stride;
    int32_t q0, len;
    float*  dst;
    int32_t inner;
    int32_t col_block;
    int64_t outer_stride, block_stride;
    int32_t elem_stride;
    int32_t reserved;
} acm_reduce_seg_t;

typedef struct {
    int32_t n, cap;
    acm_reduce_seg_t* segs;
} acm_reduce_list_t;

int acm_reduce_flush(acm_reduce_list_t* list, acm_stream_t stream);

int acm_gemm_split(int transA, int transB, int64_t M, int64_t N, int64_t K,
                   const float* A, int64_t lda, const float* B, int64_t ldb,
                   float* C, int64_t ldc, int64_t split_col, float* C2, int64_t ldc2, int relu,
                   void* workspace, size_t workspace_bytes, acm_stream_t stream);

int acm_proj_fwd(int64_t n_rows, int64_t f_in, int f_out, const float* X, int64_t ldx,
                 const float* w_low, const float* w_high, const float* w_mlp, int64_t ldw, int relu,
                 float* Z_lh, int64_t ld_lh, float* Z_i, int64_t ld_i, acm_stream_t stream);
int acm_proj_fwd_at(int64_t n_rows, int64_t f_in, int f_out, const float* X, int64_t ldx,
                    const float* w_low, const float* w_high, const float* w_mlp, int64_t ldw, int relu,
                    float* Z_lh, int64_t ld_lh, int64_t h_col, float* Z_i, int64_t ld_i, acm_stream_t stream);
int acm_proj_bwd_workspace_bytes(int64_t n_rows, int64_t f_in, int n_out, size_t* bytes);
int acm_proj_bwd(int64_t n_rows, int64_t f_in, int n_out, const float* X, int64_t ldx,
                 const float* dZ, int64_t lddz, const float* w_low, const float* w_high, const float* w_mlp, int64_t ldw,
                 float* dX, int64_t lddx, float* dW, int64_t lddw, int64_t dw_col_block, int64_t dw_block_stride,
                 void* workspace, size_t workspace_bytes, acm_reduce_list_t* defer, acm_stream_t stream);

int acm_linear_fwd(int64_t n_rows, int64_t f_in, int64_t f_out, const float* X, int64_t ldx,
                   const float* W, int64_t ldw, const float* bias, int relu, const acm_dropout_t* drop,
                   float* Y, int64_t ldy, void* workspace, size_t workspace_bytes, acm_stream_t stream);
int acm_bias_act(int64_t n_rows, int f, float* Y, int64_t ldy, const float* bias, int relu,
                 const acm_dropout_t* drop, acm_stream_t stream);
int acm_bias_act_bwd_workspace_bytes(int64_t n_rows, int f, size_t* bytes);
int acm_bias_act_bwd(int64_t n_rows, int f, const float* Y, int64_t ldy, const float* dY, int64_t lddy,
                     float keep_scale, int relu, float* G, int64_t ldg, float* d_bias,
                     void* workspace, size_t workspace_bytes, acm_reduce_list_t* defer, acm_stream_t stream);
int acm_linear_bwd_workspace_bytes(int64_t n_rows, int f_in, int f_out, size_t* bytes);
int acm_linear_bwd(int64_t n_rows, int f_in, int f_out, const float* X, int64_t ldx, const float* Y, int64_t ldy,
                   const float* dY, int64_t lddy, float keep_scale, int relu, float* dW, int64_t lddw, float* d_bias,
                   void* workspace, size_t workspace_bytes, acm_reduce_list_t* defer, acm_stream_t stream);
int acm_linear_fwd_add(int64_t n_rows, int f_in, int f_out, const float* X, int64_t ldx, const float* W, int64_t ldw,
                       const float* bias, int relu, const acm_dropout_t* drop, const float* add, int64_t ld_add,
                       float* Y, int64_t ldy, acm_stream_t stream);
int acm_linear_bwd_recompute(int64_t n_rows, int f_in, int f_out, const float* X, int64_t ldx, const float* W, int64_t ldw,
                             const float* bias, int relu, const acm_dropout_t* drop, const float* dY, int64_t lddy,
                             float* dW, int64_t lddw, float* d_bias, void* workspace, size_t workspace_bytes,
                             acm_reduce_list_t* defer, acm_stream_t stream);

int acm_spmm(const acm_csr_t* a, const float* G, int64_t ldg, int width,
             float* Y, int64_t ldy, void* workspace, size_t workspace_bytes,
             acm_stream_t stream);

int acm_spmm_v(const acm_csr_t* a, const float* vals, const float* G, int64_t ldg, int width,
               float* Y, int64_t ldy, int relu, void* workspace, size_t workspace_bytes,
               acm_stream_t stream);

typedef struct {
    const float* vals;
    const float* row_scale;
    const float* sub; int64_t ld_sub;
    const float* sub_scale;
    int32_t relu;
    int32_t g_bf16;
} acm_spmm_opts_t;

int acm_spmm_ex(const acm_csr_t* a, const void* G, int64_t ldg, int width, float* Y, int64_t ldy,
                const acm_spmm_opts_t* opts, void* workspace, size_t workspace_bytes, acm_stream_t stream);

int acm_cast_bf16(int64_t n_rows, int64_t n_cols, const float* src, int64_t ld_src,
                  uint16_t* dst, int64_t ld_dst, acm_stream_t stream);

typedef struct {
    int32_t f_out;
    int32_t n_channels;
    int32_t relu_after;
    int32_t relu_mlp;
    int32_t layernorm;
    float   scale;
// ... 315 lines not shown
```

Measured before the change: 49.91 billion edges/s.

## Restrict output-layer aggregation to rows carrying loss weight

```diff
diff --git a/acm_gnn_amd/_lib.py b/acm_gnn_amd/_lib.py
--- a/acm_gnn_amd/_lib.py
+++ b/acm_gnn_amd/_lib.py
@@ -9,7 +9,7 @@
 
 ACM_OK = 0
 STATUS_NAMES = {1: "ACM_EINVAL", 2: "ACM_ESHAPE", 3: "ACM_EHIP", 4: "ACM_EUNSUPPORTED", 5: "ACM_ENOMEM"}
-ABI_VERSION = 28
+ABI_VERSION = 29
 
 EXPORTED_SYMBOLS = (
     "acm_version", "acm_last_error", "acm_tuning_get", "acm_tuning_set", "acm_csr_create", "acm_csr_transpose", "acm_csr_slice_rows",
@@ -22,7 +22,7 @@
     "acm_acmii_table_bytes", "acm_acmii_table", "acm_conv_acmii_v_fwd", "acm_conv_acmii_v_bwd_workspace_bytes", "acm_conv_acmii_v_bwd",
     "acm_linear_bwd_workspace_bytes", "acm_linear_bwd", "acm_linear_fwd_add", "acm_linear_bwd_recompute",
     "acm_small_step_workspace_bytes", "acm_small_step", "acm_conv_head_fwd", "acm_conv_aggw_fwd", "acm_conv_aggw_bwd_workspace_bytes", "acm_conv_aggw_bwd",
-    "acm_eval_metrics_workspace_bytes", "acm_eval_metrics",
+    "acm_eval_metrics_workspace_bytes", "acm_eval_metrics", "acm_csr_select_rows",
 )
 
 
@@ -229,6 +229,7 @@
     lib.acm_csr_create.argtypes = [i64, i64, i64, vp, vp, vp, i32, C.POINTER(vp)]
     lib.acm_csr_transpose.argtypes = [vp, i32, C.POINTER(vp)]
     lib.acm_csr_slice_rows.argtypes = [vp, i64, i64, i32, C.POINTER(vp)]
+    lib.acm_csr_select_rows.argtypes = [vp, vp, C.POINTER(vp)]
     lib.acm_csr_destroy.argtypes = [vp]
     lib.acm_csr_destroy.restype = None
     lib.acm_csr_info.argtypes = [vp, C.POINTER(CsrInfo)]
diff --git a/acm_gnn_amd/csrc/acm_common.h b/acm_gnn_amd/csrc/acm_common.h
--- a/acm_gnn_amd/csrc/acm_common.h
+++ b/acm_gnn_amd/csrc/acm_common.h
@@ -90,7 +90,13 @@
     AcmStreams* streams;
     AcmItemStreams* item_streams;
     int device;
-};
+    int32_t origin;
+    int32_t borrows_ids;
+};
+#define ACM_ORIGIN_CREATED 0
+#define ACM_ORIGIN_TRANSPOSED 1
+#define ACM_ORIGIN_SLICED 2
+#define ACM_ORIGIN_ROWS 3
 
 struct StreamView {
     const int32_t* ids;
diff --git a/acm_gnn_amd/csrc/acm_conv.hip b/acm_gnn_amd/csrc/acm_conv.hip
--- a/acm_gnn_amd/csrc/acm_conv.hip
+++ b/acm_gnn_amd/csrc/acm_conv.hip
@@ -238,7 +238,7 @@
 template <int FP, int NG>
 __global__ __launch_bounds__(256) void conv_tail_rows_kernel(acm_conv_fwd_t pf, acm_loss_t pl, acm_conv_bwd_local_t pb,
                                                              int n_rows, float* __restrict__ loss_partial,
-                                                             float* __restrict__ k3_partial) {
+                                                             float* __restrict__ k3_partial, int marked_rows_only) {
     extern __shared__ float lds[];
     __shared__ float red[256];
     constexpr int K = NG + 1;
@@ -250,7 +250,19 @@
     ParamAcc<LaySerial<FP>> pa;
     pa.zero();
     float term = 0.f;
-    if (active) {
+    if (active && marked_rows_only && pl.row_weight[row] == 0.f) {
+        float* pr = pf.pre + (long)row * pf.ld_pre;
+        for (int f = 0; f < F; ++f) {
+            pf.out[(long)row * pf.ld_out + f] = 0.f;
+            pl.dlogits[(long)row * pl.ld_dlogits + f] = 0.f;
+            pb.g_low[(long)row * pb.ld_g_low + f] = 0.f;
+            pb.g_high[(long)row * pb.ld_g_high + f] = 0.f;
+            pb.g_mlp[(long)row * pb.ld_g_mlp + f] = 0.f;
+#pragma unroll
+            for (int c = 0; c < NG; ++c) pr[c * F + f] = 0.f;
+        }
+        *reinterpret_cast<float4*>(pf.att + (long)row * 4) = make_float4(0.f, 0.f, 0.f, 0.f);
+    } else if (active) {
         float acc[NG][FP];
         const float* pr = pf.pre + (long)row * pf.ld_pre;
 #pragma unroll
@@ -349,6 +361,9 @@
                 "acm_conv_fwd_tail: post-ops / bf16 operands are not part of the fused tail");
     ACM_REQUIRE(a->n_long == 0 || narrow_finishes_long_rows(a), ACM_EUNSUPPORTED,
                 "acm_conv_fwd_tail: this graph's narrow gather leaves partial sums of long rows");
+    const int marked_rows_only = a->origin == ACM_ORIGIN_ROWS;
+    ACM_REQUIRE(!marked_rows_only || F <= 4, ACM_EUNSUPPORTED,
+                "acm_conv_fwd_tail: a row-selected operator needs f_out <= 4 (the thread-per-row tail)");
     ACM_REQUIRE(p->g_low && p->g_high && p->s_high && p->s_mlp && p->out && p->pre && p->att && p->att_mix &&
                     l->labels && l->row_weight && l->loss && l->dlogits && b->att_mix && b->g_low && b->g_high &&
                     b->g_mlp && b->d_att_mix, ACM_EINVAL, "acm_conv_fwd_tail: NULL tensor pointer");
@@ -380,7 +395,7 @@
             hipLaunchKernelGGL((conv_tail_packed8_kernel<2>), dim3(nblk), dim3(256), lds, s, *p, *l, *b, n, loss_partial, k3_partial);
         else
             hipLaunchKernelGGL((conv_tail_rows_kernel<decltype(fp)::value, 2>), dim3(nblk), dim3(256), lds, s, *p, *l, *b, n, loss_partial,
-                               k3_partial);
+                               k3_partial, marked_rows_only);
     });
     ACM_CHECK_HIP(hipGetLastError());
     const acm_reduce_seg_t seg = {loss_partial, nblk, 1, 0, 1, l->loss, 1, 0, 0, 0};
diff --git a/acm_gnn_amd/csrc/acm_csr.cpp b/acm_gnn_amd/csrc/acm_csr.cpp
--- a/acm_gnn_amd/csrc/acm_csr.cpp
+++ b/acm_gnn_amd/csrc/acm_csr.cpp
@@ -32,7 +32,7 @@
 const TuningField kTuningFields[] = {{"chunk", &acm_tuning_t::chunk},           {"wide_form", &acm_tuning_t::wide_form},
                                      {"bwd_split", &acm_tuning_t::bwd_split},   {"rows16", &acm_tuning_t::rows16},
                                      {"agg_fused", &acm_tuning_t::agg_fused},   {"gemm_forms", &acm_tuning_t::gemm_forms}};
-const char* const kHostKeys[] = {"rewrites", "implicit", "relabel", "pipeline", "csr_features", "small_step"};
+const char* const kHostKeys[] = {"rewrites", "implicit", "relabel", "pipeline", "csr_features", "small_step", "restrict"};
 
 const char* tuning_invalid(const acm_tuning_t& t) {
     if (t.chunk != 0 && (t.chunk < 8 || t.chunk > 4096 || (t.chunk & (t.chunk - 1)))) return "chunk";
@@ -117,8 +117,8 @@
 
 void free_handle(acm_csr* a) {
     if (!a) return;
-    if (a->indptr) (void)hipFree(a->indptr);
-    if (a->indices) (void)hipFree(a->indices);
+    if (a->indptr && !a->borrows_ids) (void)hipFree(a->indptr);
+    if (a->indices && !a->borrows_ids) (void)hipFree(a->indices);
     if (a->vals) (void)hipFree(a->vals);
     if (a->long_index) (void)hipFree(a->long_index);
     if (a->src_pos) (void)hipFree(a->src_pos);
@@ -130,7 +130,8 @@
 }
 
 void build_items(const std::vector<int32_t>& indptr, int chunk, std::vector<AcmItem>& items,
-                 std::vector<AcmLongRow>& longs, int64_t& n_slots, int32_t& max_deg, int64_t& n_windows, int64_t& n_multi) {
+                 std::vector<AcmLongRow>& longs, int64_t& n_slots, int32_t& max_deg, int64_t& n_windows, int64_t& n_multi,
+                 const uint8_t* keep = nullptr) {
     const int64_t n = (int64_t)indptr.size() - 1;
     items.clear();
     longs.clear();
@@ -139,6 +140,7 @@
     max_deg = 0;
     n_multi = 0;
     for (int64_t r = 0; r < n; ++r) {
+        if (keep && !keep[r]) continue;
         const int32_t b = indptr[r], e = indptr[r + 1];
         const int32_t deg = e - b;
         max_deg = std::max(max_deg, deg);
@@ -175,17 +177,17 @@
     }
     n_windows = (int64_t)items.size() / ACM_WINDOW;
     for (int64_t r = 0; r < n; ++r)
-        if (indptr[r + 1] - indptr[r] <= chunk) items.push_back({(int32_t)r, indptr[r], indptr[r + 1], -1});
-}
-
-int finish_handle(acm_csr* a, const std::vector<int32_t>& h_indptr, int chunk) {
+        if (indptr[r + 1] - indptr[r] <= chunk && !(keep && !keep[r])) items.push_back({(int32_t)r, indptr[r], indptr[r + 1], -1});
+}
+
+int finish_handle(acm_csr* a, const std::vector<int32_t>& h_indptr, int chunk, const uint8_t* keep = nullptr) {
     const int env_chunk = acm_tuning().chunk;
     int auto_chunk = ACM_MIN_CHUNK;
     while (auto_chunk < ACM_MAX_CHUNK && 2 * (int64_t)auto_chunk <= a->nnz / ACM_GROUPS_IN_FLIGHT) auto_chunk *= 2;
     a->chunk = chunk > 0 ? chunk : (env_chunk > 0 ? env_chunk : auto_chunk);
     std::vector<AcmItem> items;
     std::vector<AcmLongRow> longs;
-    build_items(h_indptr, a->chunk, items, longs, a->n_slots, a->max_degree, a->n_windows, a->n_multi);
+    build_items(h_indptr, a->chunk, items, longs, a->n_slots, a->max_degree, a->n_windows, a->n_multi, keep);
     a->n_items = (int64_t)items.size();
     a->n_long = (int64_t)longs.size();
     if (a->n_items) {
@@ -284,6 +286,7 @@
 extern "C" int acm_csr_transpose(const acm_csr_t* a, int chunk, acm_csr_t** out) {
     ACM_REQUIRE(a && out, ACM_EINVAL, "acm_csr_transpose: NULL argument");
     *out = nullptr;
+    ACM_REQUIRE(a->origin < ACM_ORIGIN_ROWS, ACM_EINVAL, "acm_csr_transpose: a row-selected operator (acm_csr_select_rows)");
     ACM_CHECK_HIP(hipDeviceSynchronize());
     const int64_t n = a->n_rows, m = a->n_cols, nnz = a->nnz;
     std::vector<int32_t> ip((size_t)n + 1), ix((size_t)nnz);
@@ -307,6 +310,7 @@
         }
     acm_csr* t = new_handle(m, n, nnz);
     ACM_REQUIRE(t, ACM_ENOMEM, "acm_csr_transpose: host allocation failed");
+    t->origin = ACM_ORIGIN_TRANSPOSED;
     int st = alloc_arrays(t, a->vals != nullptr);
     if (st == ACM_OK) {
         hipError_t e = hipMemcpy(t->indptr, tp.data(), tp.size() * sizeof(int32_t), hipMemcpyHostToDevice);
@@ -335,6 +339,7 @@
                                   acm_csr_t** out) {
     ACM_REQUIRE(a && out, ACM_EINVAL, "acm_csr_slice_rows: NULL argument");
     *out = nullptr;
+    ACM_REQUIRE(a->origin < ACM_ORIGIN_ROWS, ACM_EINVAL, "acm_csr_slice_rows: a row-selected operator (acm_csr_select_rows)");
     ACM_REQUIRE(0 <= row_begin && row_begin <= row_end && row_end <= a->n_rows, ACM_ESHAPE,
                 "acm_csr_slice_rows: bad range [%lld,%lld) of %lld rows", (long long)row_begin,
                 (long long)row_end, (long long)a->n_rows);
@@ -348,6 +353,7 @@
     const int64_t nnz = ip[n];
     acm_csr* s = new_handle(n, a->n_cols, nnz);
     ACM_REQUIRE(s, ACM_ENOMEM, "acm_csr_slice_rows: host allocation failed");
+    s->origin = ACM_ORIGIN_SLICED;
     int st = alloc_arrays(s, a->vals != nullptr);
     if (st == ACM_OK) {
         hipError_t e = hipMemcpy(s->indptr, ip.data(), ip.size() * sizeof(int32_t), hipMemcpyHostToDevice);
@@ -361,6 +367,34 @@
         }
     }
     if (st == ACM_OK) st = finish_handle(s, ip, chunk);
+    if (st != ACM_OK) {
+        free_handle(s);
+        return st;
+    }
+    *out = s;
+    return ACM_OK;
+}
+
+extern "C" int acm_csr_select_rows(const acm_csr_t* a, const uint8_t* row_mask_dev, acm_csr_t** out) {
+    ACM_REQUIRE(a && row_mask_dev && out, ACM_EINVAL, "acm_csr_select_rows: NULL argument");
+    *out = nullptr;
+    ACM_REQUIRE(a->vals == nullptr, ACM_EINVAL, "acm_csr_select_rows: explicit-value operators are not restricted (pattern-only handles only)");
+    ACM_REQUIRE(a->origin == ACM_ORIGIN_CREATED, ACM_EINVAL,
+                "acm_csr_select_rows: the parent must come from acm_csr_create (not transposed, sliced or restricted itself)");
+    int st;
+    ACM_CHECK_HIP(hipDeviceSynchronize());
+    const int64_t n = a->n_rows;
+    std::vector<int32_t> ip((size_t)n + 1);
+    std::vector<uint8_t> keep((size_t)std::max<int64_t>(n, 1), 0);
+    ACM_CHECK_HIP(hipMemcpy(ip.data(), a->indptr, ip.size() * sizeof(int32_t), hipMemcpyDeviceToHost));
+    if (n) ACM_CHECK_HIP(hipMemcpy(keep.data(), row_mask_dev, (size_t)n, hipMemcpyDeviceToHost));
+    acm_csr* s = new_handle(n, a->n_cols, a->nnz);
+    ACM_REQUIRE(s, ACM_ENOMEM, "acm_csr_select_rows: host allocation failed");
+    s->origin = ACM_ORIGIN_ROWS;
+    s->borrows_ids = 1;
+    s->indptr = a->indptr;
+    s->indices = a->indices;
+    st = finish_handle(s, ip, a->chunk, keep.data());
     if (st != ACM_OK) {
         free_handle(s);
         return st;
@@ -411,6 +445,7 @@
     ACM_REQUIRE(a, ACM_EINVAL, "acm_csr_build_streams: NULL handle");
     if (a->streams) return ACM_OK;
     ACM_REQUIRE(a->vals == nullptr, ACM_EUNSUPPORTED, "acm_csr_build_streams: pattern-only operators only");
+    ACM_REQUIRE(a->origin < ACM_ORIGIN_ROWS, ACM_EUNSUPPORTED, "acm_csr_build_streams: a row-selected operator");
     ACM_REQUIRE(a->n_cols < ACM_STREAM_SENTINEL, ACM_EUNSUPPORTED, "acm_csr_build_streams: %lld columns", (long long)a->n_cols);
     if (lmax <= 0) lmax = 512;
     ACM_REQUIRE(lmax % 32 == 0 && lmax <= 4096, ACM_EINVAL, "acm_csr_build_streams: lmax %d must be a multiple of 32, at most 4096", lmax);
@@ -551,6 +586,7 @@
     ACM_REQUIRE(a, ACM_EINVAL, "acm_csr_build_item_streams: NULL handle");
     if (a->item_streams) return ACM_OK;
     ACM_REQUIRE(a->vals == nullptr, ACM_EUNSUPPORTED, "acm_csr_build_item_streams: pattern-only operators only");
+    ACM_REQUIRE(a->origin < ACM_ORIGIN_ROWS, ACM_EUNSUPPORTED, "acm_csr_build_item_streams: a row-selected operator");
     ACM_REQUIRE(a->n_items > 0 && a->nnz > 0, ACM_EUNSUPPORTED, "acm_csr_build_item_streams: empty operator");
     ACM_REQUIRE(a->n_cols < ((int64_t)1 << 31) - 1, ACM_EUNSUPPORTED, "acm_csr_build_item_streams: %lld columns", (long long)a->n_cols);
     ACM_CHECK_HIP(hipDeviceSynchronize());
diff --git a/acm_gnn_amd/functional/__init__.py b/acm_gnn_amd/functional/__init__.py
--- a/acm_gnn_amd/functional/__init__.py
+++ b/acm_gnn_amd/functional/__init__.py
@@ -1,7 +1,7 @@
 from .. import _lib, tuning
 from ..graph import CsrGraph, FilterOperators, SparseFeatures, _device_ctx, _require_cuda, _stream
 from ._launch import KernelTimer, _Timed, set_kernel_timer
-from ._context import (CallContext, DeferredReductions, InputPipeline, Tape, TapeBroken, _ambient,
+from ._context import (CallContext, DeferredReductions, InputPipeline, RestrictedOutput, Tape, TapeBroken, _ambient,
                        deferred_reductions, deferred_reductions_as, fused_loss_tail, input_pipeline, on_tape)
 from .ops import (DropoutState, _drop_spec, agg_pad_width, cast_bf16, dropout, eval_metrics, eval_metrics_buffers,
                   gemm, gemm_drop_supported, gemm_split, masked_nll, mm, nll_loss_and_grad, proj3, proj_bwd,
diff --git a/acm_gnn_amd/functional/_context.py b/acm_gnn_amd/functional/_context.py
--- a/acm_gnn_amd/functional/_context.py
+++ b/acm_gnn_amd/functional/_context.py
@@ -83,10 +83,10 @@
 
 
 class CallContext:
-    __slots__ = ("defer", "tail", "pipe", "next_proj", "pre_proj", "hidden_private")
-
-    def __init__(self, defer=None, tail=None, pipe=None):
-        self.defer, self.tail, self.pipe = defer, tail, pipe
+    __slots__ = ("defer", "tail", "pipe", "restrict", "next_proj", "pre_proj", "hidden_private")
+
+    def __init__(self, defer=None, tail=None, pipe=None, restrict=None):
+        self.defer, self.tail, self.pipe, self.restrict = defer, tail, pipe, restrict
         self.next_proj = self.pre_proj = None
         self.hidden_private = None
 
@@ -417,6 +417,49 @@
         self._host_steps = self.state.host_steps
 
 
+class RestrictedOutput:
+
+    def __init__(self, ops, weights):
+        self.parent, self.weights = ops.low, weights
+        self._version = weights._version
+        self.used = 0
+        mask = (weights != 0).to(torch.uint8).contiguous()
+        self.n_marked = int(mask.sum())
+        self.rows = ops.low.select_rows(mask)
+
+    @staticmethod
+    def why_not(model, ops, weights):
+        from ..graph import FilterOperators
+        if tuning.HOST.restrict <= 0:
+            return "switched off (ACM_TUNING restrict=0)"
+        if not isinstance(ops, FilterOperators) or not ops.implicit or ops.sharded or getattr(ops, "general", False) \
+                or int(getattr(ops, "hops", 1)) != 1 or ops.low_t is not ops.low:
+            return "needs one device's pattern-only 1-hop operator"
+        lib = _lib.load()
+        if not hasattr(lib, "acm_csr_select_rows"):
+            return "the loaded library has no restricted operators"
+        if not isinstance(weights, torch.Tensor) or weights.dtype != _F32 or weights.dim() != 1 or not weights.is_contiguous() \
+                or weights.numel() != ops.low.n_rows or ops.low.n_rows != ops.low.n_cols or weights.device != torch.device(ops.low.device):
+            return "row weights are not a contiguous float32 vector over the operator's rows"
+        try:
+            last = model.gcns[-1]
+            if last.weight_low.shape[1] > 4 or last._config().n_channels != 3:
+                return "the output layer does not take the thread-per-row loss tail"
+        except (AttributeError, IndexError, TypeError):
+            return "the model's output layer is not known"
+        if weights.is_cuda and torch.cuda.is_current_stream_capturing():
+            return "operators cannot be built inside a capture"
+        if bool((weights != 0).all()):
+            return "every row carries weight"
+        return None
+
+    def stale(self):
+        return self.weights._version != self._version
+
+    def matches(self, graph, row_weight):
+        return graph is self.parent and row_weight is self.weights and not self.stale()
+
+
 def _next_proj_request(call, f, dev, row_local_only=False):
     nxt, call.next_proj = call.next_proj, None
     if nxt is None or not row_local_only or not (tuning.kernel()["rows16"] & tuning.ROWS16_EPI):
diff --git a/acm_gnn_amd/functional/conv_literal.py b/acm_gnn_amd/functional/conv_literal.py
--- a/acm_gnn_amd/functional/conv_literal.py
+++ b/acm_gnn_amd/functional/conv_literal.py
@@ -9,7 +9,7 @@
 from ._conv_shared import _NO_GRADS, _chan_block, _conv_prologue, _flat_views, _gathered_input, _grads, _head_params, _hop_buffer, \
     _k3_setup, _low_product, _narrow_tables, _pack_head, _reduce_replicated, _set_head, _set_post, _struc_grad, _struc_rows, \
     _unpack_head
-from ._launch import _F32, _as_f32c, _capturing, _vp, _workspace, _workspace_bytes, launch
+from ._launch import EUNSUPPORTED, _F32, _as_f32c, _capturing, _vp, _workspace, _workspace_bytes, launch
 from .ops import _drop_now, _drop_spec, cast_bf16, gemm, gemm_drop_supported, gemm_split, proj3, proj_bwd, proj_bwd_supported, \
     proj_fwd, spmm, spmm_v
 
@@ -178,6 +178,7 @@
         ws = graph.workspace((k - 1) * f)
         tail_req = call.tail
         ctx.tail = None
+        ctx.row_selected = False
         st = None
         if (tail_req is not None and tail_req.out is None and tail_layer and not general and k == 3 and f <= 8
                 and not cfg.gather_bf16 and not post_relu and post_scale is None and post_drop is None
@@ -223,8 +224,18 @@
     if nbytes is None:
         return None
     wt = torch.empty(max(nbytes // 4, 1), dtype=_F32, device=dev)
-    st = launch("acm_conv_fwd_tail", f"conv_fwd_tail/F{f}k{k}", dev, graph.handle, C.byref(p), C.byref(lo), C.byref(q), _vp(ws), ws.numel() * 4,
-                _vp(wt), nbytes, unsupported_ok=True)
+    restrict = call.restrict
+    st = EUNSUPPORTED
+    if restrict is not None and f <= 4 and restrict.matches(graph, tail_req.row_weight):
+        wr = restrict.rows.workspace((k - 1) * f)
+        st = launch("acm_conv_fwd_tail", f"conv_fwd_tail/F{f}k{k}", dev, restrict.rows.handle, C.byref(p), C.byref(lo), C.byref(q), _vp(wr),
+                    wr.numel() * 4, _vp(wt), nbytes, unsupported_ok=True)
+        if st == 0:
+            ctx.row_selected = True
+            restrict.used += 1
+    if st == EUNSUPPORTED:
+        st = launch("acm_conv_fwd_tail", f"conv_fwd_tail/F{f}k{k}", dev, graph.handle, C.byref(p), C.byref(lo), C.byref(q), _vp(ws),
+                    ws.numel() * 4, _vp(wt), nbytes, unsupported_ok=True)
     if st == 0:
         st3["keep"] = (y, w_row, wt)
         ctx.tail = st3
@@ -247,6 +258,8 @@
     done = tail is not None and grad_out.data_ptr() == tail["grad_out"].data_ptr()
     st3 = tail if done else _k3_setup(cfg, ops, k, f, n, dev, wl.shape[0], pre, zi, vecs, lnw, lnb, mix, grad_out,
                                       ctx.post_relu, ctx.post_scale, ctx.post_drop, fb=ctx.fb)
+    if not done and getattr(ctx, "row_selected", False):
+        raise RuntimeError("acm_conv: a forward over the row-selected operator takes the fused loss tail's gradient only")
     if done:
         ctx.tail = None
     elif getattr(ctx, "mask_table", None) is not None:
diff --git a/acm_gnn_amd/graph.py b/acm_gnn_amd/graph.py
--- a/acm_gnn_amd/graph.py
+++ b/acm_gnn_amd/graph.py
@@ -161,6 +161,20 @@
             _lib.check(_lib.load().acm_csr_slice_rows(self._h, int(begin), int(end), 0, C.byref(out)),
                        "acm_csr_slice_rows")
         return CsrGraph(out.value, self.device)
+
+    def select_rows(self, mask):
+        if mask.dtype != torch.uint8 or mask.dim() != 1 or not mask.is_contiguous() or mask.device != torch.device(self.device):
+            raise ValueError(f"select_rows: the mask must be a contiguous uint8 vector on {self.device}")
+        if mask.numel() != self.n_rows:
+            raise ValueError(f"select_rows: {mask.numel()} mask entries for {self.n_rows} rows")
+        out = C.c_void_p()
+        with _device_ctx(self.device):
+            _sync(self.device)
+            st = _lib.load().acm_csr_select_rows(self._h, mask.data_ptr(), C.byref(out))
+        _lib.check(st, "acm_csr_select_rows")
+        child = CsrGraph(out.value, self.device)
+        child._parent = self
+        return child
 
     def arrays(self):
         _sync(self.device)
diff --git a/acm_gnn_amd/train.py b/acm_gnn_amd/train.py
--- a/acm_gnn_amd/train.py
+++ b/acm_gnn_amd/train.py
@@ -114,8 +114,22 @@
             if why is None:
                 self.small = SmallPlan(model, self.x, self.adj, self.labels, self.weights, optimizer)
                 self.pipe = None
+        self.restrict, self.restrict_refused = None, "not requested"
+        self._build_restrict()
         if use_graph:
             self._capture()
+
+    def _build_restrict(self):
+        if self.small is not None:
+            why = "the fused small-graph step"
+        elif not self._takes_call:
+            why = "the model does not take the step's CallContext"
+        else:
+            why = AF.RestrictedOutput.why_not(self.model, self.adj, self.weights)
+        self._restrict_version = self.weights._version
+        self.restrict = AF.RestrictedOutput(self.adj, self.weights) if why is None else None
+        self.restrict_refused = why
+        return self.restrict
 
     def _one_step(self):
         if self.small is not None:
@@ -135,8 +149,12 @@
                 self.pipe = pipe = None
             else:
                 pipe.prime()
+        restrict = self.restrict
+        if self.weights._version != self._restrict_version:
+            capturing = self.weights.is_cuda and torch.cuda.is_current_stream_capturing()
+            restrict = None if capturing else self._build_restrict()
         pending = AF.DeferredReductions() if self._defer else None
-        call = AF.CallContext(defer=pending, pipe=pipe)
+        call = AF.CallContext(defer=pending, pipe=pipe, restrict=restrict)
         tape = AF.Tape() if (self._tape and not (torch.cuda.is_available() and torch.cuda.is_current_stream_capturing())) else None
         rng = _rng_snapshot(self.labels.device) if (tape is not None and not self._tape_proven) else None
         try:
diff --git a/acm_gnn_amd/tuning.py b/acm_gnn_amd/tuning.py
--- a/acm_gnn_amd/tuning.py
+++ b/acm_gnn_amd/tuning.py
@@ -4,9 +4,10 @@
 import threading
 
 KERNEL_KEYS = ("chunk", "wide_form", "bwd_split", "rows16", "agg_fused", "gemm_forms")
-HOST_DEFAULTS = {"rewrites": 15, "implicit": 1, "relabel": -1, "pipeline": 8192, "csr_features": 256, "small_step": 16384}
+HOST_DEFAULTS = {"rewrites": 15, "implicit": 1, "relabel": -1, "pipeline": 8192, "csr_features": 256, "small_step": 16384,
+                 "restrict": 1}
 HOST_RANGES = {"rewrites": (0, 15), "implicit": (0, 1), "relabel": (-1, 1), "pipeline": (0, 1 << 31), "csr_features": (0, 1 << 31),
-               "small_step": (0, 16384)}
+               "small_step": (0, 16384), "restrict": (0, 1)}
 
 REWRITE_AGG_FIRST = 1
 REWRITE_ACMII_RECOMPUTE = 2
diff --git a/include/acm_hip.h b/include/acm_hip.h
--- a/include/acm_hip.h
+++ b/include/acm_hip.h
@@ -8,7 +8,7 @@
 extern "C" {
 #endif
 
-#define ACM_ABI_VERSION 28
+#define ACM_ABI_VERSION 29
 
 typedef enum {
     ACM_OK = 0,
@@ -43,6 +43,8 @@
 int acm_csr_transpose(const acm_csr_t* a, int chunk, acm_csr_t** out);
 int acm_csr_slice_rows(const acm_csr_t* a, int64_t row_begin, int64_t row_end,
                        int chunk, acm_csr_t** out);
+
+int acm_csr_select_rows(const acm_csr_t* a, const uint8_t* row_mask_dev, acm_csr_t** out);
 void acm_csr_destroy(acm_csr_t* a);
 
 int acm_shard_plan(int64_t n_rows, const int64_t* indptr_host, int world, int64_t row_cost,
```

Result: no change. 49.60 billion edges/s (-0.6%).
